# mimbres/neural-audio-fp

Measured on AMD Instinct MI355X. Metric: fingerprint generation throughput (1-s segments/s), higher is better.
Workload: dtype f32

## Files before the change

include/nafp.h:

```cpp
#ifndef NAFP_H
#define NAFP_H

#include <stdint.h>

#ifdef __cplusplus
extern "C" {
#endif

#define NAFP_ABI_VERSION 1

enum {
    NAFP_OK = 0,
    NAFP_ERR_INVALID_ARG = 1,
    NAFP_ERR_UNSUPPORTED = 2,
    NAFP_ERR_HIP = 3,
    NAFP_ERR_WORKSPACE = 4,
    NAFP_ERR_NO_WEIGHTS = 5
};

typedef struct nafp_melspec nafp_melspec;
typedef struct nafp_encoder nafp_encoder;

int nafp_abi_version(void);
const char* nafp_status_string(int status);
int nafp_last_hip_error(void);
uint32_t nafp_crc32c_host(const void* data_host, int64_t n, uint32_t crc);


int nafp_mel_filterbank_host(int fs, int n_fft, int n_mels, float f_min, float f_max,
                             float* out_host);

int nafp_melspec_create(nafp_melspec** plan, int fs, int seg_len, int n_fft, int hop,
                        int n_mels, float f_min, float f_max);
int nafp_melspec_destroy(nafp_melspec* plan);
int nafp_melspec_n_frames(const nafp_melspec* plan);
int nafp_melspec_n_mels(const nafp_melspec* plan);

#define NAFP_MELSPEC_DEFER 2
int nafp_melspec_forward_f32(nafp_melspec* plan, const float* audio, int64_t n_seg,
                             int group_size, int segment_norm, float* feat,
                             float* group_stat, void* stream);
int nafp_melspec_forward_i16(nafp_melspec* plan, const int16_t* audio, int64_t n_seg,
                             int group_size, int segment_norm, float* feat,
                             float* group_stat, void* stream);

int nafp_melspec_finish(nafp_melspec* plan, float* feat, const float* group_stat, int64_t n_seg, int group_size,
                        int segment_norm, void* stream);

int nafp_melspec_forward_windows_i16(nafp_melspec* plan, const int16_t* pcm, const int64_t* seg_offset,
                                     const int32_t* seg_valid, int64_t n_seg, int group_size,
                                     int segment_norm, float* feat, float* group_stat, void* stream);


int nafp_encoder_create(nafp_encoder** enc, int in_f, int in_t, int emb_sz);
int nafp_encoder_destroy(nafp_encoder* enc);

#define NAFP_NORM_LAYER2D 0
#define NAFP_NORM_LAYER1D 1
#define NAFP_NORM_BATCH 2
int nafp_encoder_create_ex(nafp_encoder** enc, int in_f, int in_t, int emb_sz, int norm);
int nafp_encoder_norm(const nafp_encoder* enc);
int nafp_encoder_n_trainable(const nafp_encoder* enc);

int nafp_encoder_n_tensors(const nafp_encoder* enc);
int64_t nafp_encoder_tensor_numel(const nafp_encoder* enc, int index);
int nafp_encoder_tensor_shape(const nafp_encoder* enc, int index, int64_t dims_out[4]);
int64_t nafp_encoder_flat_dim(const nafp_encoder* enc);

int nafp_encoder_set_weights(nafp_encoder* enc, const float* const* tensors_host_array,
                             void* stream);

int64_t nafp_encoder_workspace_bytes(const nafp_encoder* enc, int64_t n_seg);

int nafp_encoder_forward(nafp_encoder* enc, const float* feat, int64_t n_seg,
                         void* workspace, int64_t workspace_bytes,
                         float* out_flat, float* out_emb, int l2norm, void* stream);

int nafp_encoder_forward_raw(nafp_encoder* enc, const float* raw_feat, const float* group_stat, int group_size,
                             int segment_norm, int64_t n_seg, void* workspace, int64_t workspace_bytes,
                             float* out_flat, float* out_emb, int l2norm, void* stream);

#define NAFP_ENCODER_PROFILE_KERNELS 17
int nafp_encoder_profile_enable(nafp_encoder* enc, int max_forwards);
int nafp_encoder_profile_count(const nafp_encoder* enc);
int nafp_encoder_profile_coarse(nafp_encoder* enc, int coarse);
int nafp_encoder_profile_read(nafp_encoder* enc, int slot, float* ms_out_host);
int nafp_conv_timeline(void* dev_buf, int64_t capacity_u64, int cin, int cout, int positions);
int nafp_conv_timeline_grid(int* out5_host);

int64_t nafp_encoder_train_workspace_bytes(const nafp_encoder* enc, int64_t n_seg);
int nafp_encoder_forward_train(nafp_encoder* enc, const float* feat, int64_t n_seg, void* workspace,
                               int64_t workspace_bytes, float* out_emb, int l2norm, void* stream);
int nafp_encoder_backward(nafp_encoder* enc, const float* feat, const float* d_emb, int64_t n_seg,
                          void* workspace, int64_t workspace_bytes, float* const* grads_host_array,
                          int l2norm, void* stream);

#define NAFP_GRAD_GROUPS 4
int nafp_encoder_grad_group_range(const nafp_encoder* enc, int group, int* first_tensor, int* last_tensor);
int nafp_encoder_grad_group_wait(nafp_encoder* enc, int group, void* stream);

#define NAFP_OPT_FUSE_CONV0 1
#define NAFP_OPT_FUSED_LN_BWD 2
#define NAFP_OPT_BWD_OVERLAP 4
#define NAFP_OPT_SMALLNET 5
#define NAFP_OPT_BF16X3 3
int nafp_encoder_set_option(nafp_encoder* enc, int option, int value);

int nafp_encoder_div_enc(nafp_encoder* enc, const float* flat, int64_t n_seg,
                         float* out_emb, int l2norm, void* stream);

int nafp_l2_normalize_rows(const float* x, int64_t n_rows, int dim, float* out, void* stream);

int nafp_pack_embedding_grads(const float* d_a_all, const float* d_b_all, const float* loss_sum, float loss_scale,
                              int64_t world, int64_t n_anchors, int dim, float* send, void* stream);


int64_t nafp_ntxent_workspace_bytes(int64_t n_local, int64_t n_global);

int nafp_ntxent_forward(const float* emb_org_local, const float* emb_rep_local,
                        const float* emb_org_all, const float* emb_rep_all,
                        int64_t n_local, int64_t n_global, int64_t rank_offset, int d,
                        float tau, float* loss_sum, float* sim_mtx,
                        float* d_org_all, float* d_rep_all,
                        void* workspace, int64_t workspace_bytes, void* stream);


typedef struct { int f0, f1, t0, t1; } nafp_rect;

int nafp_specaug_apply(float* feat, int64_t n_seg, int F, int T, const nafp_rect* rects_host,
                       int n_rects, const unsigned char* active, float fill_value, void* stream);

int nafp_specaug_apply_fill_dev(float* feat, int64_t n_seg, int F, int T, const nafp_rect* rects_host,
                                int n_rects, const unsigned char* active, const float* fill_value_dev,
                                void* stream);
int64_t nafp_specaug_mean_workspace_bytes(void);
int nafp_specaug_mean(const float* feat, int64_t n, float* mean_out, void* workspace, int64_t workspace_bytes,
                      void* stream);

int nafp_specaug_apply_ex(float* feat, int64_t n_seg, int F, int T, const int32_t* rects_dev, int n_rects, int64_t n_sets,
                          const unsigned char* active_dev, const float* filler, int64_t n_fill_seg,
                          const float* scale_offset_dev, void* stream);
int nafp_specaug_range(const float* feat, int64_t n, float* scale_offset_out, void* workspace, int64_t workspace_bytes,
                       void* stream);


typedef struct {
    float* param; const float* grad; float* m; float* v;
    int64_t numel; int64_t var_len;
} nafp_opt_tensor;

float nafp_cosine_decay_lr_host(float lr0, int64_t step, int64_t decay_steps, float alpha);
float nafp_cosine_decay_restarts_lr_host(float lr0, int64_t step, int64_t first_decay_steps, float t_mul,
                                         float m_mul, float alpha);

int nafp_adam_step(const nafp_opt_tensor* tensors_host, int n, float lr, float beta1, float beta2,
                   float eps, int64_t step, void* stream);

int64_t nafp_lamb_workspace_bytes(const nafp_opt_tensor* tensors_host, int n);
int nafp_lamb_step(const nafp_opt_tensor* tensors_host, int n, float lr, float beta1, float beta2,
                   float eps, float weight_decay, int64_t step, void* workspace,
                   int64_t workspace_bytes, void* stream);

int64_t nafp_triplet_workspace_bytes(int64_t n_anchor, int64_t n_pos);
int nafp_triplet_forward(const float* emb_anchor, const float* emb_pos, int64_t n_anchor, int64_t n_pos, int dim,
                         int mode, float margin, float* loss_out, float* pairwise_dist, float* d_anchor,
                         float* d_pos, void* workspace, int64_t workspace_bytes, void* stream);

typedef struct nafp_aug_row {
    int64_t ev_off;
    int64_t nz_off;
    int64_t nz2_off;
    int64_t ir_off;
    int32_t ev_valid;
    int32_t nz_valid, nz2_valid;
    int32_t ir_len;
    float snr_db;
    float amp;
    int32_t mix;
    int32_t reserved;
} nafp_aug_row;

int nafp_augment_rows(const int16_t* pcm, const nafp_aug_row* rows, int64_t n_rows, int seg_len, float* out,
                      void* stream);


int64_t nafp_search_index_aux_floats(int64_t n_index);
int nafp_search_index_prepare(const float* index, int64_t n_index, int dim, float* aux, void* stream);

int64_t nafp_search_workspace_bytes(int64_t n_query, int64_t n_index, int k);
int nafp_search_topk_l2(const float* query, int64_t n_query, const float* index, const float* aux,
                        int64_t n_index, int dim, int k, float* out_dist, int32_t* out_ids,
                        void* workspace, int64_t workspace_bytes, void* stream);

int nafp_search_seq_scores(const float* query, const float* index, int64_t n_index, int dim,
                           const int32_t* task_q0, const int32_t* task_len, int64_t n_tasks,
                           const int32_t* cand, int n_slots, float* out_scores, void* stream);

int nafp_minisearch_scores(const float* query, const float* db, int64_t n_query, int64_t n_db, int dim, int mode,
                           float* out_scores, void* stream);
int nafp_minisearch_ranks(const float* scores, int64_t n_query, int64_t n_db, int scope, int mode, int gt_id_offset,
                          int32_t* out_rank, void* stream);

#ifdef __cplusplus
}
#endif
#endif
```

neural-audio-fp_amd/csrc/api.hip:

```cpp
#include "nafp_common.h"

#include <algorithm>
#include <cstdlib>
#include <cstring>
#include <vector>

namespace nafp {

thread_local int g_last_hip_error = 0;

static const int kHiddenCh[8] = {128, 128, 256, 256, 512, 512, 1024, 1024};
static const int kStrideT[8] = {2, 2, 2, 2, 1, 2, 1, 2};

std::vector<ConvGeom> encoder_geometry(int in_f, int in_t) {
    std::vector<ConvGeom> g;
    int F = in_f, T = in_t, C = 1;
    for (int i = 0; i < 8; ++i) {
        SamePad pt = same_pad(T, 3, kStrideT[i]);
        g.push_back(ConvGeom{0, F, T, C, F, pt.n_out, kHiddenCh[i], kStrideT[i], pt.before});
        T = pt.n_out; C = kHiddenCh[i];
        SamePad pf = same_pad(F, 3, 2);
        g.push_back(ConvGeom{1, F, T, C, pf.n_out, T, kHiddenCh[i], 2, pf.before});
        F = pf.n_out;
    }
    return g;
}

struct CopyTable { const float* src[96]; float* dst[96]; int64_t n[96]; int nz[96]; int count; int* nonfinite; };
__device__ __forceinline__ float nz_scale(float g) { return fabsf(g) < 1e-30f ? copysignf(1e-30f, g) : g; }
__device__ __forceinline__ bool nonfinite4(float4 v) {
    return !(fabsf(v.x) <= 3.4028234664e38f) || !(fabsf(v.y) <= 3.4028234664e38f) || !(fabsf(v.z) <= 3.4028234664e38f) || !(fabsf(v.w) <= 3.4028234664e38f);
}
__global__ __launch_bounds__(256) void multi_copy_kernel(const CopyTable t) {
    const int e = blockIdx.y;
    const float* __restrict__ s = t.src[e]; float* __restrict__ d = t.dst[e];
    const int64_t n = t.n[e];
    const bool nz = t.nz[e] != 0;
    bool bad = false;
    if ((((uintptr_t)s | (uintptr_t)d) & 15) == 0) {
        for (int64_t i = blockIdx.x * 256ll + threadIdx.x; i < n / 4; i += (int64_t)gridDim.x * 256) {
            float4 v = ((const float4*)s)[i];
            bad = bad || nonfinite4(v);
            if (nz) { v.x = nz_scale(v.x); v.y = nz_scale(v.y); v.z = nz_scale(v.z); v.w = nz_scale(v.w); }
            ((float4*)d)[i] = v;
        }
        for (int64_t i = n / 4 * 4 + blockIdx.x * 256ll + threadIdx.x; i < n; i += (int64_t)gridDim.x * 256) {
            bad = bad || !(fabsf(s[i]) <= 3.4028234664e38f);
            d[i] = nz ? nz_scale(s[i]) : s[i];
        }
    } else {
        for (int64_t i = blockIdx.x * 256ll + threadIdx.x; i < n; i += (int64_t)gridDim.x * 256) {
            bad = bad || !(fabsf(s[i]) <= 3.4028234664e38f);
            d[i] = nz ? nz_scale(s[i]) : s[i];
        }
    }
    if (bad && t.nonfinite) atomicOr(t.nonfinite, 1);
}
#define NAFP_OPT_DEBUG_SIDE_DELAY 6
#define NAFP_OPT_DEBUG_SW_DELAY 7
__global__ void debug_delay_kernel(long long us) {
    const unsigned long long t0 = __builtin_amdgcn_s_memrealtime();
    while ((long long)(__builtin_amdgcn_s_memrealtime() - t0) < us * 100) __builtin_amdgcn_s_sleep(32);
}
struct BiasTable { float* hb[16]; const float* bias[16]; int64_t n[16]; int cout[16]; int count; };
__global__ __launch_bounds__(256) void add_bias_kernel(const BiasTable t) {
    const int e = blockIdx.y;
    float* __restrict__ h = t.hb[e]; const float* __restrict__ b = t.bias[e];
    const int64_t n = t.n[e]; const int C = t.cout[e];
    for (int64_t i = blockIdx.x * 256ll + threadIdx.x; i < n; i += (int64_t)gridDim.x * 256) h[i] += b[i % C];
}

}

using namespace nafp;

constexpr int NAFP_PROF_EV = 34;
struct nafp_encoder {
    int in_f, in_t, emb_sz;
    int norm = NAFP_NORM_LAYER2D;
    int n_trainable = 68;
    std::vector<float*> d_gc, d_bc, d_mm, d_mv;
    bool ln1d_images_set = false;
    std::vector<ConvGeom> geom;
    int64_t flat_dim; int S;
    std::vector<std::vector<int64_t>> shapes;
    float* d_blob = nullptr;
    int64_t blob_floats = 0;
    std::vector<float*> d_w;
    std::vector<float*> d_bias, d_gamma, d_beta;
    std::vector<float*> d_G, d_Hb;
    float *d_w1p = nullptr, *d_b1p = nullptr, *d_w2p = nullptr, *d_b2 = nullptr;
    std::vector<float*> d_wd;
    float *d_w1k = nullptr, *d_b1k = nullptr, *d_w2k = nullptr;
    double* d_inv_n = nullptr;
    int* d_wflag = nullptr;
    float* d_sw_slab = nullptr; int64_t sw_slab_floats = 0;
    bool has_weights = false;
    hipEvent_t sw_copied = nullptr, sw_l1 = nullptr, sw_done = nullptr;
    hipStream_t sw_stream = nullptr;
    bool sw_recorded = false;
    bool opt_fuse_conv0 = []() { const char* v = getenv("NAFP_FUSE0"); return v && v[0] == '1'; }();
    int opt_fused_ln_bwd = []() { const char* v = getenv("NAFP_DGRAD_LN"); return v ? atoi(v) : 0; }();
    int64_t bufA_per_seg = 0, bufB_per_seg = 0;
    std::vector<hipEvent_t> prof_events;
    int prof_max = 0, prof_count = 0;
    int opt_bf16x3 = 0;
    float* d_x6_blob = nullptr; std::vector<float*> d_whm; std::vector<void*> d_wl; bool x6_dirty = true;
    std::vector<float*> d_wdhm; std::vector<void*> d_wdl;
    int prof_coarse = 0;
    hipEvent_t grad_events[NAFP_GRAD_GROUPS] = {nullptr, nullptr, nullptr, nullptr};
    bool grad_events_valid = false;
    int opt_bwd_overlap = []() { const char* v = getenv("NAFP_BWD_OVERLAP"); return v ? atoi(v) : 2; }();
    bool keep_t_env = []() { const char* v = getenv("NAFP_KEEP_T"); return v && v[0] == '1'; }();
    bool keep_t() const { return keep_t_env || (opt_fused_ln_bwd != 0 && norm == NAFP_NORM_LAYER2D) || norm == NAFP_NORM_LAYER1D; }
    struct TrainRec { const void* ws; int64_t B; bool keep_t; };
    std::vector<TrainRec> train_recs;
    void train_rec_put(const void* ws, int64_t B, bool kt) {
        for (auto& r : train_recs) if (r.ws == ws) { r.B = B; r.keep_t = kt; return; }
        if (train_recs.size() >= 16) train_recs.erase(train_recs.begin());
        train_recs.push_back({ws, B, kt});
    }
    bool train_rec_ok(const void* ws, int64_t B, bool kt) const {
        for (const auto& r : train_recs) if (r.ws == ws) return r.B == B && r.keep_t == kt;
        return false;
    }
    hipStream_t side_stream = nullptr;
    hipEvent_t ev_main[16] = {}, ev_side[16] = {};
    int debug_side_delay_us = 0;
    int debug_sw_delay_us = 0;
    static constexpr int NAFP_SW_STREAMS = 4;
    hipStream_t sw_streams[NAFP_SW_STREAMS] = {};
    hipEvent_t sw_fork = nullptr, sw_join[NAFP_SW_STREAMS] = {};
};

static const int kGroupFirst[NAFP_GRAD_GROUPS] = {48, 32, 16, 0};
static const int kGroupLast[NAFP_GRAD_GROUPS] = {67, 47, 31, 15};

static void profile_free(nafp_encoder* e) {
    for (auto ev : e->prof_events) (void)hipEventDestroy(ev);
    e->prof_events.clear();
    e->prof_max = 0; e->prof_count = 0;
}

static int64_t numel(const std::vector<int64_t>& s) {
    int64_t n = 1;
    for (auto d : s) n *= d;
    return n;
}

extern "C" int nafp_abi_version(void) { return NAFP_ABI_VERSION; }

extern "C" const char* nafp_status_string(int status) {
    switch (status) {
        case NAFP_OK: return "ok";
        case NAFP_ERR_INVALID_ARG: return "invalid argument";
        case NAFP_ERR_UNSUPPORTED: return "unsupported geometry or option";
        case NAFP_ERR_HIP: return "HIP runtime error";
        case NAFP_ERR_WORKSPACE: return "workspace too small";
        case NAFP_ERR_NO_WEIGHTS: return "encoder weights not set";
        default: return "unknown status";
    }
}

extern "C" int nafp_last_hip_error(void) { return g_last_hip_error; }

extern "C" uint32_t nafp_crc32c_host(const void* data, int64_t n, uint32_t crc) {
    static uint32_t T[8][256];
    static bool init = false;
    if (!init) {
        for (uint32_t i = 0; i < 256; ++i) {
            uint32_t c = i;
            for (int k = 0; k < 8; ++k) c = (c >> 1) ^ (0x82F63B78u & (0u - (c & 1u)));
            T[0][i] = c;
        }
        for (uint32_t i = 0; i < 256; ++i)
            for (int t = 1; t < 8; ++t) T[t][i] = (T[t - 1][i] >> 8) ^ T[0][T[t - 1][i] & 0xffu];
        init = true;
    }
    const unsigned char* p = (const unsigned char*)data;
    uint32_t c = ~crc;
    while (n > 0 && ((uintptr_t)p & 7)) { c = (c >> 8) ^ T[0][(c ^ *p++) & 0xffu]; --n; }
    while (n >= 8) {
        uint64_t w; memcpy(&w, p, 8);
        w ^= c;
        c = T[7][w & 0xff] ^ T[6][(w >> 8) & 0xff] ^ T[5][(w >> 16) & 0xff] ^ T[4][(w >> 24) & 0xff] ^
            T[3][(w >> 32) & 0xff] ^ T[2][(w >> 40) & 0xff] ^ T[1][(w >> 48) & 0xff] ^ T[0][(w >> 56) & 0xff];
        p += 8; n -= 8;
    }
    while (n-- > 0) c = (c >> 8) ^ T[0][(c ^ *p++) & 0xffu];
    return ~c;
}

extern "C" int nafp_encoder_create(nafp_encoder** out, int in_f, int in_t, int emb_sz) {
    return nafp_encoder_create_ex(out, in_f, in_t, emb_sz, NAFP_NORM_LAYER2D);
}
extern "C" int nafp_encoder_norm(const nafp_encoder* e) { return e ? e->norm : -1; }
extern "C" int nafp_encoder_n_trainable(const nafp_encoder* e) { return e ? e->n_trainable : -1; }

extern "C" int nafp_encoder_create_ex(nafp_encoder** out, int in_f, int in_t, int emb_sz, int norm) {
    if (!out || in_f <= 0 || in_t <= 0 || emb_sz <= 0) return NAFP_ERR_INVALID_ARG;
    if (norm != NAFP_NORM_LAYER2D && norm != NAFP_NORM_LAYER1D && norm != NAFP_NORM_BATCH) return NAFP_ERR_INVALID_ARG;
    nafp_encoder* e = new nafp_encoder();
    e->in_f = in_f; e->in_t = in_t; e->emb_sz = emb_sz; e->norm = norm;
    e->geom = encoder_geometry(in_f, in_t);
    const ConvGeom& last = e->geom.back();
    e->flat_dim = (int64_t)last.Fout * last.Tout * last.Cout;
    if (e->flat_dim % emb_sz != 0 || emb_sz % 64 != 0 || emb_sz > 256 || e->flat_dim / emb_sz > 16) {
        delete e; return NAFP_ERR_UNSUPPORTED;
    }
    e->S = (int)(e->flat_dim / emb_sz);
    for (int j = 0; j < 16; ++j) {
        const ConvGeom& g = e->geom[j];
        if (g.axis == 0) e->shapes.push_back({1, 3, g.Cin, g.Cout});
        else             e->shapes.push_back({3, 1, g.Cin, g.Cout});
        e->shapes.push_back({g.Cout});
        e->shapes.push_back({g.Fout, g.Tout, g.Cout});
        e->shapes.push_back({g.Fout, g.Tout, g.Cout});
    }
    e->shapes.push_back({emb_sz, e->S, 32});
    e->shapes.push_back({emb_sz, 32});
    e->shapes.push_back({emb_sz, 32, 1});
    e->shapes.push_back({emb_sz, 1});
    int64_t total = 0;
    for (auto& s : e->shapes) total += (numel(s) + 63) / 64 * 64;
    if (norm != NAFP_NORM_LAYER2D) for (int j = 0; j < 16; ++j) total += 4 * ((e->geom[j].Cout + 63) / 64 * 64);
    for (int j = 1; j < 16; ++j) total += 2 * ((numel(e->shapes[4 * j + 2]) + 63) / 64 * 64);
    for (int j = 1; j < 16; ++j) total += (numel(e->shapes[4 * j]) + 63) / 64 * 64;
    total += (numel(e->shapes[64]) + 63) / 64 * 64 + 2 * ((numel(e->shapes[65]) + 63) / 64 * 64) + 64 + 64;
    for (int j = 1; j < 16; ++j) e->sw_slab_floats = std::max(e->sw_slab_floats, conv_gemm_slab_floats(2, e->geom[j]));
    total += nafp_encoder::NAFP_SW_STREAMS * (e->sw_slab_floats + 64);
    e->blob_floats = total;
    hipError_t err = hipMalloc(&e->d_blob, sizeof(float) * total);
    if (err != hipSuccess) { g_last_hip_error = (int)err; delete e; return NAFP_ERR_HIP; }
    float* p = e->d_blob;
    auto take = [&](int idx) { float* r = p; p += (numel(e->shapes[idx]) + 63) / 64 * 64; return r; };
    for (int j = 0; j < 16; ++j) {
        e->d_w.push_back(take(4 * j));
        e->d_bias.push_back(take(4 * j + 1));
        e->d_gamma.push_back(take(4 * j + 2));
        e->d_beta.push_back(take(4 * j + 3));
    }
    e->d_w1p = take(64); e->d_b1p = take(65); e->d_w2p = take(66); e->d_b2 = take(67);
    e->d_G.push_back(nullptr); e->d_Hb.push_back(nullptr);
    for (int j = 1; j < 16; ++j) { e->d_G.push_back(take(4 * j + 2)); e->d_Hb.push_back(take(4 * j + 2)); }
    e->d_wd.push_back(nullptr);
    for (int j = 1; j < 16; ++j) e->d_wd.push_back(take(4 * j));
    e->d_w1k = take(64); e->d_b1k = take(65); e->d_w2k = take(65);
    e->d_inv_n = (double*)p; p += 64;
    e->d_wflag = (int*)p; p += 64;
    e->d_sw_slab = p; p += nafp_encoder::NAFP_SW_STREAMS * (e->sw_slab_floats + 64);
    if (norm != NAFP_NORM_LAYER2D)
        for (int j = 0; j < 16; ++j) {
            const int64_t c = (e->geom[j].Cout + 63) / 64 * 64;
            e->d_gc.push_back(p); e->d_bc.push_back(p + c); e->d_mm.push_back(p + 2 * c); e->d_mv.push_back(p + 3 * c); p += 4 * c;
        }
    for (int j = 0; j < 16; ++j) {
        const int64_t n = numel(e->shapes[4 * j + 2]);
        if (e->d_beta[j] != e->d_gamma[j] + n || (j >= 1 && e->d_Hb[j] != e->d_G[j] + n)) {
            (void)hipFree(e->d_blob); delete e; return NAFP_ERR_UNSUPPORTED;
        }
    }
    {
        double inv_n[16];
        for (int j = 0; j < 16; ++j) inv_n[j] = 1.0 / ((double)e->geom[j].Fout * e->geom[j].Tout * e->geom[j].Cout);
        err = hipMemcpy(e->d_inv_n, inv_n, sizeof(inv_n), hipMemcpyHostToDevice);
        if (err != hipSuccess) { g_last_hip_error = (int)err; (void)hipFree(e->d_blob); delete e; return NAFP_ERR_HIP; }
    }
    for (int j = 0; j < 16; ++j) {
        const ConvGeom& g = e->geom[j];
        const int64_t n = (int64_t)g.Fout * g.Tout * g.Cout;
        if (j % 2 == 0) e->bufA_per_seg = std::max(e->bufA_per_seg, n);
        else            e->bufB_per_seg = std::max(e->bufB_per_seg, n);
    }
    if (norm != NAFP_NORM_LAYER2D) {
        for (int j = 0; j < 16; ++j) { e->shapes[4 * j + 2] = {e->geom[j].Cout}; e->shapes[4 * j + 3] = {e->geom[j].Cout}; }
        if (norm == NAFP_NORM_BATCH)
            for (int j = 0; j < 16; ++j) { e->shapes.push_back({e->geom[j].Cout}); e->shapes.push_back({e->geom[j].Cout}); }
    }
    *out = e;
    return NAFP_OK;
}

extern "C" int nafp_encoder_destroy(nafp_encoder* e) {
    if (!e) return NAFP_OK;
    if (e->d_blob) (void)hipFree(e->d_blob);
    if (e->d_x6_blob) (void)hipFree(e->d_x6_blob);
    profile_free(e);
    for (auto& ev : e->grad_events) if (ev) (void)hipEventDestroy(ev);
    for (auto& ev : e->ev_main) if (ev) (void)hipEventDestroy(ev);
    for (auto& ev : e->ev_side) if (ev) (void)hipEventDestroy(ev);
    if (e->side_stream) (void)hipStreamDestroy(e->side_stream);
    for (auto& q : e->sw_streams) if (q) (void)hipStreamDestroy(q);
    for (auto& ev : e->sw_join) if (ev) (void)hipEventDestroy(ev);
    if (e->sw_fork) (void)hipEventDestroy(e->sw_fork);
    if (e->sw_copied) (void)hipEventDestroy(e->sw_copied);
    if (e->sw_l1) (void)hipEventDestroy(e->sw_l1);
    if (e->sw_done) (void)hipEventDestroy(e->sw_done);
    delete e;
    return NAFP_OK;
}

static int split_weights(nafp_encoder* e, hipStream_t st, int j_lo, int j_hi) {
    SplitTable t; t.count = 0;
    for (int j = j_lo; j <= j_hi; ++j) {
        const int64_t n = (int64_t)e->geom[j].Cout * 3 * e->geom[j].Cin;
        t.wp[t.count] = e->d_w[j]; t.hm[t.count] = e->d_whm[j]; t.wl[t.count] = e->d_wl[j]; t.n8[t.count] = n / 8; t.K[t.count] = 3 * e->geom[j].Cin; ++t.count;
        if (e->geom[j].Cout % 16 == 0 && e->d_wd[j]) {
            t.wp[t.count] = e->d_wd[j]; t.hm[t.count] = e->d_wdhm[j]; t.wl[t.count] = e->d_wdl[j]; t.n8[t.count] = n / 8; t.K[t.count] = 3 * e->geom[j].Cout; ++t.count;
        }
    }
    return launch_split_weights_multi(t, st);
}
static int split_all_weights(nafp_encoder* e, hipStream_t st) {
    { int rcs = split_weights(e, st, 1, 15); if (rcs != NAFP_OK) return rcs; }
    e->x6_dirty = false;
    return NAFP_OK;
}

extern "C" int nafp_encoder_set_option(nafp_encoder* e, int option, int value) {
    if (!e) return NAFP_ERR_INVALID_ARG;
    switch (option) {
        case NAFP_OPT_FUSE_CONV0: e->opt_fuse_conv0 = value != 0; return NAFP_OK;
        case NAFP_OPT_BF16X3:
            if (value < 0 || value > 2) return NAFP_ERR_INVALID_ARG;
            if (value == 2 && !e->d_x6_blob) {
                int64_t tot = 0;
                for (int j = 1; j < 16; ++j) tot += 2 * (((int64_t)e->geom[j].Cout * 3 * e->geom[j].Cin * 3 / 2 + 63) / 64 * 64);
                hipError_t er = hipMalloc(&e->d_x6_blob, sizeof(float) * tot);
                if (er != hipSuccess) { g_last_hip_error = (int)er; e->d_x6_blob = nullptr; return NAFP_ERR_HIP; }
                float* q = e->d_x6_blob;
                e->d_whm.assign(16, nullptr); e->d_wl.assign(16, nullptr); e->d_wdhm.assign(16, nullptr); e->d_wdl.assign(16, nullptr);
                for (int j = 1; j < 16; ++j) {
                    const int64_t n = (int64_t)e->geom[j].Cout * 3 * e->geom[j].Cin;
                    e->d_whm[j] = q; e->d_wl[j] = q + n; q += (n * 3 / 2 + 63) / 64 * 64;
                    e->d_wdhm[j] = q; e->d_wdl[j] = q + n; q += (n * 3 / 2 + 63) / 64 * 64;
                }
                e->x6_dirty = true;
            }
            e->opt_bf16x3 = value; return NAFP_OK;
        case NAFP_OPT_FUSED_LN_BWD:
            if (value < 0 || value > 2) return NAFP_ERR_INVALID_ARG;
            e->opt_fused_ln_bwd = value; return NAFP_OK;
        case NAFP_OPT_BWD_OVERLAP: e->opt_bwd_overlap = value < 0 ? 0 : (value > 2 ? 1 : value); return NAFP_OK;
        case NAFP_OPT_SMALLNET: return NAFP_OK;
        case NAFP_OPT_DEBUG_SIDE_DELAY:
        case NAFP_OPT_DEBUG_SW_DELAY: {
            static const bool hooks = []() { const char* v = getenv("NAFP_TEST_HOOKS"); return v && v[0] == '1'; }();
            if (!hooks) return NAFP_ERR_UNSUPPORTED;
            (option == NAFP_OPT_DEBUG_SIDE_DELAY ? e->debug_side_delay_us : e->debug_sw_delay_us) = value < 0 ? 0 : value; return NAFP_OK;
        }
        default: return NAFP_ERR_INVALID_ARG;
    }
}

extern "C" int nafp_encoder_n_tensors(const nafp_encoder* e) { return e ? (int)e->shapes.size() : -1; }

extern "C" int64_t nafp_encoder_tensor_numel(const nafp_encoder* e, int index) {
    if (!e || index < 0 || index >= (int)e->shapes.size()) return -1;
    return numel(e->shapes[index]);
}

extern "C" int nafp_encoder_tensor_shape(const nafp_encoder* e, int index, int64_t dims_out[4]) {
    if (!e || !dims_out || index < 0 || index >= (int)e->shapes.size()) return -1;
    const auto& s = e->shapes[index];
    for (size_t i = 0; i < s.size(); ++i) dims_out[i] = s[i];
    return (int)s.size();
}

extern "C" int64_t nafp_encoder_flat_dim(const nafp_encoder* e) { return e ? e->flat_dim : -1; }

extern "C" int nafp_encoder_set_weights(nafp_encoder* e, const float* const* t, void* stream) {
    if (!e || !t) return NAFP_ERR_INVALID_ARG;
    for (size_t i = 0; i < e->shapes.size(); ++i)
        if (!t[i]) return NAFP_ERR_INVALID_ARG;
    hipStream_t st = (hipStream_t)stream;
    CopyTable ct; ct.count = 0;
    auto add_copy = [&](const float* src, float* dst, int64_t n, int nz = 0) { ct.src[ct.count] = src; ct.dst[ct.count] = dst; ct.n[ct.count] = n; ct.nz[ct.count] = nz; ++ct.count; };
    add_copy(t[0], e->d_w[0], 3 * e->geom[0].Cout);
    for (int j = 0; j < 16; ++j) {
        const ConvGeom& g = e->geom[j];
        const int64_t nln = (int64_t)g.Fout * g.Tout * g.Cout;
        add_copy(t[4 * j + 1], e->d_bias[j], g.Cout);
        if (e->norm == NAFP_NORM_LAYER2D) {
            add_copy(t[4 * j + 2], e->d_gamma[j], nln, 1);
            add_copy(t[4 * j + 3], e->d_beta[j], nln);
        } else {
            add_copy(t[4 * j + 2], e->d_gc[j], g.Cout);
            add_copy(t[4 * j + 3], e->d_bc[j], g.Cout);
            if (e->norm == NAFP_NORM_BATCH) { add_copy(t[68 + 2 * j], e->d_mm[j], g.Cout); add_copy(t[69 + 2 * j], e->d_mv[j], g.Cout); }
        }
    }
    add_copy(t[64], e->d_w1k, numel(e->shapes[64]));
    add_copy(t[65], e->d_b1k, numel(e->shapes[65]));
    add_copy(t[66], e->d_w2k, numel(e->shapes[66]));
    add_copy(t[67], e->d_b2, e->emb_sz);
    if (!e->sw_copied) {
        NAFP_HIP_CHECK(hipEventCreateWithFlags(&e->sw_copied, hipEventDisableTiming));
        NAFP_HIP_CHECK(hipEventCreateWithFlags(&e->sw_done, hipEventDisableTiming));
        NAFP_HIP_CHECK(hipEventCreateWithFlags(&e->sw_l1, hipEventDisableTiming));
    }
    e->sw_recorded = false;
    NAFP_HIP_CHECK(hipMemsetAsync(e->d_wflag, 0, sizeof(int), st));
    ct.nonfinite = e->d_wflag;
    multi_copy_kernel<<<dim3(32, ct.count), 256, 0, st>>>(ct);
    NAFP_LAUNCH_CHECK();
    if (e->norm == NAFP_NORM_LAYER1D && !e->ln1d_images_set) {
        e->ln1d_images_set = true;
        for (int j = 0; j < 16; ++j) {
            const int64_t nln = (int64_t)e->geom[j].Fout * e->geom[j].Tout * e->geom[j].Cout;
            NAFP_HIP_CHECK(hipMemsetD32Async((hipDeviceptr_t)e->d_gamma[j], 0x3f800000, nln, st));
            NAFP_HIP_CHECK(hipMemsetAsync(e->d_beta[j], 0, sizeof(float) * nln, st));
        }
    } else if (e->norm == NAFP_NORM_BATCH) {
        BnExpandTable bx; bx.count = 16;
        for (int j = 0; j < 16; ++j) {
            bx.gamma_c[j] = e->d_gc[j]; bx.beta_c[j] = e->d_bc[j]; bx.mmean[j] = e->d_mm[j]; bx.mvar[j] = e->d_mv[j];
            bx.gamma_pos[j] = e->d_gamma[j]; bx.n[j] = (int64_t)e->geom[j].Fout * e->geom[j].Tout * e->geom[j].Cout; bx.C[j] = e->geom[j].Cout;
        }
        int rcx = launch_bn_expand(bx, st);
        if (rcx != NAFP_OK) return rcx;
    }
    NAFP_HIP_CHECK(hipEventRecord(e->sw_copied, st));
    auto sw_delay = [&]() -> int {
        if (e->debug_sw_delay_us <= 0) return NAFP_OK;
        debug_delay_kernel<<<1, 64, 0, st>>>((long long)e->debug_sw_delay_us);
        NAFP_LAUNCH_CHECK();
        return NAFP_OK;
    };
    { int rcd = sw_delay(); if (rcd != NAFP_OK) return rcd; }
    auto split_l1 = [&]() -> int { return e->opt_bf16x3 == 2 ? split_weights(e, st, 1, 1) : NAFP_OK; };
    {
        PackTable pt; pt.count = 0; pt.nonfinite = e->d_wflag;
        for (int j = 1; j < 16; ++j) {
            pt.k3[pt.count] = t[4 * j]; pt.wp[pt.count] = e->d_w[j]; pt.wd[pt.count] = e->d_wd[j];
            pt.cin[pt.count] = e->geom[j].Cin; pt.cout[pt.count] = e->geom[j].Cout; ++pt.count;
        }
        int rc = launch_multi_pack(pt, st);
        if (rc != NAFP_OK) return rc;
    }
    BiasTable bt; bt.count = 0;
    static const int ns_env = []() { const char* v = getenv("NAFP_SW_NSTREAMS"); return v ? atoi(v) : nafp_encoder::NAFP_SW_STREAMS; }();
    static const bool gemv_own = []() { const char* v = getenv("NAFP_SW_GEMV_OWN"); return v && v[0] == '1'; }();
    const int NS = std::max(1, std::min<int>(nafp_encoder::NAFP_SW_STREAMS, ns_env));
    if (!e->sw_fork) {
        NAFP_HIP_CHECK(hipEventCreateWithFlags(&e->sw_fork, hipEventDisableTiming));
        for (int k = 0; k < NS; ++k) {
            NAFP_HIP_CHECK(hipStreamCreateWithFlags(&e->sw_streams[k], hipStreamNonBlocking));
            NAFP_HIP_CHECK(hipEventCreateWithFlags(&e->sw_join[k], hipEventDisableTiming));
        }
    }
    bool l1_done = false;
    if (!gh_gemv_eligible(e->geom[1])) {
        ConvGemmArgs a{};
        a.wp = e->d_w[1]; a.plain = true; a.x = e->d_gamma[0]; a.bias = nullptr; a.y = e->d_G[1];
        a.slab = e->sw_slab_floats ? e->d_sw_slab : nullptr; a.slab_floats = e->sw_slab_floats;
        int rc1 = launch_conv_gemm(a, 2, e->geom[1], st);
        if (rc1 != NAFP_OK) return rc1;
        BiasTable b1; b1.count = 1;
        b1.hb[0] = e->d_Hb[1]; b1.bias[0] = e->d_bias[1]; b1.n[0] = (int64_t)e->geom[1].Fout * e->geom[1].Tout * e->geom[1].Cout; b1.cout[0] = e->geom[1].Cout;
        add_bias_kernel<<<dim3(32, 1), 256, 0, st>>>(b1);
        NAFP_LAUNCH_CHECK();
        l1_done = true;
        { int rcs = split_l1(); if (rcs != NAFP_OK) return rcs; }
        NAFP_HIP_CHECK(hipEventRecord(e->sw_l1, st));
        { int rcd = sw_delay(); if (rcd != NAFP_OK) return rcd; }
    }
    NAFP_HIP_CHECK(hipEventRecord(e->sw_fork, st));
    int fork_rc = NAFP_OK;
    int forked = 0;
    for (int k = 0; k < NS && fork_rc == NAFP_OK; ++k) {
        if (hipStreamWaitEvent(e->sw_streams[k], e->sw_fork, 0) != hipSuccess) fork_rc = NAFP_ERR_HIP; else ++forked;
    }
    GhTable gh; gh.count = 0;
    bool by_gemv[16] = {};
    for (int j = 1; j < 16; ++j)
        if (gh.count < GH_MAX_LAYERS && gh_gemv_eligible(e->geom[j])) {
            gh_table_add(gh, e->geom[j], e->d_w[j], e->d_gamma[j - 1], e->d_G[j]);
            by_gemv[j] = true;
            bt.hb[bt.count] = e->d_Hb[j]; bt.bias[bt.count] = e->d_bias[j];
            bt.n[bt.count] = (int64_t)e->geom[j].Fout * e->geom[j].Tout * e->geom[j].Cout; bt.cout[bt.count] = e->geom[j].Cout; ++bt.count;
        }
    if (fork_rc == NAFP_OK && forked == NS) fork_rc = launch_gh_gemv(gh, gemv_own ? st : e->sw_streams[NS - 1]);
    else for (int j = 1; j < 16; ++j) by_gemv[j] = false;
    if (forked != NS) bt.count = 0;
    int n_tiled = 0;
    for (int j = 1; j < 16 && fork_rc == NAFP_OK; ++j) {
        if (by_gemv[j] || (j == 1 && l1_done)) continue;
        const int k = (n_tiled++) % NS;
        ConvGemmArgs a{};
        a.wp = e->d_w[j]; a.plain = true;
        a.x = e->d_gamma[j - 1]; a.bias = nullptr; a.y = e->d_G[j];
        a.slab = e->sw_slab_floats ? e->d_sw_slab + (int64_t)k * (e->sw_slab_floats + 64) : nullptr; a.slab_floats = e->sw_slab_floats;
        fork_rc = launch_conv_gemm(a, 2, e->geom[j], e->sw_streams[k]);
        bt.hb[bt.count] = e->d_Hb[j]; bt.bias[bt.count] = e->d_bias[j];
        bt.n[bt.count] = (int64_t)e->geom[j].Fout * e->geom[j].Tout * e->geom[j].Cout; bt.cout[bt.count] = e->geom[j].Cout; ++bt.count;
    }
    for (int k = 0; k < forked; ++k) {
        if (hipEventRecord(e->sw_join[k], e->sw_streams[k]) != hipSuccess || hipStreamWaitEvent(st, e->sw_join[k], 0) != hipSuccess) {
            (void)hipStreamSynchronize(e->sw_streams[k]);
            if (fork_rc == NAFP_OK) fork_rc = NAFP_ERR_HIP;
        }
    }
    if (fork_rc != NAFP_OK) return fork_rc;
    add_bias_kernel<<<dim3(32, bt.count), 256, 0, st>>>(bt);
    NAFP_LAUNCH_CHECK();
    int rc = launch_pack_div(t[64], t[65], t[66], e->d_w1p, e->d_b1p, e->d_w2p, e->emb_sz, e->S, st);
    if (rc != NAFP_OK) return rc;
    if (!l1_done) {
        { int rcs = split_l1(); if (rcs != NAFP_OK) return rcs; }
        NAFP_HIP_CHECK(hipEventRecord(e->sw_l1, st));
        { int rcd = sw_delay(); if (rcd != NAFP_OK) return rcd; }
    }
    e->x6_dirty = true;
    if (e->opt_bf16x3 == 2) {
        int rcs = split_weights(e, st, 2, 15);
        if (rcs != NAFP_OK) return rcs;
        e->x6_dirty = false;
    }
    NAFP_HIP_CHECK(hipEventRecord(e->sw_done, st));
    e->sw_stream = st; e->sw_recorded = true;
    e->has_weights = true;
    return NAFP_OK;
}

static int wait_weights(nafp_encoder* e, hipStream_t st, int stage = 2) {
    if (!e->sw_recorded || st == e->sw_stream) return NAFP_OK;
    NAFP_HIP_CHECK(hipStreamWaitEvent(st, stage == 0 ? e->sw_copied : (stage == 1 ? e->sw_l1 : e->sw_done), 0));
    return NAFP_OK;
}

static int64_t align_up(int64_t v, int64_t a) { return (v + a - 1) / a * a; }

static int64_t forward_slab_floats(const nafp_encoder* e, int64_t n_seg) {
    int64_t slab = 0;
    for (int j = 1; j < 16; ++j) slab = std::max(slab, conv_gemm_slab_floats(n_seg, e->geom[j], false, fwd_plan_b()));
    return slab;
}

extern "C" int64_t nafp_encoder_workspace_bytes(const nafp_encoder* e, int64_t n_seg) {
    if (!e || n_seg < 0) return -1;
    const int64_t stats = align_up((int64_t)sizeof(double) * 2 * 16 * n_seg, 256) + NAFP_TICKET_SLOTS * (int64_t)sizeof(unsigned);
    const int64_t a = align_up((int64_t)sizeof(float) * e->bufA_per_seg * n_seg, 256);
    const int64_t b = align_up((int64_t)sizeof(float) * e->bufB_per_seg * n_seg, 256);
    return stats + a + b + align_up(forward_slab_floats(e, n_seg) * (int64_t)sizeof(float), 256) + 256;
}

static int encoder_forward_impl(nafp_encoder* e, const float* feat, const float* gstat, int group_size, int segment_norm,
                                int64_t n_seg, void* workspace, int64_t workspace_bytes, float* out_flat,
                                float* out_emb, int l2norm, void* stream);

extern "C" int nafp_encoder_forward(nafp_encoder* e, const float* feat, int64_t n_seg,
                                    void* workspace, int64_t workspace_bytes,
                                    float* out_flat, float* out_emb, int l2norm, void* stream) {
    return encoder_forward_impl(e, feat, nullptr, 0, 0, n_seg, workspace, workspace_bytes, out_flat, out_emb, l2norm, stream);
}

extern "C" int nafp_encoder_forward_raw(nafp_encoder* e, const float* raw_feat, const float* group_stat, int group_size,
                                        int segment_norm, int64_t n_seg, void* workspace, int64_t workspace_bytes,
                                        float* out_flat, float* out_emb, int l2norm, void* stream) {
    if (!group_stat) return NAFP_ERR_INVALID_ARG;
    if (group_size <= 0 || group_size > n_seg) group_size = (int)std::min<int64_t>(n_seg, INT32_MAX);
    return encoder_forward_impl(e, raw_feat, group_stat, group_size, segment_norm & 1, n_seg, workspace, workspace_bytes,
                                out_flat, out_emb, l2norm, stream);
}

static int encoder_forward_impl(nafp_encoder* e, const float* feat, const float* gstat, int group_size, int segment_norm,
                                int64_t n_seg, void* workspace, int64_t workspace_bytes, float* out_flat,
                                float* out_emb, int l2norm, void* stream) {
    if (!e || !feat || !workspace || n_seg < 0) return NAFP_ERR_INVALID_ARG;
    if (!e->has_weights) return NAFP_ERR_NO_WEIGHTS;
    if (n_seg == 0) return NAFP_OK;
    if (workspace_bytes < nafp_encoder_workspace_bytes(e, n_seg)) return NAFP_ERR_WORKSPACE;
    if (n_seg * e->bufA_per_seg >= ((int64_t)1 << 40)) return NAFP_ERR_UNSUPPORTED;
    hipStream_t st = (hipStream_t)stream;
    char* ws = (char*)align_up((int64_t)(uintptr_t)workspace, 256);
    const int64_t stats_only = align_up((int64_t)sizeof(double) * 2 * 16 * n_seg, 256);
    const int64_t stats_bytes = stats_only + NAFP_TICKET_SLOTS * (int64_t)sizeof(unsigned);
    stat_t* stats = (stat_t*)ws;
    unsigned* tickets = (unsigned*)(ws + stats_only);
    float* bufA = (float*)(ws + stats_bytes);
    float* bufB = (float*)(ws + stats_bytes + align_up((int64_t)sizeof(float) * e->bufA_per_seg * n_seg, 256));
    float* slab = (float*)((char*)bufB + align_up((int64_t)sizeof(float) * e->bufB_per_seg * n_seg, 256));
    const int64_t slab_floats = forward_slab_floats(e, n_seg);
    { int wrc = wait_weights(e, st); if (wrc != NAFP_OK) return wrc; }
    if (e->opt_bf16x3 == 2 && e->x6_dirty) {
        { int rcs = split_all_weights(e, st); if (rcs != NAFP_OK) return rcs; }
        if (!e->sw_done) NAFP_HIP_CHECK(hipEventCreateWithFlags(&e->sw_done, hipEventDisableTiming));
        NAFP_HIP_CHECK(hipEventRecord(e->sw_done, st));
        e->sw_stream = st; e->sw_recorded = true;
    }
    NAFP_HIP_CHECK(hipMemsetAsync(stats, 0, stats_bytes, st));
    hipEvent_t* ev = nullptr;
    if (e->prof_max > 0 && e->prof_count < e->prof_max) ev = e->prof_events.data() + (size_t)NAFP_PROF_EV * e->prof_count++;
    if (ev && e->prof_coarse < 2) NAFP_HIP_CHECK(hipEventRecord(ev[0], st));

    const bool alt = e->norm != NAFP_NORM_LAYER2D;
    auto stats_of = [&](int j) { return stats + 2 * n_seg * j; };
    auto row_pass = [&](float* z, int j) -> int {
        if (e->norm != NAFP_NORM_LAYER1D) return NAFP_OK;
        return launch_ln1d_fwd(z, n_seg * e->geom[j].Fout * e->geom[j].Tout, e->geom[j].Cout, e->d_gc[j], e->d_bc[j], st);
    };
    static const bool x6_fuse0 = []() { const char* v = getenv("NAFP_X6_FUSE0"); return !v || v[0] != '0'; }();
    const bool fuse0 = !alt && (e->opt_fuse_conv0 || (e->opt_bf16x3 == 2 && x6_fuse0)) && e->geom[1].axis == 1 && e->geom[1].Cin % 16 == 0 &&
                       e->geom[0].Tin <= 64 && (e->opt_bf16x3 != 2 || e->geom[1].Cin == 128);
    int rc = fuse0 ? launch_conv0_stats(feat, e->d_w[0], e->d_bias[0], stats, n_seg, e->geom[0], st, gstat, group_size, segment_norm)
                   : launch_conv0(feat, e->d_w[0], e->d_bias[0], e->d_gamma[0], bufA, nullptr, stats, n_seg, e->geom[0], st,
                                  gstat, group_size, segment_norm, alt);
    if (rc != NAFP_OK) return rc;
    if (!fuse0) { rc = row_pass(bufA, 0); if (rc != NAFP_OK) return rc; }
    if (ev && e->prof_coarse < 2) NAFP_HIP_CHECK(hipEventRecord(ev[1], st));
    float* cur = bufA;
    for (int j = 1; j < 16; ++j) {
        float* nxt = (j % 2 == 0) ? bufA : bufB;
        ConvGemmArgs a{};
        a.x = cur; a.stats_in = stats_of(j - 1); a.ident_stats = alt;
        a.wp = e->d_w[j]; a.G = e->d_G[j]; a.Hb = e->d_Hb[j]; a.gamma_out = e->d_gamma[j];
        a.y = nxt; a.stats_out = stats + 2 * n_seg * j; a.plain = false;
        a.slab = slab_floats ? slab : nullptr; a.slab_floats = slab_floats; a.tickets = tickets; a.bf16x3 = e->opt_bf16x3;
        static const int x6_layers = []() { const char* v = getenv("NAFP_X6_LAYERS"); return v ? (int)strtol(v, nullptr, 0) : 0xffff; }();
        if (!((x6_layers >> j) & 1)) a.bf16x3 = 0;
        if (a.bf16x3 == 2) { a.wp_hm = e->d_whm[j]; a.wp_l = e->d_wl[j]; }
        a.plan_b = fwd_plan_b();
        if (j == 1 && fuse0) {
            a.x = nullptr; a.f0_feat = feat; a.f0_w = e->d_w[0]; a.f0_bias = e->d_bias[0];
            a.f0_gamma = e->d_gamma[0]; a.f0_geom = &e->geom[0];
            a.f0_gstat = gstat; a.f0_group = group_size; a.f0_segnorm = segment_norm;
        }
        if (ev && e->prof_coarse == 0) { a.ev_start = ev[2 * j]; a.ev_stop = ev[2 * j + 1]; }
        if (ev && e->prof_coarse == 2) {
            if (j == 1) a.ev_start = ev[2];
            if (j == 15) a.ev_stop = ev[31];
        }
        rc = launch_conv_gemm(a, n_seg, e->geom[j], st);
        if (rc != NAFP_OK) return rc;
        rc = row_pass(nxt, j);
        if (rc != NAFP_OK) return rc;
        cur = nxt;
    }
    TailArgs t;
    t.x = cur; t.stats = stats_of(15); t.ident_stats = alt; t.gamma = e->d_gamma[15]; t.beta = e->d_beta[15];
    t.w1p = e->d_w1p; t.b1p = e->d_b1p; t.w2p = e->d_w2p; t.b2 = e->d_b2;
    t.out_flat = out_flat; t.out_emb = out_emb;
    t.D = (int)e->flat_dim; t.Q = e->emb_sz; t.S = e->S; t.l2norm = l2norm; t.nonfinite_weights = e->d_wflag; t.launch_error = nullptr;
    if (ev && e->prof_coarse < 2) NAFP_HIP_CHECK(hipEventRecord(ev[32], st));
    rc = launch_tail(t, n_seg, st);
    if (rc != NAFP_OK) return rc;
    if (ev && e->prof_coarse < 2) NAFP_HIP_CHECK(hipEventRecord(ev[33], st));
    return NAFP_OK;
}

extern "C" int nafp_encoder_profile_enable(nafp_encoder* e, int max_forwards) {
    if (!e || max_forwards < 0 || max_forwards > 4096) return NAFP_ERR_INVALID_ARG;
    profile_free(e);
    for (int i = 0; i < max_forwards * NAFP_PROF_EV; ++i) {
        hipEvent_t ev;
        static const int ev_mode = []() { const char* v = getenv("NAFP_PROF_EVENT_FENCE"); return v ? atoi(v) : 0; }();
        hipError_t err = ev_mode == 1 ? hipEventCreate(&ev)
                         : hipEventCreateWithFlags(&ev, ev_mode == 2 ? hipEventReleaseToDevice : hipEventDisableSystemFence);
        if (err != hipSuccess) { g_last_hip_error = (int)err; profile_free(e); return NAFP_ERR_HIP; }
        e->prof_events.push_back(ev);
    }
    e->prof_max = max_forwards;
    return NAFP_OK;
}

extern "C" int nafp_encoder_profile_coarse(nafp_encoder* e, int coarse) {
    if (!e) return NAFP_ERR_INVALID_ARG;
    e->prof_coarse = coarse < 0 ? 0 : (coarse > 2 ? 2 : coarse);
    return NAFP_OK;
}

extern "C" int nafp_encoder_profile_count(const nafp_encoder* e) { return e ? e->prof_count : -1; }

extern "C" int nafp_encoder_profile_read(nafp_encoder* e, int slot, float* ms_out_host) {
    if (!e || !ms_out_host || slot < 0 || slot >= e->prof_count) return NAFP_ERR_INVALID_ARG;
    hipEvent_t* ev = e->prof_events.data() + (size_t)NAFP_PROF_EV * slot;
    NAFP_HIP_CHECK(hipEventSynchronize(e->prof_coarse == 2 ? ev[31] : ev[33]));
    for (int k = 0; k < 17; ++k) ms_out_host[k] = 0.f;
    if (e->prof_coarse == 2) {
        NAFP_HIP_CHECK(hipEventElapsedTime(ms_out_host + 1, ev[2], ev[31]));
        return NAFP_OK;
    }
    NAFP_HIP_CHECK(hipEventElapsedTime(ms_out_host + 0, ev[0], ev[1]));
    NAFP_HIP_CHECK(hipEventElapsedTime(ms_out_host + 16, ev[32], ev[33]));
    if (e->prof_coarse) {
        NAFP_HIP_CHECK(hipEventElapsedTime(ms_out_host + 1, ev[1], ev[32]));
        return NAFP_OK;
    }
    for (int j = 1; j < 16; ++j) NAFP_HIP_CHECK(hipEventElapsedTime(ms_out_host + j, ev[2 * j], ev[2 * j + 1]));
    return NAFP_OK;
}

extern "C" int nafp_conv_timeline(void* dev_buf, int64_t capacity_u64, int cin, int cout, int positions) {
    if (dev_buf && capacity_u64 <= 0) return NAFP_ERR_INVALID_ARG;
    return conv_timeline_set((unsigned long long*)dev_buf, capacity_u64, cin, cout, positions);
}
extern "C" int nafp_conv_timeline_grid(int* out5_host) {
    if (!out5_host) return NAFP_ERR_INVALID_ARG;
    return conv_timeline_grid(out5_host);
}

extern "C" int nafp_encoder_div_enc(nafp_encoder* e, const float* flat, int64_t n_seg,
                                    float* out_emb, int l2norm, void* stream) {
    if (!e || !flat || !out_emb || n_seg < 0) return NAFP_ERR_INVALID_ARG;
    if (!e->has_weights) return NAFP_ERR_NO_WEIGHTS;
    TailArgs t;
    t.x = flat; t.stats = nullptr; t.ident_stats = false; t.gamma = nullptr; t.beta = nullptr;
    t.w1p = e->d_w1p; t.b1p = e->d_b1p; t.w2p = e->d_w2p; t.b2 = e->d_b2;
    t.out_flat = nullptr; t.out_emb = out_emb;
    t.D = (int)e->flat_dim; t.Q = e->emb_sz; t.S = e->S; t.l2norm = l2norm; t.nonfinite_weights = e->d_wflag; t.launch_error = nullptr;
    { int wrc = wait_weights(e, (hipStream_t)stream); if (wrc != NAFP_OK) return wrc; }
    return launch_tail(t, n_seg, (hipStream_t)stream);
}


namespace {
struct TrainLayout {
    int64_t B;
    stat_t* stats; unsigned* tickets; float* mr; float* sc;
    char* zero_begin; int64_t zero_bytes;
    double* lnsum[16]; float* S1[16]; float* S2[16];
    float* z[16]; float* v[16];
    float* slab; int64_t slab_floats;
    float* slab2; int64_t slab2_floats; unsigned* tickets2;
    float* dA; float* dB; float* dy;
    float* dts[16];
    float* dgp; float* dbp;
    int64_t bytes;
};

TrainLayout train_layout(const nafp_encoder* e, int64_t B, void* ws) {
    TrainLayout L; L.B = B;
    char* p = (char*)(((uintptr_t)ws + 255) & ~(uintptr_t)255);
    char* p0 = p;
    auto take = [&](int64_t bytes) { char* r = p; p += (bytes + 255) / 256 * 256; return r; };
    L.stats = (stat_t*)take((int64_t)sizeof(stat_t) * 2 * 16 * B);
    L.tickets = (unsigned*)take(2 * NAFP_TICKET_SLOTS * (int64_t)sizeof(unsigned));
    L.tickets2 = L.tickets + NAFP_TICKET_SLOTS;
    L.mr = (float*)take((int64_t)sizeof(float) * 2 * 16 * B);
    L.sc = (float*)take((int64_t)sizeof(float) * 8 * B);
    L.zero_begin = p;
    for (int j = 0; j < 16; ++j) L.lnsum[j] = (double*)take((int64_t)sizeof(double) * 2 * B);
    for (int j = 0; j < 16; ++j) {
        const int64_t n = (int64_t)e->geom[j].Fout * e->geom[j].Tout * e->geom[j].Cout;
        L.S1[j] = (float*)take((int64_t)sizeof(float) * n);
        L.S2[j] = (float*)take((int64_t)sizeof(float) * n);
    }
    L.zero_bytes = p - L.zero_begin;
    int64_t max_n = 0;
    for (int j = 0; j < 16; ++j) {
        const int64_t n = (int64_t)e->geom[j].Fout * e->geom[j].Tout * e->geom[j].Cout;
        max_n = std::max(max_n, n);
        L.z[j] = (float*)take((int64_t)sizeof(float) * n * B);
        L.v[j] = ((j == 0 && e->norm != NAFP_NORM_LAYER1D) || !e->keep_t()) ? nullptr : (float*)take((int64_t)sizeof(float) * n * B);
    }
    L.slab_floats = 0;
    for (int j = 1; j < 16; ++j)
        L.slab_floats = std::max(L.slab_floats, std::max(conv_gemm_slab_floats(B, e->geom[j], true), wgrad_slab_floats(B, e->geom[j])));
    L.slab = (float*)take((int64_t)sizeof(float) * L.slab_floats);
    L.slab2_floats = 0;
    for (int j = 1; j < 16; ++j)
        if (e->geom[j].Fout * e->geom[j].Tout < 16) L.slab2_floats = std::max(L.slab2_floats, wgrad_slab_floats(B, e->geom[j]));
    L.slab2 = (float*)take((int64_t)sizeof(float) * L.slab2_floats);
    L.dA = (float*)take((int64_t)sizeof(float) * max_n * B);
    L.dB = (float*)take((int64_t)sizeof(float) * max_n * B);
    L.dy = (float*)take((int64_t)sizeof(float) * e->emb_sz * B);
    for (int j = 0; j < 16; ++j) {
        const int64_t n = (int64_t)e->geom[j].Fout * e->geom[j].Tout * e->geom[j].Cout;
        L.dts[j] = (j >= 1 && e->geom[j].Fout * e->geom[j].Tout < 16) ? (float*)take((int64_t)sizeof(float) * n * B) : nullptr;
    }
    L.dgp = nullptr; L.dbp = nullptr;
    if (e->norm != NAFP_NORM_LAYER2D) {
        L.dgp = (float*)take((int64_t)sizeof(float) * 2 * max_n);
        L.dbp = L.dgp + max_n;
// ... 262 lines not shown
```

neural-audio-fp_amd/csrc/conv.hip:

```cpp
#include "nafp_common.h"
#include <hip/hip_ext.h>

#include <cstdlib>

namespace nafp {

using f32x16 = __attribute__((ext_vector_type(16))) float;
using f32x2 = __attribute__((ext_vector_type(2))) float;
#ifndef NAFP_Z_AUX
#define NAFP_Z_AUX 0
#endif
#ifndef NAFP_T_AUX
#define NAFP_T_AUX 2
#endif
__device__ __forceinline__ int f2i(float x) { return __builtin_bit_cast(int, x); }

__device__ __forceinline__ f32x2 elu2(f32x2 t) {
    const f32x2 m = t * 1.44269504088896341f;
    f32x2 e;
    e.x = fminf(fmaxf(__builtin_amdgcn_exp2f(m.x), 0.f), 1.f);
    e.y = fminf(fmaxf(__builtin_amdgcn_exp2f(m.y), 0.f), 1.f);
    e = e - 1.0f;
    f32x2 r;
    r.x = fmaxf(t.x, e.x); r.y = fmaxf(t.y, e.y);
// ... 185 lines not shown
                                                                      gstat, group_size, segment_norm);
        NAFP_LAUNCH_CHECK();
        return NAFP_OK;
    }
    constexpr int R = 32;
    const int64_t blocks = B * ((g.Fin + R - 1) / R);
    conv0_kernel<false, R><<<dim3((unsigned)blocks), 256, 0, st>>>(feat, w3, bias, nullptr, nullptr, nullptr, stats,
                                                                   g.Fin, g.Tin, g.Tout, g.Cout, g.stride, g.pad, gstat, group_size, segment_norm, 0);
    NAFP_LAUNCH_CHECK();
    return NAFP_OK;
}

constexpr int BN = 128;

#ifdef NAFP_ABLATION
#define NAFP_ABL(p_, bits_) ((p_).abl & (bits_))
#elif defined(NAFP_ABL_CONST)
#define NAFP_ABL(p_, bits_) ((NAFP_ABL_CONST) & (bits_))
#else
#define NAFP_ABL(p_, bits_) (0)
#endif

struct ConvKernelParams {
    const float* x;
    const float* wp;
    const float* wp_hm;
    const unsigned short* wp_l;
    const float* G;
    const float* Hb;
    const float* gamma_out;
    const float* bias;
    const stat_t* stats_in;
    stat_t* stats_out;
    float* y;
    float* v_out;
    int Fin, Tin, Cin, Tout, Cout;
    int axis, stride, pad;
    int B, P;
    int PT, ST, log2ST;
    int n_sg;
    int n_pb, log2_ncol;
    int xcd_group, xcd_full;
    int64_t sample_in;
    int tap_stride;
    double inv_n_in;
    int mode;
    int dgrad;
    int perm_on, perm_n0, perm_c0;
    unsigned wp_bytes;
    int n_split;
    int abl;
    unsigned* tickets;
    float* y_final;
    unsigned long long* tl;
    int opt;
    const float* f0_feat;
    const float* f0_w;
    const float* f0_bias;
    const float* f0_gamma;
    int f0_T, f0_stride, f0_pad;
    const float* f0_gstat;
    int f0_group, f0_segnorm;
    ScalarsJob sj;
};

typedef __attribute__((address_space(3))) void* lds_ptr_t;
typedef unsigned u32x4 __attribute__((ext_vector_type(4)));

__device__ __forceinline__ u32x4 make_rsrc(const void* base, unsigned bytes) {
    const unsigned long long a = (unsigned long long)base;
    u32x4 r;
    r.x = __builtin_amdgcn_readfirstlane((unsigned)a);
    r.y = __builtin_amdgcn_readfirstlane((unsigned)(a >> 32) & 0xffffu);
    r.z = __builtin_amdgcn_readfirstlane(bytes);
    r.w = 0x00020000u;
    return r;
}

__device__ __forceinline__ void lds_dma16(unsigned lds_addr, unsigned voff, u32x4 rsrc, unsigned soff) {
    unsigned keep;
    lds_addr = __builtin_amdgcn_readfirstlane(lds_addr);
    soff = __builtin_amdgcn_readfirstlane(soff);
    asm volatile("s_mov_b32 %0, m0\n\ts_mov_b32 m0, %1\n\ts_nop 4\n\t"
                 "buffer_load_dwordx4 %2, %3, %4 offen lds\n\ts_mov_b32 m0, %0"
                 : "=&s"(keep) : "s"(lds_addr), "v"(voff), "s"(rsrc), "s"(soff) : "memory");
}

struct RowGeom { int inner; unsigned mask; };
__device__ __forceinline__ RowGeom row_geom(const ConvKernelParams& p, int pos) {
    const int fo = pos / p.Tout, to = pos - fo * p.Tout;
    RowGeom g; g.mask = 0;
    if (!p.dgrad) {
        int pos0, lim;
        if (p.axis == 0) { pos0 = to * p.stride - p.pad; lim = p.Tin; g.inner = (fo * p.Tin + pos0) * p.Cin; }
        else             { pos0 = fo * p.stride - p.pad; lim = p.Fin; g.inner = (pos0 * p.Tin + to) * p.Cin; }
#pragma unroll
        for (int t = 0; t < 3; ++t)
            if (pos0 + t >= 0 && pos0 + t < lim) g.mask |= 1u << t;
    } else {
        const int u = (p.axis == 0 ? to : fo) + p.pad;
        const int n_out = p.axis == 0 ? p.Tin : p.Fin;
        const int S = p.axis == 0 ? p.Cin : p.Tin * p.Cin;
        const int A0 = p.axis == 0 ? (fo * p.Tin) * p.Cin : to * p.Cin;
        const int sh = p.stride == 2 ? 1 : 0;
        g.inner = A0 + ((u * S) >> sh);
#pragma unroll
        for (int k = 0; k < 3; ++k) {
            const int d = u - k;
            if (d >= 0 && (d & sh) == 0 && (d >> sh) < n_out) g.mask |= 1u << k;
        }
    }
    return g;
}

__device__ __forceinline__ int tile_pos(const ConvKernelParams& p, int idx) {
    if (!p.perm_on || idx >= p.P) return idx;
    if (p.perm_on == 2) {
        const int L = p.Tout, lines = p.P / L, n0 = L - 1;
        if (idx < lines * n0) { const int line = idx / n0; return line * L + (idx - line * n0); }
        return (idx - lines * n0) * L + n0;
    }
    const int n0 = p.perm_n0;
    if (p.axis == 0) {
        const int L = p.Tout, lines = p.P / L, n1 = L - n0;
        if (idx < lines * n0) { const int line = idx / n0; return line * L + 2 * (idx - line * n0) + p.perm_c0; }
        const int j = idx - lines * n0, line = j / n1;
        return line * L + 2 * (j - line * n1) + 1 - p.perm_c0;
    }
    if (idx < n0 * p.Tout) { const int e = idx / p.Tout; return (2 * e + p.perm_c0) * p.Tout + (idx - e * p.Tout); }
    const int j = idx - n0 * p.Tout, e = j / p.Tout;
    return (2 * e + 1 - p.perm_c0) * p.Tout + (j - e * p.Tout);
}

__device__ __forceinline__ float half_wave_sum_dpp(float x) {
    int v = __builtin_bit_cast(int, x);
#define NAFP_DPP_ADD(ctrl_, rmask_)                                                                       \
    v = __builtin_bit_cast(int, __builtin_bit_cast(float, v) +                                            \
                                    __builtin_bit_cast(float, __builtin_amdgcn_update_dpp(0, v, ctrl_, rmask_, 0xf, true)));
    NAFP_DPP_ADD(0x111, 0xf)
    NAFP_DPP_ADD(0x112, 0xf)
    NAFP_DPP_ADD(0x114, 0xf)
    NAFP_DPP_ADD(0x118, 0xf)
    NAFP_DPP_ADD(0x142, 0xa)
#undef NAFP_DPP_ADD
    return __builtin_bit_cast(float, v);
}

#ifndef NAFP_EXP_X6_NOSPLIT
#define NAFP_EXP_X6_NOSPLIT 0
#endif
#ifndef NAFP_EXP_SKIP_TAP2
#define NAFP_EXP_SKIP_TAP2 0
#endif
template <int BM, int BNT, int BK, int NSTAGE, bool FUSE0, int EPI, int PREC = 0>
__device__ __forceinline__ bool conv_gemm_body(const ConvKernelParams& p) {
    static_assert(!FUSE0 || (BK == 16 && BM == 128), "the in-kernel conv0 generator is written for BK = 16, BM = 128");
    static_assert(BM == 128 || BM == 256, "tile rows");
    static_assert(BNT == 128 || (BNT == 64 && BM == 128 && !FUSE0), "tile columns");
    constexpr int NIW = BNT / 64;
    constexpr int NT = 2 * BM;
    constexpr int NW = BM / 32;
    constexpr int CH = BK / 4;
    constexpr int RPI = 64 / CH;
    constexpr int NI = 32 / RPI;
    constexpr int BROWS = BNT / NW;
    constexpr int NIB = BROWS / RPI;
    static_assert(NIB >= 1, "B rows per wave");
    constexpr int TILE = (FUSE0 && PREC == 2) ? BM * 24 : BM * BK;
    constexpr int TILEB = BNT * BK;
    constexpr int LROWS = BNT / NW;
    constexpr int TILEL = PREC == 2 ? BNT * 8 : 0;
    constexpr int STAGE = TILE + TILEB + TILEL;
    constexpr int NDMA = NI + NIB + (PREC == 2 ? 1 : 0);
    extern __shared__ __attribute__((aligned(16))) float smem[];
    float* sRB = smem + NSTAGE * STAGE;
    float* sCB = sRB + BM;
    int* sPos = (int*)(sCB + BM);
    int* sInner = sPos + 32;
    unsigned* sMask = (unsigned*)(sPos + 64);
    float* sW0 = sCB + BM + 96;
    const int tid = threadIdx.x, lane = tid & 63;
    const int wave = __builtin_amdgcn_readfirstlane(tid >> 6);
    const int wm = wave >> 1, wn = wave & 1;
    int sg = blockIdx.x, pb = blockIdx.y, colz = blockIdx.z, zsp = 0;
    if (p.opt & 8) {
        const unsigned lin = blockIdx.x, G = (unsigned)p.xcd_group;
        unsigned v = lin;
        if (lin < (unsigned)p.xcd_full) {
            const unsigned xcd = lin & 7u, j = lin >> 3;
            const unsigned blk = j / G, i = j - blk * G;
            v = (blk * 8u + xcd) * G + i;
        }
        unsigned rt;
        if (p.opt & 16) {
            const unsigned n_rt = (unsigned)(p.n_sg * p.n_pb);
            unsigned t = v / n_rt; rt = v - t * n_rt;
            if (p.n_split > 1) { const unsigned c = t / (unsigned)p.n_split; zsp = (int)(t - c * (unsigned)p.n_split); t = c; }
            colz = (int)t;
        } else {
            colz = (int)(v & ((1u << p.log2_ncol) - 1u)); v >>= p.log2_ncol;
            if (p.n_split > 1) { const unsigned r = v / (unsigned)p.n_split; zsp = (int)(v - r * (unsigned)p.n_split); v = r; }
            rt = v;
        }
        pb = (int)(rt / (unsigned)p.n_sg); sg = (int)(rt - (unsigned)pb * (unsigned)p.n_sg);
    } else
    if (!(p.opt & 4)) { pb = blockIdx.x / p.n_sg; sg = blockIdx.x - pb * p.n_sg; colz = blockIdx.y; zsp = blockIdx.z; }
    if ((EPI == 3 || EPI == 5) && p.sj.sc) {
        const long long wg = blockIdx.x + (long long)gridDim.x * (blockIdx.y + (long long)gridDim.y * blockIdx.z);
        const long long n_wg = (long long)gridDim.x * gridDim.y * gridDim.z;
        for (long long b = wg * NT + tid; b < p.sj.B; b += n_wg * NT) {
            const float mean = p.sj.mr[2 * b], rstd = p.sj.mr[2 * b + 1];
            float* o = p.sj.sc + 8 * b;
            o[0] = mean; o[1] = rstd;
            o[2] = (float)(p.sj.lnsum[2 * b] * p.sj.inv_n); o[3] = (float)(p.sj.lnsum[2 * b + 1] * p.sj.inv_n);
            o[4] = 1.f / rstd;
            o[5] = p.sj.mr_prev ? p.sj.mr_prev[2 * b + 1] : 1.f;
            o[6] = p.sj.mr_prev ? -p.sj.mr_prev[2 * b] : 0.f;
            o[7] = 0.f;
        }
    }
    const int tile_n0 = colz * BNT;
    const int K = 3 * p.Cin;
#define NAFP_TL(k_)                                                                            \
    if (p.tl && lane == 0)                                                                                 \
        p.tl[(((size_t)blockIdx.x + (size_t)gridDim.x * (blockIdx.y + (size_t)gridDim.y * blockIdx.z)) * 8 + wave) * 8 + (k_)] = \
            __builtin_readcyclecounter();
    if (p.tl && lane == 0)
        p.tl[(((size_t)blockIdx.x + (size_t)gridDim.x * (blockIdx.y + (size_t)gridDim.y * blockIdx.z)) * 8 + wave) * 8] =
            (unsigned long long)__builtin_amdgcn_s_getreg(0xF804) |
            ((unsigned long long)__builtin_amdgcn_s_getreg(0xF814) << 32);
    NAFP_TL(1)
    if (p.opt & 1) __builtin_amdgcn_s_setprio(3);
    const int ST1 = p.ST - 1;
    const int b0 = sg * p.ST;
    const int nb = min(p.ST, p.B - b0);

    const bool stat_thread = tid >= 64 && tid < 64 + p.ST;
    double st_sum = 0.0, st_sq = 0.0;
    if (stat_thread && p.mode != 1 && b0 + tid - 64 < p.B) {
        st_sum = stat_get(p.stats_in + 2 * (int64_t)(b0 + tid - 64));
        st_sq = stat_get(p.stats_in + 2 * (int64_t)(b0 + tid - 64) + 1);
        if (st_sq != st_sq && p.stats_out) stat_poison(p.stats_out + 2 * (int64_t)(b0 + tid - 64));
    }
    if (tid < 32) {
        int pos = p.P, inner = 0; unsigned mask = 0;
        if (tid < p.PT) {
            pos = tile_pos(p, pb * p.PT + tid);
            if (pos < p.P) { const RowGeom rg = row_geom(p, pos); inner = rg.inner; mask = rg.mask; }
        }
        sPos[tid] = pos; sInner[tid] = inner; sMask[tid] = mask;
    }
    __syncthreads();

    constexpr unsigned OOB = 0x80000000u;
    unsigned voffA[NI];
    unsigned vmaskA[NI];
    unsigned voffB[NIB];
#pragma unroll
    for (int q = 0; q < NIB; ++q) {
        const int lr = wave * BROWS + q * RPI + lane / CH;
        const int pc = lane % CH;
        const int swz = BK == 32 ? ((lr >> 1) & 7) : ((lr >> 2) & 3);
        voffB[q] = (unsigned)((tile_n0 + lr) * K + (pc ^ swz) * 4) * 4u;
    }
#pragma unroll
    for (int q = 0; q < NI; ++q) {
        const int lr = wave * 32 + q * RPI + lane / CH;
        const int pc = lane % CH;
        const int swz = BK == 32 ? ((lr >> 1) & 7) : ((lr >> 2) & 3);
        const int lc = pc ^ swz;
        const int slot_q = lr >> p.log2ST;
        const int sl = lr & ST1;
        voffA[q] = 0; vmaskA[q] = 0;
        if (sPos[slot_q] < p.P && sl < nb) {
            voffA[q] = (unsigned)(sl * (int)p.sample_in + sInner[slot_q] + lc * 4) * 4u;
            vmaskA[q] = sMask[slot_q];
        }
    }
    float x0[3][3];
    unsigned g_valid = 0;
    int g_off = 0;
    const int g_row = tid >> 1, g_ch = (tid & 1) * 8;
    const int g_swz = (g_row >> 2) & 3;
    if (FUSE0) {
        for (int i = tid; i < 4 * p.Cin; i += NT) sW0[i] = i < 3 * p.Cin ? p.f0_w[i] : p.f0_bias[i - 3 * p.Cin];
#pragma unroll
        for (int t = 0; t < 3; ++t) { x0[t][0] = 0.f; x0[t][1] = 0.f; x0[t][2] = 0.f; }
        const int pos = pb * p.PT + (g_row >> p.log2ST);
        const int sl = g_row & ST1;
        if (pos < p.P && sl < nb) {
            float f0_gmax = 0.f, f0_nh = 0.f, f0_nd = 1.f;
            if (p.f0_gstat) {
                const int64_t gi = p.f0_group > 0 ? (int64_t)(b0 + sl) / p.f0_group : 0;
                f0_gmax = p.f0_gstat[2 * gi];
                if (p.f0_segnorm) { const float mn = fmaxf(p.f0_gstat[2 * gi + 1] - f0_gmax, -80.f); f0_nh = mn / 2.f; f0_nd = fabsf(f0_nh + 1e-10f); }
            }
            const int fo = pos / p.Tout, to = pos - fo * p.Tout;
            const int f00 = fo * p.stride - p.pad;
            g_off = (f00 * p.Tin + to) * p.Cin;
            const int t00 = to * p.f0_stride - p.f0_pad;
            const float* fb = p.f0_feat + ((int64_t)(b0 + sl) * p.Fin) * p.f0_T;
#pragma unroll
            for (int t = 0; t < 3; ++t) {
                const int f = f00 + t;
                if (f >= 0 && f < p.Fin) {
                    g_valid |= 1u << t;
#pragma unroll
                    for (int k = 0; k < 3; ++k) {
                        const int tt = t00 + k;
                        float xv = 0.f;
                        if (tt >= 0 && tt < p.f0_T) {
                            xv = fb[(int64_t)f * p.f0_T + tt];
                            if (p.f0_gstat) {
                                xv = max_keep_nan(xv - f0_gmax, -80.f);
                                if (p.f0_segnorm) xv = (xv - f0_nh) / f0_nd;
                            }
                        }
                        x0[t][k] = xv;
                    }
                }
            }
        }
        __syncthreads();
    }
    unsigned live = 0;
    {
        const unsigned m = sMask[lane & 31];
#pragma unroll
        for (int t = 0; t < 3; ++t)
            if (__ballot((m >> t) & 1u) != 0ull) live |= 1u << t;
    }
    unsigned tap_pack = 0; int n_live = 0;
#pragma unroll
    for (int t = 0; t < 3; ++t)
        if (live & (1u << t)) { tap_pack |= (unsigned)t << (2 * n_live); ++n_live; }
    const int cpt = p.Cin / BK;
    const int n_steps_all = n_live * cpt;
    int s_begin = 0, n_steps = n_steps_all;
    if (p.n_split > 1) {
        s_begin = (int)((unsigned)(n_steps_all * zsp) / (unsigned)p.n_split);
        n_steps = (int)((unsigned)(n_steps_all * (zsp + 1)) / (unsigned)p.n_split);
    }
#define NAFP_STEP_AT(step_, tsel_, c0_)                                                        \
    const int tsel_ = s_begin == 0 ? ((step_) >= cpt ? 1 : 0) : (step_) / cpt;                 \
    const int c0_ = ((step_) - tsel_ * cpt) * BK;

    const u32x4 rsA = make_rsrc(p.x + (int64_t)b0 * p.sample_in,
                                NAFP_ABL(p, 512) ? 0u : (unsigned)nb * (unsigned)p.sample_in * 4u);
    const u32x4 rsB = make_rsrc(PREC == 2 ? p.wp_hm : p.wp, NAFP_ABL(p, 4096) ? 0u : p.wp_bytes);
    const unsigned lds0 = (unsigned)(unsigned long long)(lds_ptr_t)smem + (unsigned)(wave * 32 * BK * 4);
    const unsigned ldsB0 = (unsigned)(unsigned long long)(lds_ptr_t)smem + (unsigned)((TILE + wave * BROWS * BK) * 4);
    const u32x4 rsL = make_rsrc((const float*)p.wp_l, NAFP_ABL(p, 4096) ? 0u : p.wp_bytes / 2);
    const unsigned ldsL0 = (unsigned)(unsigned long long)(lds_ptr_t)smem + (unsigned)((TILE + TILEB) * 4 + wave * LROWS * 32);
    const unsigned voffL = (unsigned)((tile_n0 + wave * LROWS + (lane >> 1)) * K) * 2u + (unsigned)(lane & 1) * 16u;
#define NAFP_DMA_L(slot_, k0_)                                                                 \
    if (PREC == 2 && lane < 2 * LROWS) lds_dma16(ldsL0 + (unsigned)((slot_) * STAGE * 4), voffL, rsL, (unsigned)((k0_) * 2));

#define NAFP_DMA_STEP(s_, slot_)                                                              \
    {                                                                                          \
        NAFP_STEP_AT(s_, tsel_l, c0_l)                                                         \
        const int tap_l = (int)((tap_pack >> (2 * tsel_l)) & 3u);                              \
        const unsigned la_l = lds0 + (unsigned)((slot_) * STAGE * 4);                          \
        const unsigned lb_l = ldsB0 + (unsigned)((slot_) * STAGE * 4);                         \
        const unsigned tapb_l = (unsigned)(tap_l * p.tap_stride) * 4u;                         \
        _Pragma("unroll") for (int q = 0; q < NI; ++q) {                                       \
            const unsigned va = ((vmaskA[q] >> tap_l) & 1u) ? voffA[q] + tapb_l : OOB;         \
            if (!FUSE0) lds_dma16(la_l + q * RPI * BK * 4, va, rsA, (unsigned)(c0_l * 4));     \
            if (q < NIB) lds_dma16(lb_l + q * RPI * BK * 4, voffB[q], rsB,                      \
                                   (unsigned)((tap_l * p.Cin + c0_l) * 4));                    \
        }                                                                                      \
        NAFP_DMA_L(slot_, tap_l * p.Cin + c0_l)                                                \
    }
    float4 gg0 = make_float4(0.f, 0.f, 0.f, 0.f), gg1 = gg0;
#define NAFP_GEN_LOAD(s_)                                                                     \
    {                                                                                          \
        const int tsel_l = (s_) / cpt;                                                         \
        const int tap_l = (int)((tap_pack >> (2 * tsel_l)) & 3u);                              \
        const int c0_l = ((s_) - tsel_l * cpt) * BK;                                           \
        const int go_l = ((g_valid >> tap_l) & 1u) ? g_off + tap_l * p.tap_stride + c0_l + g_ch : 0; \
        gg0 = *(const float4*)(p.f0_gamma + go_l);                                             \
        gg1 = *(const float4*)(p.f0_gamma + go_l + 4);                                         \
    }
#define NAFP_GEN_ONE(j_, G_) \
    __fmul_rn((ok_l ? elu1(fmaf(xc_l, wt_l[2 * p.Cin + (j_)], fmaf(xb_l, wt_l[p.Cin + (j_)], fmaf(xa_l, wt_l[(j_)], wt_l[3 * p.Cin + (j_)])))) : 0.f), (G_))
#define NAFP_GEN_STORE(s_, slot_)                                                             \
    {                                                                                          \
        const int tsel_l = (s_) / cpt;                                                         \
        const int tap_l = (int)((tap_pack >> (2 * tsel_l)) & 3u);                              \
        const int c0_l = ((s_) - tsel_l * cpt) * BK;                                           \
        const bool ok_l = (g_valid >> tap_l) & 1u;                                             \
        const float xa_l = tap_l == 0 ? x0[0][0] : (tap_l == 1 ? x0[1][0] : x0[2][0]);         \
        const float xb_l = tap_l == 0 ? x0[0][1] : (tap_l == 1 ? x0[1][1] : x0[2][1]);         \
        const float xc_l = tap_l == 0 ? x0[0][2] : (tap_l == 1 ? x0[1][2] : x0[2][2]);         \
        const float* wt_l = sW0 + c0_l + g_ch;                                                 \
        float* dst_l = smem + (slot_) * STAGE + g_row * BK;                                    \
        *(float4*)(dst_l + (((2 * (tid & 1)) ^ g_swz) * 4)) = make_float4(                      \
            NAFP_GEN_ONE(0, gg0.x), NAFP_GEN_ONE(1, gg0.y), NAFP_GEN_ONE(2, gg0.z), NAFP_GEN_ONE(3, gg0.w)); \
        *(float4*)(dst_l + (((2 * (tid & 1) + 1) ^ g_swz) * 4)) = make_float4(                  \
            NAFP_GEN_ONE(4, gg1.x), NAFP_GEN_ONE(5, gg1.y), NAFP_GEN_ONE(6, gg1.z), NAFP_GEN_ONE(7, gg1.w)); \
    }

    f32x16 acc[2][NIW];
#pragma unroll
    for (int mi = 0; mi < 2; ++mi)
#pragma unroll
        for (int ni = 0; ni < NIW; ++ni)
#pragma unroll
            for (int r = 0; r < 16; ++r) acc[mi][ni][r] = 0.f;

    NAFP_TL(2)
    if (p.opt & 1) __builtin_amdgcn_s_setprio(0);
#pragma unroll
    for (int s = 0; s < NSTAGE - 1; ++s)
        if (s_begin + s < n_steps) {
            NAFP_DMA_STEP(s_begin + s, s)
            if (FUSE0 && PREC != 2) {
                NAFP_GEN_LOAD(s_begin + s)
                NAFP_GEN_STORE(s_begin + s, s)
            }
        }

    if (stat_thread) {
        float r = 0.f, c = 0.f;
        if (p.mode != 1 && b0 + tid - 64 < p.B) {
            if (p.inv_n_in < 0.0) {
                const double z = st_sq * 0.0;
                r = (float)(1.0 + z); c = (float)z;
            } else {
                const double mean = st_sum * p.inv_n_in;
                double var = st_sq * p.inv_n_in - mean * mean;
                var = var < 0.0 ? 0.0 : var;
                const double rstd = 1.0 / sqrt(var + (double)LN_EPS);
                r = (float)rstd; c = (float)(-mean * rstd);
            }
        }
        sRB[tid - 64] = r; sCB[tid - 64] = c;
    }

    const int rl = lane & 31, hh = lane >> 5;
    const int rswz = BK == 32 ? ((rl >> 1) & 7) : ((rl >> 2) & 3);
    const int aoff = (wm * 64 + rl) * BK, boff = TILE + (wn * (BNT / 2) + rl) * BK;
    const int ncol = lane & 31;
    const int n_base = tile_n0 + wn * (BNT / 2) + ncol;
    const int g4 = p.ST >> 2;
    constexpr int MIL = 1;
    float Gv[MIL][4][NIW], Hv[MIL][4][NIW], gv[MIL][4][NIW];
    const int pc_bytes = p.P * p.Cout * 4;
    const __amdgpu_buffer_rsrc_t rsG = __builtin_amdgcn_make_buffer_rsrc(const_cast<float*>(p.G), 0, pc_bytes, 0x00020000);
    const __amdgpu_buffer_rsrc_t rsH = __builtin_amdgcn_make_buffer_rsrc(const_cast<float*>(p.Hb), 0, pc_bytes, 0x00020000);
    const __amdgpu_buffer_rsrc_t rsg = __builtin_amdgcn_make_buffer_rsrc(const_cast<float*>(p.gamma_out), 0, pc_bytes, 0x00020000);
#define NAFP_EPI_LOAD(mi_, slot_)                                                              \
    _Pragma("unroll") for (int rg = 0; rg < 4; ++rg) {                                         \
        const int grp_l = wm * 16 + (mi_) * 8 + 2 * rg + (lane >> 5);                          \
        const int pos_l = sPos[grp_l >> (p.log2ST - 2)];                \
        const int pofs_l = pos_l < p.P ? (pos_l * p.Cout + n_base) * 4 : (int)0x80000000;      \
        _Pragma("unroll") for (int ni = 0; ni < NIW; ++ni) {                                   \
            if NAFP_ABL(p, 32) { Gv[slot_][rg][ni] = 0.5f; Hv[slot_][rg][ni] = 0.25f; gv[slot_][rg][ni] = 1.5f; continue; } \
            Gv[slot_][rg][ni] = __builtin_bit_cast(float, __builtin_amdgcn_raw_buffer_load_b32(rsG, pofs_l, ni * 128, 0)); \
            Hv[slot_][rg][ni] = __builtin_bit_cast(float, __builtin_amdgcn_raw_buffer_load_b32(rsH, pofs_l, ni * 128, 0)); \
            gv[slot_][rg][ni] = __builtin_bit_cast(float, __builtin_amdgcn_raw_buffer_load_b32(rsg, pofs_l, ni * 128, 0)); \
        }                                                                                      \
    }
    int slot = 0;
    if NAFP_ABL(p, 8) {
        asm volatile("s_waitcnt vmcnt(0)" ::: "memory");
        if (acc[0][0][0] == 12345.678f) p.y[tid] = smem[tid];
        return false;
    }
#define NAFP_LD_FRAG(St_, kk_, a_, b_)                                                         \
    {                                                                                          \
        const int pc4_l = ((2 * (kk_) + hh) ^ rswz) * 4;                                       \
        _Pragma("unroll") for (int mi = 0; mi < 2; ++mi) a_[mi] = *(const float4*)((St_) + aoff + mi * 32 * BK + pc4_l);   \
        _Pragma("unroll") for (int ni = 0; ni < NIW; ++ni) b_[ni] = *(const float4*)((St_) + boff + ni * 32 * BK + pc4_l); \
    }
#define NAFP_MM_FRAG(a_, b_)                                                                   \
    _Pragma("unroll") for (int mi = 0; mi < 2; ++mi)                                           \
        _Pragma("unroll") for (int ni = 0; ni < NIW; ++ni) {                                   \
            acc[mi][ni] = __builtin_amdgcn_mfma_f32_32x32x2f32(a_[mi].x, b_[ni].x, acc[mi][ni], 0, 0, 0); \
            acc[mi][ni] = __builtin_amdgcn_mfma_f32_32x32x2f32(a_[mi].y, b_[ni].y, acc[mi][ni], 0, 0, 0); \
            acc[mi][ni] = __builtin_amdgcn_mfma_f32_32x32x2f32(a_[mi].z, b_[ni].z, acc[mi][ni], 0, 0, 0); \
            acc[mi][ni] = __builtin_amdgcn_mfma_f32_32x32x2f32(a_[mi].w, b_[ni].w, acc[mi][ni], 0, 0, 0); \
        }
#define NAFP_WAIT_STEP(s_)                                                                     \
    if (NSTAGE == 2 || (s_) + NSTAGE - 2 >= n_steps) asm volatile("s_waitcnt vmcnt(0)" ::: "memory"); \
    else asm volatile("s_waitcnt vmcnt(%0)" :: "i"((NSTAGE - 2) * NDMA) : "memory");
    if (!FUSE0 && BK == 16 && !NAFP_ABL(p, 4 | 2048) && s_begin < n_steps) {
        float4 a0[2], b0[NIW], a1[2], b1[NIW];
        NAFP_STEP_AT(s_begin + NSTAGE - 1, d_tsel0, d_c00)
        int d_tsel = d_tsel0, d_c0 = d_c00;
        int d_tap = 0; unsigned d_tapb = 0;
        unsigned cur_va[NI];
#define NAFP_DMA_TAP()                                                                         \
        {                                                                                      \
            d_tap = (int)((tap_pack >> (2 * d_tsel)) & 3u); d_tapb = (unsigned)(d_tap * p.tap_stride) * 4u; \
            _Pragma("unroll") for (int q = 0; q < NI; ++q) cur_va[q] = (((vmaskA[q] >> d_tap) & 1u) && !(NAFP_EXP_SKIP_TAP2 && d_tap == 2)) ? voffA[q] + d_tapb : OOB; \
        }
        NAFP_DMA_TAP()
#define NAFP_DMA_PIECE(q_, slot_)                                                              \
        {                                                                                      \
            lds_dma16(lds0 + (unsigned)((slot_) * STAGE * 4) + (q_) * RPI * BK * 4, cur_va[q_], rsA, (unsigned)(d_c0 * 4)); \
            if ((q_) < NIB) lds_dma16(ldsB0 + (unsigned)((slot_) * STAGE * 4) + (q_) * RPI * BK * 4, voffB[(q_) < NIB ? (q_) : 0], rsB, \
                                      (unsigned)((d_tap * p.Cin + d_c0) * 4));                 \
            if ((q_) == NI - 1) { d_c0 += BK; if (d_c0 == p.Cin) { d_c0 = 0; ++d_tsel; NAFP_DMA_TAP() } } \
        }
#define NAFP_MM_HALF(a_, b_, mi_)                                                              \
        _Pragma("unroll") for (int ni = 0; ni < NIW; ++ni) {                                   \
            acc[mi_][ni] = __builtin_amdgcn_mfma_f32_32x32x2f32(a_[mi_].x, b_[ni].x, acc[mi_][ni], 0, 0, 0); \
            acc[mi_][ni] = __builtin_amdgcn_mfma_f32_32x32x2f32(a_[mi_].y, b_[ni].y, acc[mi_][ni], 0, 0, 0); \
            acc[mi_][ni] = __builtin_amdgcn_mfma_f32_32x32x2f32(a_[mi_].z, b_[ni].z, acc[mi_][ni], 0, 0, 0); \
            acc[mi_][ni] = __builtin_amdgcn_mfma_f32_32x32x2f32(a_[mi_].w, b_[ni].w, acc[mi_][ni], 0, 0, 0); \
        }
        static_assert(NI == 2, "the DMA of a step is issued as two pieces");
        if (PREC >= 1) {
            typedef __bf16 bf16x8 __attribute__((ext_vector_type(8)));
            for (int s = s_begin; s < n_steps; ++s) {
                NAFP_WAIT_STEP(s)
                __builtin_amdgcn_s_barrier();
                if (s == s_begin) { NAFP_TL(3) }
                const bool has_next = s + NSTAGE - 1 < n_steps && !NAFP_ABL(p, 1);
                int nslot = slot + NSTAGE - 1; if (nslot >= NSTAGE) nslot -= NSTAGE;
                const float* St = smem + slot * STAGE;
                float4 af[2][2], bf[PREC == 2 ? 1 : NIW][2];
                bf16x8 ah[2], al[2], bh[NIW], bl[NIW];
                bf16x8 am[PREC == 2 ? 2 : 1], bm[PREC == 2 ? NIW : 1];
#pragma unroll
                for (int c = 0; c < 2; ++c) {
                    const int pc4 = ((2 * hh + c) ^ rswz) * 4;
#pragma unroll
                    for (int mi = 0; mi < 2; ++mi) af[mi][c] = *(const float4*)(St + aoff + mi * 32 * BK + pc4);
                    if (PREC != 2) {
#pragma unroll
                        for (int ni = 0; ni < NIW; ++ni) bf[ni][c] = *(const float4*)(St + boff + ni * 32 * BK + pc4);
                    }
                }
                if (PREC == 2) {
#pragma unroll
                    for (int ni = 0; ni < NIW; ++ni) {
                        bh[ni] = *(const bf16x8*)(St + boff + ni * 32 * BK + ((hh ^ rswz) * 4));
                        bm[ni] = *(const bf16x8*)(St + boff + ni * 32 * BK + (((2 + hh) ^ rswz) * 4));
                        bl[ni] = *(const bf16x8*)(St + TILE + TILEB + (wn * (BNT / 2) + ni * 32 + rl) * 8 + hh * 4);
                    }
                }
                if (has_next) { NAFP_DMA_PIECE(0, nslot) NAFP_DMA_L(nslot, d_tap * p.Cin + d_c0) NAFP_DMA_PIECE(1, nslot) }
#define NAFP_SPLIT8(f_, hi_, mid_, lo_)                                                        \
                {                                                                                  \
                    const float x_l[8] = {f_[0].x, f_[0].y, f_[0].z, f_[0].w, f_[1].x, f_[1].y, f_[1].z, f_[1].w}; \
                    _Pragma("unroll") for (int e = 0; e < 8; ++e) {                                \
                        const __bf16 h_l = (__bf16)x_l[e];                                         \
                        const float r1_l = x_l[e] - (float)h_l;                                    \
                        hi_[e] = h_l;                                                              \
                        if (PREC == 2 && NAFP_EXP_X6_NOSPLIT) {                                    \
                            mid_[e] = h_l; lo_[e] = h_l;       \
                        } else if (PREC == 2) {                                                    \
                            const __bf16 m_l = (__bf16)r1_l;                                       \
                            mid_[e] = m_l; lo_[e] = (__bf16)(r1_l - (float)m_l);                   \
                        } else {                                                                   \
                            lo_[e] = (__bf16)r1_l;                                                 \
                        }                                                                          \
                    }                                                                              \
                }
#define NAFP_SPLIT8_PAIRS(f_, hi_, mid_, lo_)                                                  \
                {                                                                                  \
                    typedef __bf16 bf16x2_l __attribute__((ext_vector_type(2)));                   \
                    typedef float f32x2_l __attribute__((ext_vector_type(2)));                     \
                    typedef unsigned u32x4_l __attribute__((ext_vector_type(4)));                  \
                    const float x_l[8] = {f_[0].x, f_[0].y, f_[0].z, f_[0].w, f_[1].x, f_[1].y, f_[1].z, f_[1].w}; \
                    u32x4_l uh_l, um_l, ul_l;                                                      \
                    _Pragma("unroll") for (int e = 0; e < 4; ++e) {                                \
                        f32x2_l x2; x2.x = x_l[2 * e]; x2.y = x_l[2 * e + 1];                      \
                        const unsigned h2 = __builtin_bit_cast(unsigned, __builtin_convertvector(x2, bf16x2_l)); \
                        f32x2_l r2; r2.x = x2.x - __uint_as_float(h2 << 16); r2.y = x2.y - __uint_as_float(h2 & 0xffff0000u); \
                        const unsigned m2 = __builtin_bit_cast(unsigned, __builtin_convertvector(r2, bf16x2_l)); \
                        f32x2_l t2; t2.x = r2.x - __uint_as_float(m2 << 16); t2.y = r2.y - __uint_as_float(m2 & 0xffff0000u); \
                        uh_l[e] = h2; um_l[e] = m2; ul_l[e] = __builtin_bit_cast(unsigned, __builtin_convertvector(t2, bf16x2_l)); \
                    }                                                                              \
                    hi_ = __builtin_bit_cast(bf16x8, uh_l); mid_ = __builtin_bit_cast(bf16x8, um_l); lo_ = __builtin_bit_cast(bf16x8, ul_l); \
                }
                if (PREC == 2 && !NAFP_EXP_X6_NOSPLIT) {
#pragma unroll
                    for (int mi = 0; mi < 2; ++mi) NAFP_SPLIT8_PAIRS(af[mi], ah[mi], am[PREC == 2 ? mi : 0], al[mi])
                } else {
#pragma unroll
                for (int mi = 0; mi < 2; ++mi) NAFP_SPLIT8(af[mi], ah[mi], am[PREC == 2 ? mi : 0], al[mi])
                }
#undef NAFP_SPLIT8_PAIRS
                if (PREC != 2) {
#pragma unroll
                    for (int ni = 0; ni < NIW; ++ni) NAFP_SPLIT8(bf[PREC == 2 ? 0 : ni], bh[ni], bm[0], bl[ni])
                }
#undef NAFP_SPLIT8
#pragma unroll
                for (int mi = 0; mi < 2; ++mi)
#pragma unroll
                    for (int ni = 0; ni < NIW; ++ni) {
                        if (PREC == 2) {
                            acc[mi][ni] = __builtin_amdgcn_mfma_f32_32x32x16_bf16(al[mi], bh[ni], acc[mi][ni], 0, 0, 0);
                            acc[mi][ni] = __builtin_amdgcn_mfma_f32_32x32x16_bf16(am[PREC == 2 ? mi : 0], bm[PREC == 2 ? ni : 0], acc[mi][ni], 0, 0, 0);
                            acc[mi][ni] = __builtin_amdgcn_mfma_f32_32x32x16_bf16(ah[mi], bl[ni], acc[mi][ni], 0, 0, 0);
                            acc[mi][ni] = __builtin_amdgcn_mfma_f32_32x32x16_bf16(am[PREC == 2 ? mi : 0], bh[ni], acc[mi][ni], 0, 0, 0);
                            acc[mi][ni] = __builtin_amdgcn_mfma_f32_32x32x16_bf16(ah[mi], bm[PREC == 2 ? ni : 0], acc[mi][ni], 0, 0, 0);
                            acc[mi][ni] = __builtin_amdgcn_mfma_f32_32x32x16_bf16(ah[mi], bh[ni], acc[mi][ni], 0, 0, 0);
                        } else {
                            acc[mi][ni] = __builtin_amdgcn_mfma_f32_32x32x16_bf16(al[mi], bh[ni], acc[mi][ni], 0, 0, 0);
                            acc[mi][ni] = __builtin_amdgcn_mfma_f32_32x32x16_bf16(ah[mi], bl[ni], acc[mi][ni], 0, 0, 0);
                            acc[mi][ni] = __builtin_amdgcn_mfma_f32_32x32x16_bf16(ah[mi], bh[ni], acc[mi][ni], 0, 0, 0);
                        }
                    }
                if (++slot == NSTAGE) slot = 0;
            }
        } else {
        {
            NAFP_WAIT_STEP(s_begin)
            __builtin_amdgcn_s_barrier();
            NAFP_TL(3)
            const float* St = smem + slot * STAGE;
            NAFP_LD_FRAG(St, 0, a0, b0)
            NAFP_LD_FRAG(St, 1, a1, b1)
            __builtin_amdgcn_sched_barrier(0);
            if (s_begin + NSTAGE - 1 < n_steps && !NAFP_ABL(p, 1)) { NAFP_DMA_PIECE(0, NSTAGE - 1) NAFP_DMA_PIECE(1, NSTAGE - 1) }
            __builtin_amdgcn_sched_barrier(0);
            NAFP_MM_FRAG(a0, b0)
            __builtin_amdgcn_sched_barrier(0);
            slot = 1;
        }
#define NAFP_K_STEP(SLOT_, NSLOT_)                                                             \
        {                                                                                      \
             \
            asm volatile("s_waitcnt lgkmcnt(0)" ::: "memory");                                 \
            NAFP_WAIT_STEP(s)                                                                  \
            __builtin_amdgcn_s_barrier();                                                      \
            const bool has_next = s + NSTAGE - 1 < n_steps && !NAFP_ABL(p, 1);                 \
            const int nslot = (NSLOT_);                                                        \
            const float* St = smem + (SLOT_) * STAGE;                                          \
            NAFP_LD_FRAG(St, 0, a0, b0)                                                        \
            __builtin_amdgcn_sched_barrier(0);                                                 \
            NAFP_MM_HALF(a1, b1, 0)                                                            \
            __builtin_amdgcn_sched_barrier(0);                                                 \
            if (has_next) { NAFP_DMA_PIECE(0, nslot) }                                         \
            __builtin_amdgcn_sched_barrier(0);                                                 \
            NAFP_MM_HALF(a1, b1, 1)                                                            \
            __builtin_amdgcn_sched_barrier(0);                                                 \
            if (has_next) { NAFP_DMA_PIECE(1, nslot) }                                         \
            NAFP_LD_FRAG(St, 1, a1, b1)                                                        \
            __builtin_amdgcn_sched_barrier(0);                                                 \
            if (s == n_steps - 1) break;           \
            NAFP_MM_FRAG(a0, b0)                                                               \
            __builtin_amdgcn_sched_barrier(0);                                                 \
            ++s;                                                                               \
        }
        static_assert(PREC != 0 || NSTAGE == 3 || BNT == 64, "the K-loop body is written out once per ring slot (128-column tiles)");
        if (s_begin + 1 < n_steps) {
            if (BNT == 128) {
                for (int s = s_begin + 1;;) {
                    NAFP_K_STEP(1, 0)
                    NAFP_K_STEP(2, 1)
                    NAFP_K_STEP(0, 2)
                }
            } else {
                int rs = 1;
                int s = s_begin + 1;
                for (; s < n_steps - 1;) {
                    NAFP_K_STEP(rs, (rs == 0 ? NSTAGE - 1 : rs - 1))
                    if (++rs == NSTAGE) rs = 0;
                }
                do { NAFP_K_STEP(rs, (rs == 0 ? NSTAGE - 1 : rs - 1)) } while (false);
            }
        }
#undef NAFP_K_STEP
        if ((EPI == 0 || EPI == 1) && BM == 128) { NAFP_EPI_LOAD(0, 0) }
        __builtin_amdgcn_sched_barrier(0);
        if (s_begin + 1 < n_steps) { NAFP_MM_FRAG(a0, b0) }
        NAFP_MM_FRAG(a1, b1)
        }
#undef NAFP_DMA_PIECE
#undef NAFP_DMA_TAP
#undef NAFP_MM_HALF
    } else if (FUSE0 && PREC == 2) {
        typedef __bf16 bf16x8 __attribute__((ext_vector_type(8)));
        static_assert(!(FUSE0 && PREC == 2) || NSTAGE == 2, "two ring slots");
        constexpr int C0 = 128;
        const int a_rd = (wm * 64 + rl) * 8 + ((hh ^ ((rl >> 3) & 1)) * 4);
        const int a_wr = g_row * 8 + (((tid & 1) ^ ((g_row >> 3) & 1)) * 4);
        const __amdgpu_buffer_rsrc_t rsG0 = __builtin_amdgcn_make_buffer_rsrc(const_cast<float*>(p.f0_gamma), 0, (int)((unsigned)p.sample_in * 4u), 0x00020000);
        int gvoff0, gvoff1, gvoff2;
        gvoff0 = (g_valid & 1u) ? (g_off + g_ch) * 4 : (int)0x80000000;
        gvoff1 = (g_valid & 2u) ? (g_off + p.tap_stride + g_ch) * 4 : (int)0x80000000;
        gvoff2 = (g_valid & 4u) ? (g_off + 2 * p.tap_stride + g_ch) * 4 : (int)0x80000000;
        const float* wrow = sW0 + g_ch;
        int g_tsel = 0, g_c0 = 0;
        float4 wq[8], gq[2];
        float gxa = 0.f, gxb = 0.f, gxc = 0.f;
#define NAFP_X6_GEN_REQ()                                                                      \
        {                                                                                      \
            const int tap_l = (int)((tap_pack >> (2 * g_tsel)) & 3u);                          \
            gxa = tap_l == 0 ? x0[0][0] : (tap_l == 1 ? x0[1][0] : x0[2][0]);                  \
            gxb = tap_l == 0 ? x0[0][1] : (tap_l == 1 ? x0[1][1] : x0[2][1]);                  \
            gxc = tap_l == 0 ? x0[0][2] : (tap_l == 1 ? x0[1][2] : x0[2][2]);                  \
            const int gv_l = tap_l == 0 ? gvoff0 : (tap_l == 1 ? gvoff1 : gvoff2);             \
            gq[0] = __builtin_bit_cast(float4, __builtin_amdgcn_raw_buffer_load_b128(rsG0, gv_l, g_c0 * 4, 0));      \
            gq[1] = __builtin_bit_cast(float4, __builtin_amdgcn_raw_buffer_load_b128(rsG0, gv_l + 16, g_c0 * 4, 0)); \
            const float* w_l = wrow + g_c0;                                                    \
            _Pragma("unroll") for (int r_ = 0; r_ < 4; ++r_) {                                 \
                wq[2 * r_] = *(const float4*)(w_l + r_ * C0); wq[2 * r_ + 1] = *(const float4*)(w_l + r_ * C0 + 4); \
            }                                                                                  \
            g_c0 += BK; if (g_c0 == C0) { g_c0 = 0; ++g_tsel; }                                \
        }
#define NAFP_X6_GEN_ONE(e_) \
        __fmul_rn(elu1(fmaf(gxc, ((const float*)&wq[4])[e_], fmaf(gxb, ((const float*)&wq[2])[e_], fmaf(gxa, ((const float*)&wq[0])[e_], ((const float*)&wq[6])[e_])))), ((const float*)&gq[0])[e_])
#define NAFP_X6_GEN(slot_)                                                                     \
        {                                                                                      \
            bf16x8 h_l, m_l, l_l;                                                              \
            _Pragma("unroll") for (int e = 0; e < 8; ++e) {                                    \
                const float v_l = NAFP_X6_GEN_ONE(e);                                          \
                const __bf16 hh_l = (__bf16)v_l;                                               \
                const float r1_l = v_l - (float)hh_l;                                          \
                const __bf16 mm_l = (__bf16)r1_l;                                              \
                h_l[e] = hh_l; m_l[e] = mm_l; l_l[e] = (__bf16)(r1_l - (float)mm_l);           \
            }                                                                                  \
            float* dst_l = smem + (slot_) * STAGE + a_wr;                                      \
            *(bf16x8*)dst_l = h_l; *(bf16x8*)(dst_l + BM * 8) = m_l; *(bf16x8*)(dst_l + 2 * BM * 8) = l_l; \
        }
        NAFP_X6_GEN_REQ()
        NAFP_X6_GEN(0)
#define NAFP_X6_MFMAS()                                                                        \
        _Pragma("unroll") for (int mi = 0; mi < 2; ++mi)                                       \
            _Pragma("unroll") for (int ni = 0; ni < NIW; ++ni) {                               \
                acc[mi][ni] = __builtin_amdgcn_mfma_f32_32x32x16_bf16(al[mi], bh[ni], acc[mi][ni], 0, 0, 0); \
                acc[mi][ni] = __builtin_amdgcn_mfma_f32_32x32x16_bf16(am[mi], bm[ni], acc[mi][ni], 0, 0, 0); \
                acc[mi][ni] = __builtin_amdgcn_mfma_f32_32x32x16_bf16(ah[mi], bl[ni], acc[mi][ni], 0, 0, 0); \
                acc[mi][ni] = __builtin_amdgcn_mfma_f32_32x32x16_bf16(am[mi], bh[ni], acc[mi][ni], 0, 0, 0); \
                acc[mi][ni] = __builtin_amdgcn_mfma_f32_32x32x16_bf16(ah[mi], bm[ni], acc[mi][ni], 0, 0, 0); \
                acc[mi][ni] = __builtin_amdgcn_mfma_f32_32x32x16_bf16(ah[mi], bh[ni], acc[mi][ni], 0, 0, 0); \
            }
#define NAFP_X6_READ_FRAGS(St_)                                                                \
        _Pragma("unroll") for (int mi = 0; mi < 2; ++mi) {                                     \
            ah[mi] = *(const bf16x8*)((St_) + a_rd + mi * 32 * 8);                             \
            am[mi] = *(const bf16x8*)((St_) + BM * 8 + a_rd + mi * 32 * 8);                    \
            al[mi] = *(const bf16x8*)((St_) + 2 * BM * 8 + a_rd + mi * 32 * 8);                \
        }                                                                                      \
        _Pragma("unroll") for (int ni = 0; ni < NIW; ++ni) {                                   \
            bh[ni] = *(const bf16x8*)((St_) + boff + ni * 32 * BK + ((hh ^ rswz) * 4));        \
            bm[ni] = *(const bf16x8*)((St_) + boff + ni * 32 * BK + (((2 + hh) ^ rswz) * 4));  \
            bl[ni] = *(const bf16x8*)((St_) + TILE + TILEB + (wn * (BNT / 2) + ni * 32 + rl) * 8 + hh * 4); \
        }
        int s = 0;
        for (; s + 1 < n_steps; ++s) {
            asm volatile("s_waitcnt vmcnt(0) lgkmcnt(0)" ::: "memory");
            __builtin_amdgcn_s_barrier();
            if (s == 0) { NAFP_TL(3) }
            const int nslot = slot ^ 1;
            const float* St = smem + slot * STAGE;
            bf16x8 ah[2], am[2], al[2], bh[NIW], bm[NIW], bl[NIW];
            NAFP_X6_READ_FRAGS(St)
            NAFP_DMA_STEP(s + 1, nslot)
            NAFP_X6_GEN_REQ()
            NAFP_X6_MFMAS()
            NAFP_X6_GEN(nslot)
            slot = nslot;
        }
        {
            asm volatile("s_waitcnt vmcnt(0) lgkmcnt(0)" ::: "memory");
            __builtin_amdgcn_s_barrier();
            const float* St = smem + slot * STAGE;
            bf16x8 ah[2], am[2], al[2], bh[NIW], bm[NIW], bl[NIW];
            NAFP_X6_READ_FRAGS(St)
            NAFP_X6_MFMAS()
        }
#undef NAFP_X6_GEN_REQ
#undef NAFP_X6_GEN_ONE
#undef NAFP_X6_GEN
#undef NAFP_X6_MFMAS
#undef NAFP_X6_READ_FRAGS
    } else
    for (int s = s_begin; s < n_steps; ++s) {
        if (FUSE0) asm volatile("s_waitcnt vmcnt(0) lgkmcnt(0)" ::: "memory");
        else if (NSTAGE == 2 || s + NSTAGE - 2 >= n_steps) asm volatile("s_waitcnt vmcnt(0)" ::: "memory");
        else asm volatile("s_waitcnt vmcnt(%0)" :: "i"((NSTAGE - 2) * (NI + NIB)) : "memory");
        __builtin_amdgcn_s_barrier();
        const bool has_next = s + NSTAGE - 1 < n_steps && !NAFP_ABL(p, 1);
        int nslot = slot + NSTAGE - 1; if (nslot >= NSTAGE) nslot -= NSTAGE;
        const float* St = smem + slot * STAGE;
        if NAFP_ABL(p, 4) {
            if (has_next) { NAFP_DMA_STEP(s + NSTAGE - 1, nslot) }
            if (++slot == NSTAGE) slot = 0;
            continue;
        }
        float4 a0[2], b0[NIW];
        {
            const int pc4 = ((0 + hh) ^ rswz) * 4;
#pragma unroll
            for (int mi = 0; mi < 2; ++mi) a0[mi] = *(const float4*)(St + aoff + mi * 32 * BK + pc4);
#pragma unroll
            for (int ni = 0; ni < NIW; ++ni) b0[ni] = *(const float4*)(St + boff + ni * 32 * BK + pc4);
        }
        if (has_next) {
            NAFP_DMA_STEP(s + NSTAGE - 1, nslot)
            if (FUSE0) NAFP_GEN_LOAD(s + NSTAGE - 1)
        }
#pragma unroll
        for (int kk = 0; kk < BK / 8; ++kk) {
            const int pc4 = ((2 * kk + hh) ^ rswz) * 4;
            float4 a[2], b[NIW];
#pragma unroll
            for (int mi = 0; mi < 2; ++mi) a[mi] = kk == 0 ? a0[mi] : *(const float4*)(St + aoff + mi * 32 * BK + pc4);
#pragma unroll
            for (int ni = 0; ni < NIW; ++ni) b[ni] = kk == 0 ? b0[ni] : *(const float4*)(St + boff + ni * 32 * BK + pc4);
#pragma unroll
            for (int mi = 0; mi < 2; ++mi)
#pragma unroll
                for (int ni = 0; ni < NIW; ++ni) {
                    acc[mi][ni] = __builtin_amdgcn_mfma_f32_32x32x2f32(a[mi].x, b[ni].x, acc[mi][ni], 0, 0, 0);
                    acc[mi][ni] = __builtin_amdgcn_mfma_f32_32x32x2f32(a[mi].y, b[ni].y, acc[mi][ni], 0, 0, 0);
                    acc[mi][ni] = __builtin_amdgcn_mfma_f32_32x32x2f32(a[mi].z, b[ni].z, acc[mi][ni], 0, 0, 0);
                    acc[mi][ni] = __builtin_amdgcn_mfma_f32_32x32x2f32(a[mi].w, b[ni].w, acc[mi][ni], 0, 0, 0);
                }
        }
        if (FUSE0 && has_next) NAFP_GEN_STORE(s + NSTAGE - 1, nslot)
        if (++slot == NSTAGE) slot = 0;
    }
    NAFP_TL(4)
    if (p.opt & 2) __builtin_amdgcn_s_setprio(3);
    asm volatile("s_waitcnt lgkmcnt(0)" ::: "memory");
    __builtin_amdgcn_s_barrier();
    NAFP_TL(5)

    if NAFP_ABL(p, 2) {
        float t = 0.f;
#pragma unroll
        for (int mi = 0; mi < 2; ++mi)
#pragma unroll
            for (int ni = 0; ni < NIW; ++ni)
#pragma unroll
                for (int r = 0; r < 16; ++r) t += acc[mi][ni][r];
        if (t == 12345.678f) p.y[tid] = t;
        return false;
    }
    const int ystep_b = p.P * p.Cout * 4;
    if (EPI == 3) {
        float bv[NIW];
#pragma unroll
        for (int ni = 0; ni < NIW; ++ni) bv[ni] = p.bias ? p.bias[n_base + ni * 32] : 0.f;
#pragma unroll
        for (int ni = 0; ni < NIW; ++ni) asm volatile("" : "+v"(bv[ni]));
        const __amdgpu_buffer_rsrc_t rsP = __builtin_amdgcn_make_buffer_rsrc(
            p.y + ((int64_t)zsp * p.B + b0) * p.P * p.Cout, 0, (int)((unsigned)nb * (unsigned)ystep_b), 0x00020000);
#pragma unroll
        for (int mi = 0; mi < 2; ++mi)
#pragma unroll
            for (int rg = 0; rg < 4; ++rg) {
                const int grp = wm * 16 + mi * 8 + 2 * rg + (lane >> 5);
                const int pos = sPos[grp >> (p.log2ST - 2)];
                const int sl0 = (grp & (g4 - 1)) << 2;
                const int voff = pos < p.P ? ((sl0 * p.P + pos) * p.Cout + n_base) * 4 : (int)0x80000000;
#pragma unroll
                for (int q = 0; q < 4; ++q)
#pragma unroll
                    for (int ni = 0; ni < NIW; ++ni)
                        __builtin_amdgcn_raw_buffer_store_b32(f2i(acc[mi][ni][rg * 4 + q] + bv[ni]), rsP, voff, q * ystep_b + ni * 128, 0);
            }
        NAFP_TL(6)
        NAFP_TL(7)
        return false;
    }

    if (EPI == 4 || EPI == 5) {
        const __amdgpu_buffer_rsrc_t rsP = __builtin_amdgcn_make_buffer_rsrc(
            p.y + ((int64_t)zsp * p.B + b0) * p.P * p.Cout, 0, (int)((unsigned)nb * (unsigned)ystep_b), 0x00020000);
        int voffs[2][4];
#pragma unroll
        for (int mi = 0; mi < 2; ++mi)
#pragma unroll
            for (int rg = 0; rg < 4; ++rg) {
                const int grp = wm * 16 + mi * 8 + 2 * rg + (lane >> 5);
                const int pos = sPos[grp >> (p.log2ST - 2)];
                const int sl0 = (grp & (g4 - 1)) << 2;
                voffs[mi][rg] = pos < p.P ? ((sl0 * p.P + pos) * p.Cout + n_base) * 4 : (int)0x80000000;
#pragma unroll
                for (int q = 0; q < 4; ++q)
#pragma unroll
                    for (int ni = 0; ni < NIW; ++ni)
                        __builtin_amdgcn_raw_buffer_store_b32(f2i(acc[mi][ni][rg * 4 + q]), rsP, voffs[mi][rg], q * ystep_b + ni * 128, 17);
            }
        asm volatile("s_waitcnt vmcnt(0)" ::: "memory");
        __builtin_amdgcn_s_barrier();
        unsigned* sTicket = (unsigned*)smem;
        const unsigned tile_id = (unsigned)((pb * p.n_sg + sg) * (p.Cout / BNT) + colz);
        if (tid == 0) sTicket[0] = __hip_atomic_fetch_add(p.tickets + tile_id, 1u, __ATOMIC_RELAXED, __HIP_MEMORY_SCOPE_AGENT);
        __syncthreads();
        const unsigned ticket = sTicket[0];
        if (ticket != (unsigned)(p.n_split - 1)) return false;
        __syncthreads();
        if (tid == 0)
            __hip_atomic_store(p.tickets + tile_id, 0u, __ATOMIC_RELAXED, __HIP_MEMORY_SCOPE_AGENT);
#pragma unroll
        for (int mi = 0; mi < 2; ++mi)
#pragma unroll
            for (int ni = 0; ni < NIW; ++ni)
#pragma unroll
                for (int r = 0; r < 16; ++r) acc[mi][ni][r] = 0.f;
        for (int z = 0; z < p.n_split; ++z) {
            const __amdgpu_buffer_rsrc_t rsZ = __builtin_amdgcn_make_buffer_rsrc(
                p.y + ((int64_t)z * p.B + b0) * p.P * p.Cout, 0, (int)((unsigned)nb * (unsigned)ystep_b), 0x00020000);
#pragma unroll
            for (int mi = 0; mi < 2; ++mi)
#pragma unroll
                for (int rg = 0; rg < 4; ++rg)
#pragma unroll
                    for (int q = 0; q < 4; ++q)
#pragma unroll
                        for (int ni = 0; ni < NIW; ++ni)
                            acc[mi][ni][rg * 4 + q] += __builtin_bit_cast(
                                float, __builtin_amdgcn_raw_buffer_load_b32(rsZ, voffs[mi][rg], q * ystep_b + ni * 128, 17));
        }
        if (EPI == 5) {
            float bv[NIW];
#pragma unroll
            for (int ni = 0; ni < NIW; ++ni) bv[ni] = p.bias ? p.bias[n_base + ni * 32] : 0.f;
#pragma unroll
            for (int ni = 0; ni < NIW; ++ni) asm volatile("" : "+v"(bv[ni]));
            const __amdgpu_buffer_rsrc_t rsF = __builtin_amdgcn_make_buffer_rsrc(
                p.y_final + (int64_t)b0 * p.P * p.Cout, 0, (int)((unsigned)nb * (unsigned)ystep_b), 0x00020000);
#pragma unroll
            for (int mi = 0; mi < 2; ++mi)
#pragma unroll
                for (int rg = 0; rg < 4; ++rg)
#pragma unroll
                    for (int q = 0; q < 4; ++q)
#pragma unroll
                        for (int ni = 0; ni < NIW; ++ni)
                            __builtin_amdgcn_raw_buffer_store_b32(f2i(acc[mi][ni][rg * 4 + q] + bv[ni]), rsF, voffs[mi][rg], q * ystep_b + ni * 128, 0);
            return false;
        }
    }

    f32x2 s2[2] = {{0.f, 0.f}, {0.f, 0.f}}, q2[2] = {{0.f, 0.f}, {0.f, 0.f}};
    float* rowS = smem;
    float* rowQ = smem + BM;
    const bool fast_stats = (EPI != 2 && EPI != 4) || p.ST == 4 || p.ST == 8;
    if (!fast_stats) {
        if (tid < BM) { rowS[tid] = 0.f; rowQ[tid] = 0.f; }
        __syncthreads();
    }
    constexpr bool PREF = (EPI == 0 || EPI == 1) && !FUSE0 && BK == 16 && BM == 128 && PREC == 0;
    if (MIL == 2) { if (!PREF) { NAFP_EPI_LOAD(0, 0) } NAFP_EPI_LOAD(1, MIL - 1) }
    const __amdgpu_buffer_rsrc_t rsY = __builtin_amdgcn_make_buffer_rsrc(
        (EPI == 4 ? p.y_final : p.y) + (int64_t)b0 * p.P * p.Cout, 0, (int)((unsigned)nb * (unsigned)ystep_b), 0x00020000);
    const __amdgpu_buffer_rsrc_t rsV = __builtin_amdgcn_make_buffer_rsrc(
        (p.v_out ? p.v_out : (EPI == 4 ? p.y_final : p.y)) + (int64_t)b0 * p.P * p.Cout, 0, (int)((unsigned)nb * (unsigned)ystep_b), 0x00020000);
#define NAFP_EPI_MAIN(KEEP_, FAST_)                                                            \
    _Pragma("unroll") for (int mi = 0; mi < 2; ++mi) {                                         \
        const int ms = MIL == 2 ? mi : 0;                                                      \
        if (MIL == 1 && !(PREF && mi == 0)) { NAFP_EPI_LOAD(mi, 0) }                           \
        _Pragma("unroll") for (int rg = 0; rg < 4; ++rg) {                                     \
            const int grp = wm * 16 + mi * 8 + 2 * rg + (lane >> 5);       \
            const int pos = sPos[grp >> (p.log2ST - 2)];                                       \
            const int sl0 = (grp & (g4 - 1)) << 2;                          \
            const int voff = pos < p.P ? ((sl0 * p.P + pos) * p.Cout + n_base) * 4 : (int)0x80000000; \
            _Pragma("unroll") for (int qp = 0; qp < 2; ++qp) {              \
                const int r0 = rg * 4 + 2 * qp;                                                \
                const f32x2 rb2 = *(const f32x2*)(sRB + sl0 + 2 * qp), cb2 = *(const f32x2*)(sCB + sl0 + 2 * qp); \
                f32x2 rs2 = {0.f, 0.f}, rq2 = {0.f, 0.f};                                      \
                _Pragma("unroll") for (int ni = 0; ni < NIW; ++ni) {                           \
                    const f32x2 a2 = {acc[mi][ni][r0], acc[mi][ni][r0 + 1]};                   \
                    const f32x2 t2 = __builtin_elementwise_fma(rb2, a2, __builtin_elementwise_fma(cb2, (f32x2)(Gv[ms][rg][ni]), (f32x2)(Hv[ms][rg][ni]))); \
                    const f32x2 v2 = NAFP_ABL(p, 128) ? t2 : elu2(t2);     \
                    const f32x2 z2 = v2 * gv[ms][rg][ni];                                      \
                    if (!NAFP_ABL(p, 64)) {                                 \
                        __builtin_amdgcn_raw_buffer_store_b32(f2i(z2.x), rsY, voff, (2 * qp) * ystep_b + ni * 128, NAFP_Z_AUX); \
                        __builtin_amdgcn_raw_buffer_store_b32(f2i(z2.y), rsY, voff, (2 * qp + 1) * ystep_b + ni * 128, NAFP_Z_AUX); \
                    }                                                                          \
                    if (KEEP_) {                                            \
                        __builtin_amdgcn_raw_buffer_store_b32(f2i(t2.x), rsV, voff, (2 * qp) * ystep_b + ni * 128, NAFP_T_AUX); \
                        __builtin_amdgcn_raw_buffer_store_b32(f2i(t2.y), rsV, voff, (2 * qp + 1) * ystep_b + ni * 128, NAFP_T_AUX); \
                    }                                                                          \
                    rs2 += v2; rq2 = __builtin_elementwise_fma(v2, v2, rq2);                   \
                }                                                                              \
                if (FAST_) { s2[qp] += rs2; q2[qp] += rq2; }                                   \
                else {                                                                         \
                    _Pragma("unroll") for (int h2 = 0; h2 < 2; ++h2) {                         \
                        float rs = rs2[h2], rq = rq2[h2];                                      \
                        _Pragma("unroll") for (int o = 16; o > 0; o >>= 1) { rs += __shfl_xor(rs, o, 64); rq += __shfl_xor(rq, o, 64); } \
                        if (ncol == 0) { atomicAdd(rowS + (grp << 2) + 2 * qp + h2, rs); atomicAdd(rowQ + (grp << 2) + 2 * qp + h2, rq); } \
                    }                                                                          \
                }                                                                              \
            }                                                                                  \
        }                                                                                      \
    }
    if (EPI == 0) { NAFP_EPI_MAIN(false, true) }
    else if (EPI == 1) { NAFP_EPI_MAIN(true, true) }
    else if (fast_stats) {
        if (p.v_out) { NAFP_EPI_MAIN(true, true) } else { NAFP_EPI_MAIN(false, true) }
    } else {
        if (p.v_out) { NAFP_EPI_MAIN(true, false) } else { NAFP_EPI_MAIN(false, false) }
    }
#undef NAFP_EPI_MAIN
    NAFP_TL(6)
    if NAFP_ABL(p, 16) {
        if (s2[0].x + s2[0].y + s2[1].x + s2[1].y + q2[0].x + q2[0].y + q2[1].x + q2[1].y == 12345.678f) p.y[tid] = 1.f;
        return false;
    }
    if (fast_stats) {
        double* red = (double*)smem;
        float hs[4], hq[4];
#pragma unroll
        for (int q = 0; q < 4; ++q) { hs[q] = half_wave_sum_dpp(s2[q >> 1][q & 1]); hq[q] = half_wave_sum_dpp(q2[q >> 1][q & 1]); }
        if ((lane & 31) == 31) {
#pragma unroll
            for (int q = 0; q < 4; ++q) {
                red[wave * 16 + (lane >> 5) * 8 + q] = (double)hs[q];
                red[wave * 16 + (lane >> 5) * 8 + 4 + q] = (double)hq[q];
            }
        }
        __syncthreads();
        if (tid < 2 * p.ST) {
            const int which = tid / p.ST, sl = tid - which * p.ST;
            const int b = sg * p.ST + sl;
            if (b < p.B) {
                double t = 0.0;
                if (p.ST == 8) {
#pragma unroll
                    for (int w = 0; w < NW; ++w) t += red[w * 16 + (sl >> 2) * 8 + which * 4 + (sl & 3)];
                } else {
#pragma unroll
                    for (int w = 0; w < NW; ++w) t += red[w * 16 + which * 4 + sl] + red[w * 16 + 8 + which * 4 + sl];
                }
                stat_add(p.stats_out + 2 * (int64_t)b + which, t, p.inv_n_in < 0.0);
            }
        }
    } else {
        __syncthreads();
        if (tid < p.ST) {
            const int b = sg * p.ST + tid;
            if (b < p.B) {
                double ds = 0.0, dq = 0.0;
                for (int pl = 0; pl < p.PT; ++pl) { ds += (double)rowS[pl * p.ST + tid]; dq += (double)rowQ[pl * p.ST + tid]; }
                stat_add(p.stats_out + 2 * (int64_t)b, ds, p.inv_n_in < 0.0);
                stat_add(p.stats_out + 2 * (int64_t)b + 1, dq, p.inv_n_in < 0.0);
            }
        }
    }
    NAFP_TL(7)
#undef NAFP_TL
    return true;
}

#define NAFP_GEMM_KERNEL(name_, BM_, BN_, BK_, NSTAGE_, MINW_, FUSE0_, EPI_)                 \
    __global__ __launch_bounds__(2 * BM_, MINW_) void name_(const ConvKernelParams p) {       \
        conv_gemm_body<BM_, BN_, BK_, NSTAGE_, FUSE0_, EPI_>(p);                              \
    }
#define NAFP_GEMM_KERNEL_BF16X3(name_, BM_, BN_, NSTAGE_, MINW_)                                \
    __global__ __launch_bounds__(2 * BM_, MINW_) void name_(const ConvKernelParams p) {       \
        conv_gemm_body<BM_, BN_, 16, NSTAGE_, false, 0, 1>(p);                                \
    }
#define NAFP_GEMM_KERNEL_BF16X6(name_, BM_, BN_, NSTAGE_, MINW_, EPI_)                          \
    __global__ __launch_bounds__(2 * BM_, MINW_) void name_(const ConvKernelParams p) {       \
        conv_gemm_body<BM_, BN_, 16, NSTAGE_, false, EPI_, 2>(p);                             \
    }
#define NAFP_GEMM_KERNELS(name_, BM_, BN_, MINW_)                                             \
    NAFP_GEMM_KERNEL(name_##_infer, BM_, BN_, 16, 3, MINW_, false, 0)                         \
    NAFP_GEMM_KERNEL(name_##_train, BM_, BN_, 16, 3, MINW_, false, 1)                         \
    NAFP_GEMM_KERNEL(name_##_any, BM_, BN_, 16, 3, MINW_, false, 2)                           \
    NAFP_GEMM_KERNEL(name_##_plain, BM_, BN_, 16, 3, MINW_, false, 3)                         \
    static void (*const name_##_tab[4])(const ConvKernelParams) = {name_##_infer, name_##_train, name_##_any, name_##_plain};
NAFP_GEMM_KERNELS(conv_gemm_k16s3, 128, 128, 3)
NAFP_GEMM_KERNEL(conv_gemm_k16s3_fuse0, 128, 128, 16, 3, 3, true, 0)
NAFP_GEMM_KERNEL(conv_gemm_n64k16s3_infer, 128, 64, 16, 3, 4, false, 0)
NAFP_GEMM_KERNEL(conv_gemm_n64k16s3_train, 128, 64, 16, 3, 4, false, 1)
NAFP_GEMM_KERNEL(conv_gemm_n64k16s3_any, 128, 64, 16, 3, 4, false, 2)
NAFP_GEMM_KERNEL(conv_gemm_n64k16s3_plain, 128, 64, 16, 3, 4, false, 3)
NAFP_GEMM_KERNEL(conv_gemm_n64k16s3_splitfin, 128, 64, 16, 3, 4, false, 4)
NAFP_GEMM_KERNEL(conv_gemm_n64k16s3_plainfin, 128, 64, 16, 3, 4, false, 5)
NAFP_GEMM_KERNEL(conv_gemm_k16s3_plainfin, 128, 128, 16, 3, 3, false, 5)
NAFP_GEMM_KERNEL(conv_gemm_n64k16s2_infer, 128, 64, 16, 2, 5, false, 0)
NAFP_GEMM_KERNEL(conv_gemm_n64k16s2_train, 128, 64, 16, 2, 5, false, 1)
NAFP_GEMM_KERNEL(conv_gemm_n64k16s2_splitfin, 128, 64, 16, 2, 5, false, 4)
static void (*const conv_gemm_n64k16s2_tab[5])(const ConvKernelParams) = {conv_gemm_n64k16s2_infer, conv_gemm_n64k16s2_train, nullptr, nullptr,
                                                                           conv_gemm_n64k16s2_splitfin};
static void (*const conv_gemm_n64k16s3_tab[5])(const ConvKernelParams) = {conv_gemm_n64k16s3_infer, conv_gemm_n64k16s3_train, conv_gemm_n64k16s3_any,
                                                                           conv_gemm_n64k16s3_plain, conv_gemm_n64k16s3_splitfin};
NAFP_GEMM_KERNEL(conv_gemm_m256k16s3_infer, 256, 128, 16, 3, 4, false, 0)
NAFP_GEMM_KERNEL(conv_gemm_m256k16s3_train, 256, 128, 16, 3, 4, false, 1)
NAFP_GEMM_KERNEL(conv_gemm_m256k16s3_plain, 256, 128, 16, 3, 4, false, 3)
static void (*const conv_gemm_m256k16s3_tab[4])(const ConvKernelParams) = {conv_gemm_m256k16s3_infer, conv_gemm_m256k16s3_train, nullptr,
                                                                            conv_gemm_m256k16s3_plain};

NAFP_GEMM_KERNEL_BF16X3(conv_gemm_k16s3_infer_bf16x3, 128, 128, 3, 3)
NAFP_GEMM_KERNEL_BF16X3(conv_gemm_m256k16s3_infer_bf16x3, 256, 128, 3, 4)
NAFP_GEMM_KERNEL_BF16X3(conv_gemm_n64k16s2_infer_bf16x3, 128, 64, 2, 5)
#ifndef NAFP_X6_K16_NSTAGE
#define NAFP_X6_K16_NSTAGE 2
#endif
#ifndef NAFP_X6_K16_MINW
#define NAFP_X6_K16_MINW 3
#endif
#ifndef NAFP_X6_M256_NSTAGE
#define NAFP_X6_M256_NSTAGE 3
#endif
#ifndef NAFP_X6_M256_MINW
#define NAFP_X6_M256_MINW 2
#endif
NAFP_GEMM_KERNEL_BF16X6(conv_gemm_k16s3_infer_bf16x6, 128, 128, NAFP_X6_K16_NSTAGE, NAFP_X6_K16_MINW, 0)
NAFP_GEMM_KERNEL_BF16X6(conv_gemm_m256k16s3_infer_bf16x6, 256, 128, NAFP_X6_M256_NSTAGE, NAFP_X6_M256_MINW, 0)
NAFP_GEMM_KERNEL_BF16X6(conv_gemm_n64k16s2_infer_bf16x6, 128, 64, 2, 4, 0)
NAFP_GEMM_KERNEL_BF16X6(conv_gemm_k16s3_plain_bf16x6, 128, 128, NAFP_X6_K16_NSTAGE, NAFP_X6_K16_MINW, 3)
NAFP_GEMM_KERNEL_BF16X6(conv_gemm_k16s3_train_bf16x6, 128, 128, NAFP_X6_K16_NSTAGE, NAFP_X6_K16_MINW, 1)
NAFP_GEMM_KERNEL_BF16X6(conv_gemm_n64k16s2_train_bf16x6, 128, 64, 2, 4, 1)
NAFP_GEMM_KERNEL_BF16X6(conv_gemm_k16s3_any_bf16x6, 128, 128, NAFP_X6_K16_NSTAGE, NAFP_X6_K16_MINW, 2)
NAFP_GEMM_KERNEL_BF16X6(conv_gemm_n64k16s2_any_bf16x6, 128, 64, 2, 4, 2)
NAFP_GEMM_KERNEL_BF16X6(conv_gemm_n64k16s2_plain_bf16x6, 128, 64, 2, 4, 3)
__global__ __launch_bounds__(256, 3) void conv_gemm_k16s2_fuse0_bf16x6(const ConvKernelParams p) {
    conv_gemm_body<128, 128, 16, 2, true, 0, 2>(p);
}

static thread_local hipEvent_t g_ev_start = nullptr, g_ev_stop = nullptr;

__global__ __launch_bounds__(256) void split_weights_multi_kernel(const SplitTable t) {
    const float* __restrict__ wp = t.wp[blockIdx.y];
    unsigned short* __restrict__ hm = (unsigned short*)t.hm[blockIdx.y];
    unsigned short* __restrict__ wl = (unsigned short*)t.wl[blockIdx.y];
    const int64_t n8 = t.n8[blockIdx.y];
    const int K = t.K[blockIdx.y];
    typedef unsigned short u16x8 __attribute__((ext_vector_type(8)));
    for (int64_t i8 = blockIdx.x * 256ll + threadIdx.x; i8 < n8; i8 += (int64_t)gridDim.x * 256) {
        const int64_t i = i8 * 8;
        const float4 a = *(const float4*)(wp + i), b = *(const float4*)(wp + i + 4);
        const float x[8] = {a.x, a.y, a.z, a.w, b.x, b.y, b.z, b.w};
        u16x8 vh, vm, vl;
#pragma unroll
        for (int e = 0; e < 8; ++e) {
            const __bf16 h = (__bf16)x[e];
            const float r1 = x[e] - (float)h;
            const __bf16 m = (__bf16)r1;
            vh[e] = __builtin_bit_cast(unsigned short, h);
            vm[e] = __builtin_bit_cast(unsigned short, m);
            vl[e] = __builtin_bit_cast(unsigned short, (__bf16)(r1 - (float)m));
        }
        const int64_t row = i / K;
        const int k = (int)(i - row * K);
        const int64_t base = row * 2 * K + (int64_t)(k >> 4) * 32 + (k & 8);
        *(u16x8*)(hm + base) = vh;
        *(u16x8*)(hm + base + 16) = vm;
        *(u16x8*)(wl + i) = vl;
    }
}

int launch_split_weights_multi(const SplitTable& t, hipStream_t st) {
    if (t.count <= 0) return NAFP_OK;
    int64_t n8_max = 0;
    for (int j = 0; j < t.count; ++j) {
        if (t.K[j] % 16 != 0) return NAFP_ERR_UNSUPPORTED;
        n8_max = std::max(n8_max, t.n8[j]);
    }
    split_weights_multi_kernel<<<dim3((unsigned)std::min<int64_t>((n8_max + 255) / 256, 1024), (unsigned)t.count), 256, 0, st>>>(t);
    NAFP_LAUNCH_CHECK();
    return NAFP_OK;
}

template <typename KernelT>
static int launch_variant(KernelT kernel, int BM, int BNt, int BK, int NSTAGE, const ConvKernelParams& p, dim3 grid, hipStream_t st,
                          int extra_stage_floats = 0) {
    static const int lds_pad = []() { const char* e = getenv("NAFP_LDS_PAD"); return e ? atoi(e) : 0; }();
    const int lds = (NSTAGE * ((BM + BNt) * BK + extra_stage_floats) + 2 * BM + 96 + (p.f0_feat ? 4 * p.Cin : 0)) * (int)sizeof(float) + lds_pad;
    NAFP_HIP_CHECK(hipFuncSetAttribute((const void*)kernel, hipFuncAttributeMaxDynamicSharedMemorySize, lds));
    if (g_ev_start || g_ev_stop) {
        ConvKernelParams pc = p;
        void* args[] = {(void*)&pc};
        NAFP_HIP_CHECK(hipExtLaunchKernel((const void*)kernel, grid, dim3(2 * BM), args, (size_t)lds, st, g_ev_start, g_ev_stop, 0));
        g_ev_start = nullptr; g_ev_stop = nullptr;
    } else {
        kernel<<<grid, 2 * BM, lds, st>>>(p);
    }
    NAFP_LAUNCH_CHECK();
    return NAFP_OK;
}

constexpr int FIN_MAXS = 64;
template <int FIN_F4>
__global__ __launch_bounds__(256) void splitk_finish_kernel(
        const float* __restrict__ slab, int S, const float* __restrict__ G, const float* __restrict__ Hb,
        const float* __restrict__ gamma_out, const stat_t* __restrict__ stats_in,
        stat_t* __restrict__ stats_out, float* __restrict__ y, float* __restrict__ v_out, int B, int P, int Cout,
        double inv_n_in) {
    __shared__ float sR[FIN_MAXS], sC[FIN_MAXS];
    __shared__ float sPart[4][FIN_F4 / 256][2][2];
    __shared__ int sPartB[4][FIN_F4 / 256][2];
    const int tid = threadIdx.x, lane = tid & 63;
    const int c4 = Cout / 4;
    const int64_t total = (int64_t)B * P * c4;
    const int64_t i0 = (int64_t)blockIdx.x * FIN_F4;
    const int64_t i_last = std::min<int64_t>(total, i0 + FIN_F4) - 1;
    const int b_first = (int)((i0 / c4) / P), b_last = (int)((i_last / c4) / P);
    if (tid <= b_last - b_first) {
        const int b = b_first + tid;
        stat_ln_scalars(stats_in + 2 * (int64_t)b, inv_n_in, &sR[tid], &sC[tid]);
        stat_forward_poison(stats_in + 2 * (int64_t)b, stats_out + 2 * (int64_t)b);
    }
    __syncthreads();
    const int64_t slab_stride4 = total;
#pragma unroll 1
    for (int e = 0; e < FIN_F4 / 256; ++e) {
        const int64_t idx = i0 + e * 256 + tid;
        const bool live = idx < total;
        const int64_t ii = live ? idx : i0;
        const int64_t row = ii / c4;
        const int n = (int)(ii - row * c4) * 4;
        const int b = (int)(row / P), pos = (int)(row - (int64_t)b * P);
        const float4* src = (const float4*)slab + ii;
        float4 acc = src[0];
        for (int sp = 1; sp < S; ++sp) {
            const float4 t = src[sp * slab_stride4];
            acc.x += t.x; acc.y += t.y; acc.z += t.z; acc.w += t.w;
        }
        const float4 g4 = *(const float4*)(G + (int64_t)pos * Cout + n);
        const float4 h4 = *(const float4*)(Hb + (int64_t)pos * Cout + n);
        const float4 go = *(const float4*)(gamma_out + (int64_t)pos * Cout + n);
        const float rb = sR[b - b_first], cb = sC[b - b_first];
        float4 tq, v;
        tq.x = fmaf(rb, acc.x, fmaf(cb, g4.x, h4.x));
        tq.y = fmaf(rb, acc.y, fmaf(cb, g4.y, h4.y));
        tq.z = fmaf(rb, acc.z, fmaf(cb, g4.z, h4.z));
        tq.w = fmaf(rb, acc.w, fmaf(cb, g4.w, h4.w));
        v.x = elu1(tq.x); v.y = elu1(tq.y); v.z = elu1(tq.z); v.w = elu1(tq.w);
        float s = live ? (v.x + v.y) + (v.z + v.w) : 0.f;
        float q = live ? (v.x * v.x + v.y * v.y) + (v.z * v.z + v.w * v.w) : 0.f;
        if (live) {
            ((float4*)y)[idx] = make_float4(v.x * go.x, v.y * go.y, v.z * go.z, v.w * go.w);
            if (v_out) ((float4*)v_out)[idx] = tq;
        }
        const int b_lo = __shfl(b, 0, 64), b_hi = __shfl(b, 63, 64);
        const float s_lo = wave_sum(b == b_lo ? s : 0.f), q_lo = wave_sum(b == b_lo ? q : 0.f);
        const float s_hi = wave_sum(b != b_lo ? s : 0.f), q_hi = wave_sum(b != b_lo ? q : 0.f);
        if (lane == 0) {
            const int w = tid >> 6;
            sPart[w][e][0][0] = s_lo; sPart[w][e][0][1] = q_lo; sPartB[w][e][0] = b_lo;
            sPart[w][e][1][0] = s_hi; sPart[w][e][1][1] = q_hi; sPartB[w][e][1] = b_hi != b_lo ? b_hi : -1;
        }
    }
    __syncthreads();
    if (tid <= b_last - b_first) {
        const int b = b_first + tid;
        double ds = 0.0, dq = 0.0;
        for (int w = 0; w < 4; ++w)
            for (int e = 0; e < FIN_F4 / 256; ++e)
                for (int h = 0; h < 2; ++h)
                    if (sPartB[w][e][h] == b) { ds += (double)sPart[w][e][h][0]; dq += (double)sPart[w][e][h][1]; }
        stat_add(stats_out + 2 * (int64_t)b, ds, inv_n_in < 0.0);
        stat_add(stats_out + 2 * (int64_t)b + 1, dq, inv_n_in < 0.0);
    }
}

static int live_k_steps(const ConvGeom& g) {
    const int n_in = g.axis == 0 ? g.Tin : g.Fin, n_out = g.axis == 0 ? g.Tout : g.Fout;
    int n_live = 0;
    for (int t = 0; t < 3; ++t) {
        bool live = false;
        for (int o = 0; o < n_out && !live; ++o) { const int i = o * g.stride - g.pad + t; live = i >= 0 && i < n_in; }
        n_live += live;
    }
    return n_live * g.Cin / 16;
}

static bool n64_two_stage() {
    static const bool on = []() { const char* e = getenv("NAFP_N64S2"); return !e || e[0] != '0'; }();
    return on;
}

static int choose_split(int64_t n_tiles, int k_steps, int64_t out_floats, double slots = 768.0) {
    static const int force = []() { const char* e = getenv("NAFP_SPLITK"); return e ? atoi(e) : -1; }();
    if (force == 0) return 1;
    if (force > 0) return force;
    if (n_tiles >= 3072) return 1;
    if (slots == 1280.0)
        return (n_tiles >= 1000 || k_steps / 2 < 24 || 2 * out_floats * 4 > ((int64_t)64 << 20)) ? 1 : 2;
    if (slots == 768.0 && n_tiles <= 200) {
        int S = n_tiles <= 40 ? 6 : 3;
        while (S > 1 && (k_steps / S < 8 || (int64_t)S * out_floats * 4 > ((int64_t)64 << 20))) --S;
        return S;
    }
    const double overhead_steps = 6.0;
    int best = 1; double best_score = 0.0;
    for (int S = 1; S <= 16; ++S) {
        const double k = (double)k_steps / S;
        if (S > 1 && (k < 8.0 || (int64_t)S * out_floats * 4 > ((int64_t)64 << 20))) break;
        const double w = (double)n_tiles * S;
        const double rounds = (double)((int64_t)((w + slots - 1) / slots));
        double score = (w / (rounds * slots)) * (k / (k + overhead_steps));
        if (S > 1) score *= 0.93;
        if (score > best_score + 1e-9) { best_score = score; best = S; }
    }
    return best;
}

__global__ __launch_bounds__(256) void plain_finish_kernel(const float* __restrict__ slab, int S, const float* __restrict__ bias,
                                                          float* __restrict__ y, int64_t n4, int Cout) {
    for (int64_t i = blockIdx.x * 256ll + threadIdx.x; i < n4; i += (int64_t)gridDim.x * 256) {
        float4 acc = ((const float4*)slab)[i];
        for (int sp = 1; sp < S; ++sp) {
            const float4 t = ((const float4*)slab)[i + sp * n4];
            acc.x += t.x; acc.y += t.y; acc.z += t.z; acc.w += t.w;
        }
        if (bias) {
            const float4 bv = *(const float4*)(bias + (4 * i) % Cout);
            acc.x += bv.x; acc.y += bv.y; acc.z += bv.z; acc.w += bv.w;
        }
        ((float4*)y)[i] = acc;
    }
}

static int dgrad_k_steps(const ConvGeom& g) { return (g.stride == 2 ? 3 : 6) * g.Cout / 32; }

static int tile_pt(int P) {
    int pt = 1;
    while (pt * 2 <= P && pt * 2 <= 32) pt *= 2;
    return pt;
}

struct FwdTile { int pt, perm; double saved; };
static FwdTile fwd_tile(const ConvGeom& g, int BM) {
    const int P = g.Fout * g.Tout;
    FwdTile r{tile_pt(P), 0, 0.0};
    static const int mode = []() { const char* e = getenv("NAFP_TAPCLASS"); return e ? atoi(e) : 1; }();
    const int L = g.axis == 0 ? g.Tout : g.Fout, n_in = g.axis == 0 ? g.Tin : g.Fin;
    if (!mode || L < 2) return r;
// ... 155 lines not shown
        while ((1 << p.log2ST) < p.ST) ++p.log2ST;
        p.n_sg = (int)((B + p.ST - 1) / p.ST);
        p.sample_in = (int64_t)g.Fout * g.Tout * g.Cout;
        const int S = g.axis == 0 ? g.Cout : g.Tout * g.Cout;
        p.tap_stride = -(S / g.stride);
        p.inv_n_in = 1.0;
        const int L = g.axis == 0 ? g.Tin : g.Fin;
        if (g.stride == 2 && L >= 2) {
            p.perm_on = 1; p.perm_c0 = g.pad & 1;
            p.perm_n0 = (L - p.perm_c0 + 1) / 2;
        } else if (g.stride == 1 && g.axis == 0 && L == 2 && g.pad == 1) {
            p.perm_on = 2;
        }
        k_steps = dgrad_k_steps(g);
    }
    if ((int64_t)p.ST * p.sample_in * 4 >= ((int64_t)1 << 31)) return NAFP_ERR_UNSUPPORTED;
    const int64_t wbytes = (int64_t)g.Cout * 3 * g.Cin * 4;
    if (wbytes >= ((int64_t)1 << 31)) return NAFP_ERR_UNSUPPORTED;
    p.wp_bytes = (unsigned)wbytes;
    static const int abl = []() { const char* e = getenv("NAFP_ABL"); return e ? atoi(e) : 0; }();
    p.abl = a.plain ? 0 : abl;
    p.tl = nullptr;
    static const int gemm_prio = []() { const char* e = getenv("NAFP_GEMM_PRIO"); return e ? atoi(e) : 0; }();
    p.opt = gemm_prio;
    const int n_pb = (p.P + p.PT - 1) / p.PT;
    const int64_t n_tiles128 = (int64_t)p.n_sg * n_pb * (p.Cout / BN);
    const int64_t n_tiles128_plan = ((Bp + p.ST - 1) / p.ST) * n_pb * (p.Cout / BN);
    int bn = (BM == 256 || a.f0_feat) ? 128 : pick_bn(n_tiles128_plan, p.Cout, (a.plain || a.dgrad) ? 0 : k_steps);
    const bool plan_forced = BM == 128 && !a.plain && !a.dgrad && !a.f0_feat && plan_override().bn > 0;
    if (plan_forced && (plan_override().bn == 128 || p.Cout % 64 == 0)) bn = plan_override().bn;
    const bool dplan_forced = BM == 128 && a.dgrad && dgrad_plan_override().bn > 0;
    if (dplan_forced && (dgrad_plan_override().bn == 128 || p.Cout % 64 == 0)) bn = dgrad_plan_override().bn;
    const int64_t n_tiles = n_tiles128 * (BN / bn);
    int S = 1;
    const int64_t out_floats = B * p.P * p.Cout;
    if (a.slab && !a.f0_feat && BM == 128) {
        S = choose_split(n_tiles128_plan * (BN / bn), k_steps, Bp * p.P * p.Cout, bn == 64 ? ((n64_two_stage() && !a.plain) ? 1280.0 : 1024.0) : 768.0);
        if (plan_forced && plan_override().S > 0) { S = plan_override().S; while (S > 1 && k_steps / S < 4) --S; }
        if (dplan_forced && dgrad_plan_override().S > 0) { S = dgrad_plan_override().S; while (S > 1 && k_steps / S < 4) --S; }
        if ((int64_t)S * out_floats > a.slab_floats) S = 1;
        if (x6 && bn == 64 && S == 2 && (p.ST == 4 || p.ST == 8)) S = 1;
    }
    if (S > 1) { p.mode = a.plain ? 1 : 2; p.n_split = S; p.y = a.slab; p.bias = nullptr; }
    static const int fin_min = []() { const char* e = getenv("NAFP_SPLIT_INKERNEL"); return e ? atoi(e) : 320; }();
    const bool in_kernel_finish = fin_min > 0 && S > 1 && !a.plain && bn == 64 && a.tickets && n_tiles128_plan * (BN / bn) >= fin_min &&
                                  (int64_t)n_pb * (p.Cout / bn) <= NAFP_TICKET_SLOTS;
    static const int plain_fin = []() { const char* e = getenv("NAFP_PLAIN_INKERNEL"); return e ? atoi(e) : 1; }();
    const bool plain_in_kernel = plain_fin > 0 && S > 1 && a.plain && a.tickets && n_tiles <= NAFP_TICKET_SLOTS && !x6d;
    p.tickets = (in_kernel_finish || plain_in_kernel) ? a.tickets : nullptr; p.y_final = a.y;
    if (plain_in_kernel) p.bias = a.bias;
    static const int grid3d = []() { const char* e = getenv("NAFP_GRID3D"); return e ? atoi(e) : 1; }();
    static const int xcdmap = []() { const char* e = getenv("NAFP_XCDMAP"); return e ? atoi(e) : 1; }();
    const int n_col = p.Cout / bn;
    p.n_pb = n_pb; p.log2_ncol = 0; p.xcd_group = 1; p.xcd_full = 0;
    while ((1 << p.log2_ncol) < n_col) ++p.log2_ncol;
    const int64_t total_wg = (int64_t)p.n_sg * n_pb * n_col * S;
    bool xm = xcdmap != 0 && !a.f0_feat && !in_kernel_finish && !plain_in_kernel && (1 << p.log2_ncol) == n_col && total_wg < ((int64_t)1 << 31);
    if (xm) {
        const double a_bytes = (double)B * (double)p.sample_in * 4.0, w_bytes = (double)k_steps * 16.0 * p.Cout * 4.0;
        const bool row_fast = xcdmap == 3 || (xcdmap == 1 && w_bytes > a_bytes);
        p.xcd_group = row_fast ? p.n_sg * n_pb : n_col * S;
        p.xcd_full = (int)(total_wg / (8 * (int64_t)p.xcd_group) * (8 * (int64_t)p.xcd_group));
        if (p.xcd_group <= 1 || p.xcd_full == 0) xm = false;
        else p.opt |= row_fast ? (8 | 16) : 8;
    }
    const bool g3 = !xm && S == 1 && grid3d != 0 && (grid3d == 1 || BM == 256 || bn == 128);
    if (g3) p.opt |= 4;
    const dim3 grid = xm ? dim3((unsigned)total_wg)
                    : g3 ? dim3((unsigned)p.n_sg, (unsigned)n_pb, (unsigned)(p.Cout / bn))
                         : dim3((unsigned)((int64_t)p.n_sg * n_pb), (unsigned)(p.Cout / bn), (unsigned)S);
    if (!xm && (n_pb > 65535 || p.Cout / bn > 65535)) return NAFP_ERR_UNSUPPORTED;
    if (g_timeline.buf && ((!a.plain && !a.dgrad && g.Cin == g_timeline.cin) || (a.dgrad && g.Cin == -g_timeline.cin)) &&
        g.Cout == g_timeline.cout && g.Fout * g.Tout == g_timeline.positions &&
        (int64_t)grid.x * grid.y * grid.z * 64 <= g_timeline.capacity) {
        p.tl = g_timeline.buf;
        g_timeline.last_grid[0] = (int)grid.x; g_timeline.last_grid[1] = (int)grid.y; g_timeline.last_grid[2] = (int)grid.z;
        g_timeline.last_grid[3] = BM; g_timeline.last_grid[4] = bn;
    }
    int rc;
    const bool finish_follows = S > 1 && !in_kernel_finish && !plain_in_kernel;
    g_ev_start = a.ev_start; g_ev_stop = finish_follows ? nullptr : a.ev_stop;
    p.f0_feat = nullptr; p.f0_w = nullptr; p.f0_bias = nullptr; p.f0_gamma = nullptr;
    p.f0_T = 0; p.f0_stride = 1; p.f0_pad = 0; p.f0_gstat = nullptr; p.f0_group = 0; p.f0_segnorm = 0;
    p.sj = (a.sj && a.plain) ? *a.sj : ScalarsJob{nullptr, nullptr, nullptr, nullptr, 0, 0.0};
    if (a.f0_feat) {
        if (a.plain || S != 1 || !a.f0_geom || g.axis != 1 || a.f0_geom->Cout != g.Cin || a.f0_geom->Tout != g.Tin ||
            a.f0_geom->Fin != g.Fin || g.Cin % 16 != 0)
            return NAFP_ERR_UNSUPPORTED;
        p.f0_feat = a.f0_feat; p.f0_w = a.f0_w; p.f0_bias = a.f0_bias; p.f0_gamma = a.f0_gamma;
        p.f0_T = a.f0_geom->Tin; p.f0_stride = a.f0_geom->stride; p.f0_pad = a.f0_geom->pad;
        if (a.v_out || (p.ST != 4 && p.ST != 8)) return NAFP_ERR_UNSUPPORTED;
        p.f0_gstat = a.f0_gstat; p.f0_group = a.f0_group; p.f0_segnorm = a.f0_segnorm;
        if (a.bf16x3 == 2 && a.wp_hm && a.wp_l) {
            if (g.Cin != 128) return NAFP_ERR_UNSUPPORTED;
            p.wp_hm = a.wp_hm; p.wp_l = (const unsigned short*)a.wp_l;
            return launch_variant(conv_gemm_k16s2_fuse0_bf16x6, 128, 128, 16, 2, p, grid, st, 128 * 8 + 128 * 8);
        }
        return launch_variant(conv_gemm_k16s3_fuse0, 128, 128, 16, 3, p, grid, st);
    }
    const bool fast_st = p.ST == 4 || p.ST == 8;
    if (plain_in_kernel)
        return bn == 64 ? launch_variant(conv_gemm_n64k16s3_plainfin, 128, 64, 16, 3, p, grid, st)
                        : launch_variant(conv_gemm_k16s3_plainfin, 128, 128, 16, 3, p, grid, st);
    const int epi = in_kernel_finish ? 4 : p.mode != 0 ? 3 : (!fast_st ? 2 : (p.v_out ? 1 : 0));
    const bool two_stage = n64_two_stage() && bn == 64 && (epi == 0 || epi == 1 || epi == 4);
    if (a.bf16x3 == 2 && epi == 0 && (bn == 128 || two_stage) && a.wp_hm && a.wp_l) {
        p.wp_hm = a.wp_hm; p.wp_l = (const unsigned short*)a.wp_l;
        return BM == 256 ? launch_variant(conv_gemm_m256k16s3_infer_bf16x6, 256, 128, 16, NAFP_X6_M256_NSTAGE, p, grid, st, 128 * 8)
             : bn == 64 ? launch_variant(conv_gemm_n64k16s2_infer_bf16x6, 128, 64, 16, 2, p, grid, st, 64 * 8)
                        : launch_variant(conv_gemm_k16s3_infer_bf16x6, 128, 128, 16, NAFP_X6_K16_NSTAGE, p, grid, st, 128 * 8);
    }
    static const bool x6_any = []() { const char* e = getenv("NAFP_X6_ANY"); return !e || e[0] != '0'; }();
    if (x6 && epi == 2 && BM == 128 && x6_any) {
        p.wp_hm = a.wp_hm; p.wp_l = (const unsigned short*)a.wp_l;
        return bn == 64 ? launch_variant(conv_gemm_n64k16s2_any_bf16x6, 128, 64, 16, 2, p, grid, st, 64 * 8)
                        : launch_variant(conv_gemm_k16s3_any_bf16x6, 128, 128, 16, NAFP_X6_K16_NSTAGE, p, grid, st, 128 * 8);
    }
    if (x6 && epi == 1 && BM == 128 && (bn == 128 || two_stage)) {
        p.wp_hm = a.wp_hm; p.wp_l = (const unsigned short*)a.wp_l;
        return bn == 64 ? launch_variant(conv_gemm_n64k16s2_train_bf16x6, 128, 64, 16, 2, p, grid, st, 64 * 8)
                        : launch_variant(conv_gemm_k16s3_train_bf16x6, 128, 128, 16, NAFP_X6_K16_NSTAGE, p, grid, st, 128 * 8);
    }
    if (a.bf16x3 && epi == 0 && (bn == 128 || two_stage))
        return BM == 256 ? launch_variant(conv_gemm_m256k16s3_infer_bf16x3, 256, 128, 16, 3, p, grid, st)
             : bn == 64 ? launch_variant(conv_gemm_n64k16s2_infer_bf16x3, 128, 64, 16, 2, p, grid, st)
                        : launch_variant(conv_gemm_k16s3_infer_bf16x3, 128, 128, 16, 3, p, grid, st);
    if (x6 && epi == 3 && bn == 128 && BM == 128 && p.mode == 2) {
        p.wp_hm = a.wp_hm; p.wp_l = (const unsigned short*)a.wp_l;
        rc = launch_variant(conv_gemm_k16s3_plain_bf16x6, 128, 128, 16, NAFP_X6_K16_NSTAGE, p, grid, st, 128 * 8);
    } else if (x6d && epi == 3 && BM == 128) {
        p.wp_hm = a.wp_hm; p.wp_l = (const unsigned short*)a.wp_l;
        rc = bn == 64 ? launch_variant(conv_gemm_n64k16s2_plain_bf16x6, 128, 64, 16, 2, p, grid, st, 64 * 8)
                      : launch_variant(conv_gemm_k16s3_plain_bf16x6, 128, 128, 16, NAFP_X6_K16_NSTAGE, p, grid, st, 128 * 8);
    } else if (in_kernel_finish && n_tiles > NAFP_TICKET_SLOTS) {
        const int64_t tiles_per_sg = (int64_t)n_pb * (p.Cout / bn);
        const int64_t sg_per_launch = NAFP_TICKET_SLOTS / tiles_per_sg;
        const int64_t b_step = sg_per_launch * p.ST;
        const int64_t out_per_sample = (int64_t)p.P * p.Cout;
        hipEvent_t ev0 = g_ev_start, ev1 = g_ev_stop;
        rc = NAFP_OK;
        for (int64_t b0 = 0; b0 < B && rc == NAFP_OK; b0 += b_step) {
            ConvKernelParams q = p;
            const int64_t bc = std::min<int64_t>(b_step, B - b0);
            q.B = (int)bc; q.n_sg = (int)((bc + p.ST - 1) / p.ST);
            q.x = p.x + b0 * p.sample_in; q.y_final = p.y_final + b0 * out_per_sample;
            if (p.v_out) q.v_out = p.v_out + b0 * out_per_sample;
            q.stats_in = p.stats_in + 2 * b0; q.stats_out = p.stats_out + 2 * b0;
            g_ev_start = b0 == 0 ? ev0 : nullptr; g_ev_stop = b0 + b_step >= B ? ev1 : nullptr;
            const dim3 gq((unsigned)((int64_t)q.n_sg * n_pb), (unsigned)(p.Cout / bn), (unsigned)S);
            rc = two_stage ? launch_variant(conv_gemm_n64k16s2_tab[epi], 128, 64, 16, 2, q, gq, st)
                           : launch_variant(conv_gemm_n64k16s3_tab[epi], 128, 64, 16, 3, q, gq, st);
        }
        return rc;
    } else
    rc = BM == 256 ? launch_variant(conv_gemm_m256k16s3_tab[epi], 256, 128, 16, 3, p, grid, st)
         : (bn == 64 && two_stage) ? launch_variant(conv_gemm_n64k16s2_tab[epi], 128, 64, 16, 2, p, grid, st)
         : bn == 64 ? launch_variant(conv_gemm_n64k16s3_tab[epi], 128, 64, 16, 3, p, grid, st)
                    : launch_variant(conv_gemm_k16s3_tab[epi], 128, 128, 16, 3, p, grid, st);
    if (rc != NAFP_OK || S == 1 || in_kernel_finish) return rc;
    if (a.plain) {
        const int64_t n4 = out_floats / 4;
        const dim3 fgrid((unsigned)std::min<int64_t>((n4 + 255) / 256, 8192));
        if (a.ev_stop) hipExtLaunchKernelGGL(plain_finish_kernel, fgrid, dim3(256), 0, st, nullptr, a.ev_stop, 0, (const float*)a.slab, S, a.bias, a.y, n4, p.Cout);
        else plain_finish_kernel<<<fgrid, 256, 0, st>>>(a.slab, S, a.bias, a.y, n4, p.Cout);
        NAFP_LAUNCH_CHECK();
        return NAFP_OK;
    }
    if (4096 / g.Cout + 1 > FIN_MAXS || g.Cout < 128) return NAFP_ERR_UNSUPPORTED;
    const int64_t f4 = out_floats / 4;
    const int64_t f4_plan = Bp * p.P * p.Cout / 4;
#define NAFP_FIN(E_)                                                                                             \
    if (a.ev_stop) hipExtLaunchKernelGGL(splitk_finish_kernel<E_>, dim3((unsigned)((f4 + (E_) - 1) / (E_))), dim3(256), 0, st, nullptr,   \
                                         a.ev_stop, 0, (const float*)a.slab, S, a.G, a.Hb, a.gamma_out, a.stats_in, a.stats_out, a.y,   \
                                         a.v_out, p.B, p.P, g.Cout, p.inv_n_in);                                   \
    else splitk_finish_kernel<E_><<<dim3((unsigned)((f4 + (E_) - 1) / (E_))), 256, 0, st>>>(                       \
        a.slab, S, a.G, a.Hb, a.gamma_out, a.stats_in, a.stats_out, a.y, a.v_out, p.B, p.P, g.Cout, p.inv_n_in)
    if (f4_plan >= 1024 * 1024) { NAFP_FIN(1024); }
    else if (f4_plan >= 1024 * 512) { NAFP_FIN(512); }
    else { NAFP_FIN(256); }
#undef NAFP_FIN
    NAFP_LAUNCH_CHECK();
    return NAFP_OK;
}

struct DgradLnParams {
    ConvKernelParams c;
    const float* t;
    const float* gamma;
    const float* G; const float* Hb;
    const float* sc;
    float* dts;
    float* dgamma; float* dbeta; float* dbias;
    float* S1; float* S2;
    double* lnsum_below;
    int n_groups, groups_per_wg, n_chunks;
};

__global__ __launch_bounds__(256, 3) void dgrad_ln_kernel(const DgradLnParams q) {
    constexpr int BM = 128, BK = 16, NSTAGE = 3, CH = 4, RPI = 16, NI = 2;
    constexpr int TILE = BM * BK, STAGE = 2 * TILE;
    constexpr unsigned OOB = 0x80000000u;
    const ConvKernelParams& p = q.c;
    extern __shared__ __attribute__((aligned(16))) float smem[];
    float* sSc = smem + NSTAGE * STAGE;
    float* sRow = sSc + BM * 8;
    float* sCol = sRow + BM * 2;
    float* sDummy = sCol + 5 * BN;
    const int tid = threadIdx.x, lane = tid & 63;
    const int wave = __builtin_amdgcn_readfirstlane(tid >> 6);
    const int wm = wave >> 1, wn = wave & 1;
    const int chunk = blockIdx.x % q.n_chunks;
    const int pos = tile_pos(p, blockIdx.x / q.n_chunks);
    const int tile_n0 = blockIdx.y * BN;
    const int K = 3 * p.Cin;
    const int C = p.Cout;
    const RowGeom rg = row_geom(p, pos);
    unsigned tap_pack = 0; int n_live = 0;
#pragma unroll
    for (int t = 0; t < 3; ++t)
        if (rg.mask & (1u << t)) { tap_pack |= (unsigned)t << (2 * n_live); ++n_live; }
    const int cpt = p.Cin / BK, n_steps = n_live * cpt;

    unsigned voffA[NI], voffB[NI];
#pragma unroll
    for (int i = 0; i < NI; ++i) {
        const int lr = wave * 32 + i * RPI + lane / CH;
        const int lc = (lane % CH) ^ ((lr >> 2) & 3);
        voffA[i] = (unsigned)(lr * (int)p.sample_in + rg.inner + lc * 4) * 4u;
        voffB[i] = (unsigned)((tile_n0 + lr) * K + lc * 4) * 4u;
    }
    const u32x4 rsB = make_rsrc(p.wp, p.wp_bytes);
    const unsigned lds0 = (unsigned)(unsigned long long)(lds_ptr_t)smem + (unsigned)(wave * 32 * BK * 4);
    const int rl = lane & 31, hh = lane >> 5;
    const int rswz = (rl >> 2) & 3;
    const int aoff = (wm * 64 + rl) * BK, boff = TILE + (wn * 64 + rl) * BK;
    const int ncol = lane & 31;
    const int n_base = tile_n0 + wn * 64 + ncol;
    float gam[2], Gq[2], Hq[2];
#pragma unroll
    for (int ni = 0; ni < 2; ++ni) {
        const int o = pos * C + n_base + ni * 32;
        gam[ni] = q.gamma[o];
        Gq[ni] = q.lnsum_below ? q.G[o] : 0.f;
        Hq[ni] = q.lnsum_below ? q.Hb[o] : 0.f;
    }
    float ag[2] = {0.f, 0.f}, ab[2] = {0.f, 0.f}, a1[2] = {0.f, 0.f}, a2[2] = {0.f, 0.f};

    const int g_begin = chunk * q.groups_per_wg, g_end = min(q.n_groups, g_begin + q.groups_per_wg);
    for (int grp = g_begin; grp < g_end; ++grp) {
        const int b0 = grp * BM;
        const int nb = min(BM, p.B - b0);
        {
            const int r = tid >> 1, h = tid & 1;
            float4 v = make_float4(0.f, 0.f, 0.f, 0.f);
            if (r < nb) v = *(const float4*)(q.sc + 8 * (int64_t)(b0 + r) + 4 * h);
            *(float4*)(sSc + 8 * r + 4 * h) = v;
            sRow[tid] = 0.f;
            asm volatile("s_waitcnt lgkmcnt(0)" ::: "memory");
        }
        const u32x4 rsA = make_rsrc(p.x + (int64_t)b0 * p.sample_in, (unsigned)nb * (unsigned)p.sample_in * 4u);
        f32x16 acc[2][2];
#pragma unroll
        for (int mi = 0; mi < 2; ++mi)
#pragma unroll
            for (int ni = 0; ni < 2; ++ni)
#pragma unroll
                for (int r = 0; r < 16; ++r) acc[mi][ni][r] = 0.f;
#define NAFP_DL_DMA(s_, slot_)                                                                 \
        {                                                                                      \
            const int tsel_l = (s_) / cpt;                                                     \
            const int tap_l = (int)((tap_pack >> (2 * tsel_l)) & 3u);                          \
            const int c0_l = ((s_) - tsel_l * cpt) * BK;                                       \
            const unsigned la_l = lds0 + (unsigned)((slot_) * STAGE * 4);                      \
            const unsigned tapb_l = (unsigned)(tap_l * p.tap_stride) * 4u;                     \
            _Pragma("unroll") for (int i = 0; i < NI; ++i) {                                   \
                const int lr_l = wave * 32 + i * RPI + lane / CH;                              \
                lds_dma16(la_l + i * RPI * BK * 4, lr_l < nb ? voffA[i] + tapb_l : OOB, rsA, (unsigned)(c0_l * 4)); \
                lds_dma16(la_l + (TILE + i * RPI * BK) * 4, voffB[i], rsB, (unsigned)((tap_l * p.Cin + c0_l) * 4)); \
            }                                                                                  \
        }
#pragma unroll
        for (int s = 0; s < NSTAGE - 1; ++s)
            if (s < n_steps) NAFP_DL_DMA(s, s)
        int slot = 0;
        for (int s = 0; s < n_steps; ++s) {
            if (s + NSTAGE - 2 >= n_steps) asm volatile("s_waitcnt vmcnt(0)" ::: "memory");
            else asm volatile("s_waitcnt vmcnt(%0)" :: "i"((NSTAGE - 2) * 2 * NI) : "memory");
            __builtin_amdgcn_s_barrier();
            int nslot = slot + NSTAGE - 1; if (nslot >= NSTAGE) nslot -= NSTAGE;
            const float* St = smem + slot * STAGE;
            float4 a0[2], b0v[2];
            {
                const int pc4 = ((0 + hh) ^ rswz) * 4;
#pragma unroll
                for (int mi = 0; mi < 2; ++mi) a0[mi] = *(const float4*)(St + aoff + mi * 32 * BK + pc4);
#pragma unroll
                for (int ni = 0; ni < 2; ++ni) b0v[ni] = *(const float4*)(St + boff + ni * 32 * BK + pc4);
            }
            if (s + NSTAGE - 1 < n_steps) NAFP_DL_DMA(s + NSTAGE - 1, nslot)
#pragma unroll
            for (int kk = 0; kk < BK / 8; ++kk) {
                const int pc4 = ((2 * kk + hh) ^ rswz) * 4;
                float4 a[2], b[2];
#pragma unroll
                for (int mi = 0; mi < 2; ++mi) a[mi] = kk == 0 ? a0[mi] : *(const float4*)(St + aoff + mi * 32 * BK + pc4);
#pragma unroll
                for (int ni = 0; ni < 2; ++ni) b[ni] = kk == 0 ? b0v[ni] : *(const float4*)(St + boff + ni * 32 * BK + pc4);
// ... 286 lines not shown
```

neural-audio-fp_amd/csrc/nafp_common.h:

```cpp
#pragma once
#include <hip/hip_runtime.h>
#include <stdint.h>
#include <vector>

#include "../../include/nafp.h"

namespace nafp {

extern thread_local int g_last_hip_error;

#define NAFP_HIP_CHECK(expr)                                   \
    do {                                                       \
        hipError_t _e = (expr);                                \
        if (_e != hipSuccess) {                                \
            nafp::g_last_hip_error = (int)_e;                  \
            return NAFP_ERR_HIP;                               \
        }                                                      \
    } while (0)

#define NAFP_LAUNCH_CHECK() NAFP_HIP_CHECK(hipGetLastError())

constexpr float LN_EPS = 1e-3f;

struct SamePad { int n_out, before, after; };
inline SamePad same_pad(int n_in, int k, int s) {
    int n_out = (n_in + s - 1) / s;
    int total = (n_out - 1) * s + k - n_in;
    if (total < 0) total = 0;
    return {n_out, total / 2, total - total / 2};
}

struct ConvGeom {
    int axis;
    int Fin, Tin, Cin;
    int Fout, Tout, Cout;
    int stride;
    int pad;
};

std::vector<ConvGeom> encoder_geometry(int in_f, int in_t);

__device__ __forceinline__ float elu1(float v) {
    const float e = __expf(fminf(v, 0.f)) - 1.f;
    return v > 0.f ? v : (v != v ? v : e);
}

__device__ __forceinline__ float max_keep_nan(float v, float lo) { return v < lo ? lo : v; }

typedef long long stat_t;
constexpr int STAT_FRAC_BITS = 20;
constexpr double STAT_PARTIAL_LIMIT = 17179869184.0;
constexpr unsigned long long STAT_POISON = 1ull << 62;
#ifdef __HIPCC__
__device__ __forceinline__ void stat_poison(stat_t* sample_slots) {
    atomicOr((unsigned long long*)(sample_slots + 1), STAT_POISON);
}
__device__ __forceinline__ void stat_add(stat_t* slot, double v, bool range_is_benign = false) {
    if (fabs(v) < STAT_PARTIAL_LIMIT)
        atomicAdd((unsigned long long*)slot, (unsigned long long)__double2ll_rn(v * (double)(1 << STAT_FRAC_BITS)));
    else if (!(range_is_benign && fabs(v) < 1.0e300))
        atomicOr((unsigned long long*)((uintptr_t)slot | 8), STAT_POISON);
}
__device__ __forceinline__ double stat_get(const stat_t* slot) {
    const long long x = *slot;
    if (((uintptr_t)slot & 8) && (unsigned long long)x >= STAT_POISON) return __builtin_nan("");
    return (double)x * (1.0 / (double)(1 << STAT_FRAC_BITS));
}
__device__ __forceinline__ void stat_ln_scalars(const stat_t* sample_slots, double inv_n, float* r, float* c) {
    if (inv_n < 0.0) { const double z = stat_get(sample_slots + 1) * 0.0; *r = (float)(1.0 + z); *c = (float)z; return; }
    const double mean = stat_get(sample_slots) * inv_n;
    double var = stat_get(sample_slots + 1) * inv_n - mean * mean;
    var = var < 0.0 ? 0.0 : var;
    const double rstd = 1.0 / sqrt(var + (double)LN_EPS);
    *r = (float)rstd; *c = (float)(-mean * rstd);
}
__device__ __forceinline__ bool stat_is_poisoned(const stat_t* sample_slots) {
    return (unsigned long long)sample_slots[1] >= STAT_POISON;
}
__device__ __forceinline__ void stat_forward_poison(const stat_t* in_slots, stat_t* out_slots) {
    if (stat_is_poisoned(in_slots)) stat_poison(out_slots);
}
#endif

__device__ __forceinline__ float wave_sum(float v) {
#pragma unroll
    for (int o = 32; o > 0; o >>= 1) v += __shfl_xor(v, o, 64);
    return v;
}
__device__ __forceinline__ double wave_sum(double v) {
#pragma unroll
    for (int o = 32; o > 0; o >>= 1) v += __shfl_xor(v, o, 64);
    return v;
}
__device__ __forceinline__ float wave_max(float v) {
#pragma unroll
    for (int o = 32; o > 0; o >>= 1) v = fmaxf(v, __shfl_xor(v, o, 64));
    return v;
}
__device__ __forceinline__ float wave_min(float v) {
#pragma unroll
    for (int o = 32; o > 0; o >>= 1) v = fminf(v, __shfl_xor(v, o, 64));
    return v;
}

__device__ __forceinline__ void atomic_max_float(float* addr, float v) {
    if (v >= 0.f) atomicMax((int*)addr, __float_as_int(v));
    else          atomicMin((unsigned int*)addr, __float_as_uint(v));
}
__device__ __forceinline__ void atomic_min_float(float* addr, float v) {
    if (v >= 0.f) atomicMin((int*)addr, __float_as_int(v));
    else          atomicMax((unsigned int*)addr, __float_as_uint(v));
}


int launch_conv0(const float* feat, const float* w3, const float* bias, const float* gamma, float* y,
                 float* v_out, stat_t* stats, int64_t B, const ConvGeom& g, hipStream_t st,
                 const float* gstat = nullptr, int group_size = 0, int segment_norm = 0, bool ident_stats = false);

constexpr int NAFP_TICKET_SLOTS = 4096;
struct ScalarsJob { const float* mr; const double* lnsum; const float* mr_prev; float* sc; long long B; double inv_n; };
struct ConvGemmArgs {
    const float* x;
    const float* wp;
    const float* G;
    const float* Hb;
    const float* gamma_out;
    const float* bias;
    const stat_t* stats_in;
    bool ident_stats;
    stat_t* stats_out;
    float* y;
    float* v_out;
    bool plain;
    bool dgrad;
    float* slab;
    int64_t slab_floats;
    hipEvent_t ev_start, ev_stop;
    const float* wp_hm; const void* wp_l;
    int bf16x3;
    unsigned* tickets;
    const float* f0_feat; const float* f0_w; const float* f0_bias; const float* f0_gamma;
    const ConvGeom* f0_geom;
    const float* f0_gstat; int f0_group, f0_segnorm;
    const ScalarsJob* sj;
    int64_t plan_b;
};
int launch_conv0_stats(const float* feat, const float* w3, const float* bias, stat_t* stats, int64_t B,
                       const ConvGeom& g, hipStream_t st, const float* gstat = nullptr, int group_size = 0, int segment_norm = 0);
int64_t conv_gemm_slab_floats(int64_t B, const ConvGeom& g, bool with_dgrad = false, int64_t plan_b = 0);
int64_t fwd_plan_b();
int launch_conv_gemm(const ConvGemmArgs& a, int64_t B, const ConvGeom& g, hipStream_t st);
int conv_timeline_set(unsigned long long* buf, int64_t capacity_u64, int cin, int cout, int positions);
int conv_timeline_grid(int* out5);

struct DgradLnArgs {
    const float* dts_in; const float* wd;
    const float* t; const float* gamma; const float* G; const float* Hb; const float* sc;
    float* dts_out; float* dgamma; float* dbeta; float* dbias; float* S1; float* S2; double* lnsum_below;
};
bool dgrad_ln_eligible(int64_t B, const ConvGeom& g, int mode);
int launch_dgrad_ln(const DgradLnArgs& a, int64_t B, const ConvGeom& g, hipStream_t st);
int launch_ln_bwd_scalars(const float* mr, const double* lnsum, const float* mr_prev, float* sc, int64_t B, int64_t n, hipStream_t st);

struct TailArgs {
    const float* x;
    const stat_t* stats;
    const float* gamma;
    const float* beta;
    const float* w1p;
    const float* b1p;
    const float* w2p;
    const float* b2;
    float* out_flat;
    float* out_emb;
    int D, Q, S, l2norm;
    bool ident_stats;
    const int* nonfinite_weights;
    const unsigned* launch_error;
};
int launch_tail(const TailArgs& a, int64_t B, hipStream_t st);

struct TailBwdArgs {
    const float* z; const stat_t* stats; const float* gamma; const float* beta;
    bool ident_stats;
    const float* w1; const float* b1; const float* w2; const float* b2;
    const float* w1p; const float* b1p; const float* w2p;
    const float* d_emb;
    float* dy;
    float* ln;
    float* dxh;
    float* dw1; float* db1; float* dw2; float* db2;
    int D, Q, S, l2norm;
};
int launch_tail_bwd(const TailBwdArgs& a, int64_t B, hipStream_t st);
int launch_stats_to_mr(const stat_t* stats, float* mr, const double* inv_n_dev, int64_t B, int n_layers, hipStream_t st, bool identity = false);
int launch_ln_bwd(float* d, const float* tpre, const float* gamma, const float* mr, const float* mr_prev,
                  double* lnsum, float* sc, float* dgamma, float* dbeta, float* dbias, float* S1, float* S2,
                  int64_t B, int P, int C, hipStream_t st, bool reduce_here, const float* Gj, const float* Hbj,
                  double* lnsum_below, const float* feat0 = nullptr, const float* w0 = nullptr, const float* bias0 = nullptr,
                  const ConvGeom* g0 = nullptr, float* dW0 = nullptr, bool scalars_done = false,
                  float* part_slab = nullptr, int64_t part_slab_floats = 0, unsigned* tickets = nullptr, bool tpre_is_z = false);
int launch_wgrad(const float* X, const float* D, float* dW, int64_t B, const ConvGeom& g, hipStream_t st,
                 const float* X2 = nullptr, const float* D2 = nullptr, float* slab = nullptr, int64_t slab_floats = 0,
                 unsigned* tickets = nullptr, const ScalarsJob* sj = nullptr, int prec = 0);
int64_t wgrad_slab_floats(int64_t B, const ConvGeom& g);
int launch_conv0_bwd(const float* feat, const float* dt, float* dW0, float* dbias0, int64_t B, const ConvGeom& g,
                     hipStream_t st);
int launch_pack_dgrad_weight(const float* k3, float* wd, int Cin, int Cout, hipStream_t st);

struct BnExpandTable { const float* gamma_c[16]; const float* beta_c[16]; const float* mmean[16]; const float* mvar[16];
                       float* gamma_pos[16]; int64_t n[16]; int C[16]; int count; };
int launch_bn_expand(const BnExpandTable& t, hipStream_t st);
int launch_bn_param_grad(const float* dgp, const float* dbp, int P, int C, const float* mmean, const float* mvar, float* dgamma_c,
                         float* dbeta_c, hipStream_t st);
int launch_ln1d_fwd(float* x, int64_t rows, int C, const float* gamma_c, const float* beta_c, hipStream_t st);
int launch_ln1d_bwd(float* d, const float* tpre, int64_t rows, int C, const float* gamma_c, float* dgamma_c, float* dbeta_c, hipStream_t st);

struct PackTable { const float* k3[16]; float* wp[16]; float* wd[16]; int cin[16], cout[16]; int unit0[17]; int count;
                   int* nonfinite; };
int launch_multi_pack(const PackTable& t, hipStream_t st);
struct SplitTable { const float* wp[32]; float* hm[32]; void* wl[32]; int64_t n8[32]; int K[32]; int count; };
int launch_split_weights_multi(const SplitTable& t, hipStream_t st);
int launch_pack_conv_weight(const float* k3, float* wp, int Cin, int Cout, hipStream_t st);
constexpr int GH_MAX_LAYERS = 8;
struct GhTable {
    const float* wp[GH_MAX_LAYERS];
    const float* x[GH_MAX_LAYERS];
    float* y[GH_MAX_LAYERS];
    int cin[GH_MAX_LAYERS], cout[GH_MAX_LAYERS], P[GH_MAX_LAYERS], sample_in[GH_MAX_LAYERS];
    int src[GH_MAX_LAYERS][8][3];
    int wg0[GH_MAX_LAYERS + 1];
    int count;
};
bool gh_gemv_eligible(const ConvGeom& g);
void gh_table_add(GhTable& t, const ConvGeom& g, const float* wp, const float* x, float* y);
int launch_gh_gemv(const GhTable& t, hipStream_t st);
int launch_pack_div(const float* w1, const float* b1, const float* w2, float* w1p, float* b1p,
                    float* w2p, int Q, int S, hipStream_t st);

}
```

Measured before the change: 188,500.

## Add 4-wave 256x128 conv GEMM tile variant for inference layers

Adds a WIDE variant of the conv GEMM body where a 256x128 tile is computed by 4 waves (256 threads) instead of 8. Each wave covers the full 128 columns, so it does more MFMA work per wave and gets more B-fragment reuse. DMA issue is split into halves and the row-stat accumulation is split into per-column-group partials. It is enabled by default for BM=256 inference launches through a new option and env var. In exchange it raises register pressure and gives fewer waves per block to hide latency.

Result: no change. 187,400 (median of 2 runs) (-0.6%).

```diff
diff --git a/include/nafp.h b/include/nafp.h
--- a/include/nafp.h
+++ b/include/nafp.h
@@ -103,6 +103,7 @@
 #define NAFP_OPT_FUSED_LN_BWD 2
 #define NAFP_OPT_BWD_OVERLAP 4
 #define NAFP_OPT_SMALLNET 5
+#define NAFP_OPT_CONV_TILE 8
 #define NAFP_OPT_BF16X3 3
 int nafp_encoder_set_option(nafp_encoder* enc, int option, int value);
 
diff --git a/neural-audio-fp_amd/csrc/api.hip b/neural-audio-fp_amd/csrc/api.hip
--- a/neural-audio-fp_amd/csrc/api.hip
+++ b/neural-audio-fp_amd/csrc/api.hip
@@ -104,6 +104,7 @@
     int64_t bufA_per_seg = 0, bufB_per_seg = 0;
     std::vector<hipEvent_t> prof_events;
     int prof_max = 0, prof_count = 0;
+    int opt_conv_tile = []() { const char* v = getenv("NAFP_CONV_TILE"); return v ? (atoi(v) != 0 ? 1 : 0) : 1; }();
     int opt_bf16x3 = 0;
     float* d_x6_blob = nullptr; std::vector<float*> d_whm; std::vector<void*> d_wl; bool x6_dirty = true;
     std::vector<float*> d_wdhm; std::vector<void*> d_wdl;
@@ -342,6 +343,9 @@
             if (value < 0 || value > 2) return NAFP_ERR_INVALID_ARG;
             e->opt_fused_ln_bwd = value; return NAFP_OK;
         case NAFP_OPT_BWD_OVERLAP: e->opt_bwd_overlap = value < 0 ? 0 : (value > 2 ? 1 : value); return NAFP_OK;
+        case NAFP_OPT_CONV_TILE:
+            if (value < 0 || value > 1) return NAFP_ERR_INVALID_ARG;
+            e->opt_conv_tile = value; return NAFP_OK;
         case NAFP_OPT_SMALLNET: return NAFP_OK;
         case NAFP_OPT_DEBUG_SIDE_DELAY:
         case NAFP_OPT_DEBUG_SW_DELAY: {
@@ -620,6 +624,7 @@
         static const int x6_layers = []() { const char* v = getenv("NAFP_X6_LAYERS"); return v ? (int)strtol(v, nullptr, 0) : 0xffff; }();
         if (!((x6_layers >> j) & 1)) a.bf16x3 = 0;
         if (a.bf16x3 == 2) { a.wp_hm = e->d_whm[j]; a.wp_l = e->d_wl[j]; }
+        a.conv_tile = e->opt_conv_tile;
         a.plan_b = fwd_plan_b();
         if (j == 1 && fuse0) {
             a.x = nullptr; a.f0_feat = feat; a.f0_w = e->d_w[0]; a.f0_bias = e->d_bias[0];
diff --git a/neural-audio-fp_amd/csrc/conv.hip b/neural-audio-fp_amd/csrc/conv.hip
--- a/neural-audio-fp_amd/csrc/conv.hip
+++ b/neural-audio-fp_amd/csrc/conv.hip
@@ -361,17 +361,21 @@
 #ifndef NAFP_EXP_SKIP_TAP2
 #define NAFP_EXP_SKIP_TAP2 0
 #endif
-template <int BM, int BNT, int BK, int NSTAGE, bool FUSE0, int EPI, int PREC = 0>
+template <int BM, int BNT, int BK, int NSTAGE, bool FUSE0, int EPI, int PREC = 0, bool WIDE = false>
 __device__ __forceinline__ bool conv_gemm_body(const ConvKernelParams& p) {
     static_assert(!FUSE0 || (BK == 16 && BM == 128), "the in-kernel conv0 generator is written for BK = 16, BM = 128");
     static_assert(BM == 128 || BM == 256, "tile rows");
     static_assert(BNT == 128 || (BNT == 64 && BM == 128 && !FUSE0), "tile columns");
-    constexpr int NIW = BNT / 64;
-    constexpr int NT = 2 * BM;
-    constexpr int NW = BM / 32;
+    static_assert(!WIDE || (BM == 256 && BNT == 128 && BK == 16 && NSTAGE == 3 && !FUSE0 && EPI == 0 && PREC == 0), "the 4-wave tile");
+    constexpr int NWN = WIDE ? 1 : 2;
+    constexpr int NIW = BNT / (32 * NWN);
+    constexpr int NW = (BM / 64) * NWN;
+    constexpr int NT = 64 * NW;
+    constexpr int SP = WIDE ? 2 : 1;
     constexpr int CH = BK / 4;
     constexpr int RPI = 64 / CH;
-    constexpr int NI = 32 / RPI;
+    constexpr int AROWS = BM / NW;
+    constexpr int NI = AROWS / RPI;
     constexpr int BROWS = BNT / NW;
     constexpr int NIB = BROWS / RPI;
     static_assert(NIB >= 1, "B rows per wave");
@@ -390,7 +394,7 @@
     float* sW0 = sCB + BM + 96;
     const int tid = threadIdx.x, lane = tid & 63;
     const int wave = __builtin_amdgcn_readfirstlane(tid >> 6);
-    const int wm = wave >> 1, wn = wave & 1;
+    const int wm = wave / NWN, wn = wave % NWN;
     int sg = blockIdx.x, pb = blockIdx.y, colz = blockIdx.z, zsp = 0;
     if (p.opt & 8) {
         const unsigned lin = blockIdx.x, G = (unsigned)p.xcd_group;
@@ -474,7 +478,7 @@
     }
 #pragma unroll
     for (int q = 0; q < NI; ++q) {
-        const int lr = wave * 32 + q * RPI + lane / CH;
+        const int lr = wave * AROWS + q * RPI + lane / CH;
         const int pc = lane % CH;
         const int swz = BK == 32 ? ((lr >> 1) & 7) : ((lr >> 2) & 3);
         const int lc = pc ^ swz;
@@ -557,7 +561,7 @@
     const u32x4 rsA = make_rsrc(p.x + (int64_t)b0 * p.sample_in,
                                 NAFP_ABL(p, 512) ? 0u : (unsigned)nb * (unsigned)p.sample_in * 4u);
     const u32x4 rsB = make_rsrc(PREC == 2 ? p.wp_hm : p.wp, NAFP_ABL(p, 4096) ? 0u : p.wp_bytes);
-    const unsigned lds0 = (unsigned)(unsigned long long)(lds_ptr_t)smem + (unsigned)(wave * 32 * BK * 4);
+    const unsigned lds0 = (unsigned)(unsigned long long)(lds_ptr_t)smem + (unsigned)(wave * AROWS * BK * 4);
     const unsigned ldsB0 = (unsigned)(unsigned long long)(lds_ptr_t)smem + (unsigned)((TILE + wave * BROWS * BK) * 4);
     const u32x4 rsL = make_rsrc((const float*)p.wp_l, NAFP_ABL(p, 4096) ? 0u : p.wp_bytes / 2);
     const unsigned ldsL0 = (unsigned)(unsigned long long)(lds_ptr_t)smem + (unsigned)((TILE + TILEB) * 4 + wave * LROWS * 32);
@@ -648,11 +652,12 @@
 
     const int rl = lane & 31, hh = lane >> 5;
     const int rswz = BK == 32 ? ((rl >> 1) & 7) : ((rl >> 2) & 3);
-    const int aoff = (wm * 64 + rl) * BK, boff = TILE + (wn * (BNT / 2) + rl) * BK;
+    const int aoff = (wm * 64 + rl) * BK, boff = TILE + (wn * (BNT / NWN) + rl) * BK;
     const int ncol = lane & 31;
-    const int n_base = tile_n0 + wn * (BNT / 2) + ncol;
+    const int n_base = tile_n0 + wn * (BNT / NWN) + ncol;
     const int g4 = p.ST >> 2;
     constexpr int MIL = 1;
+    constexpr bool PREF = (EPI == 0 || EPI == 1) && !FUSE0 && BK == 16 && (BM == 128 || WIDE) && PREC == 0;
     float Gv[MIL][4][NIW], Hv[MIL][4][NIW], gv[MIL][4][NIW];
     const int pc_bytes = p.P * p.Cout * 4;
     const __amdgpu_buffer_rsrc_t rsG = __builtin_amdgcn_make_buffer_rsrc(const_cast<float*>(p.G), 0, pc_bytes, 0x00020000);
@@ -712,6 +717,8 @@
                                       (unsigned)((d_tap * p.Cin + d_c0) * 4));                 \
             if ((q_) == NI - 1) { d_c0 += BK; if (d_c0 == p.Cin) { d_c0 = 0; ++d_tsel; NAFP_DMA_TAP() } } \
         }
+#define NAFP_DMA_HALF(h_, slot_)                                                               \
+        _Pragma("unroll") for (int q = (h_) * (NI / 2); q < ((h_) + 1) * (NI / 2); ++q) NAFP_DMA_PIECE(q, slot_)
 #define NAFP_MM_HALF(a_, b_, mi_)                                                              \
         _Pragma("unroll") for (int ni = 0; ni < NIW; ++ni) {                                   \
             acc[mi_][ni] = __builtin_amdgcn_mfma_f32_32x32x2f32(a_[mi_].x, b_[ni].x, acc[mi_][ni], 0, 0, 0); \
@@ -719,7 +726,7 @@
             acc[mi_][ni] = __builtin_amdgcn_mfma_f32_32x32x2f32(a_[mi_].z, b_[ni].z, acc[mi_][ni], 0, 0, 0); \
             acc[mi_][ni] = __builtin_amdgcn_mfma_f32_32x32x2f32(a_[mi_].w, b_[ni].w, acc[mi_][ni], 0, 0, 0); \
         }
-        static_assert(NI == 2, "the DMA of a step is issued as two pieces");
+        static_assert(NI % 2 == 0 && (PREC == 0 || NI == 2), "the DMA of a step is issued in two halves");
         if (PREC >= 1) {
             typedef __bf16 bf16x8 __attribute__((ext_vector_type(8)));
             for (int s = s_begin; s < n_steps; ++s) {
@@ -747,7 +754,7 @@
                     for (int ni = 0; ni < NIW; ++ni) {
                         bh[ni] = *(const bf16x8*)(St + boff + ni * 32 * BK + ((hh ^ rswz) * 4));
                         bm[ni] = *(const bf16x8*)(St + boff + ni * 32 * BK + (((2 + hh) ^ rswz) * 4));
-                        bl[ni] = *(const bf16x8*)(St + TILE + TILEB + (wn * (BNT / 2) + ni * 32 + rl) * 8 + hh * 4);
+                        bl[ni] = *(const bf16x8*)(St + TILE + TILEB + (wn * (BNT / NWN) + ni * 32 + rl) * 8 + hh * 4);
                     }
                 }
                 if (has_next) { NAFP_DMA_PIECE(0, nslot) NAFP_DMA_L(nslot, d_tap * p.Cin + d_c0) NAFP_DMA_PIECE(1, nslot) }
@@ -826,7 +833,7 @@
             NAFP_LD_FRAG(St, 0, a0, b0)
             NAFP_LD_FRAG(St, 1, a1, b1)
             __builtin_amdgcn_sched_barrier(0);
-            if (s_begin + NSTAGE - 1 < n_steps && !NAFP_ABL(p, 1)) { NAFP_DMA_PIECE(0, NSTAGE - 1) NAFP_DMA_PIECE(1, NSTAGE - 1) }
+            if (s_begin + NSTAGE - 1 < n_steps && !NAFP_ABL(p, 1)) { NAFP_DMA_HALF(0, NSTAGE - 1) NAFP_DMA_HALF(1, NSTAGE - 1) }
             __builtin_amdgcn_sched_barrier(0);
             NAFP_MM_FRAG(a0, b0)
             __builtin_amdgcn_sched_barrier(0);
@@ -845,11 +852,11 @@
             __builtin_amdgcn_sched_barrier(0);                                                 \
             NAFP_MM_HALF(a1, b1, 0)                                                            \
             __builtin_amdgcn_sched_barrier(0);                                                 \
-            if (has_next) { NAFP_DMA_PIECE(0, nslot) }                                         \
+            if (has_next) { NAFP_DMA_HALF(0, nslot) }                                          \
             __builtin_amdgcn_sched_barrier(0);                                                 \
             NAFP_MM_HALF(a1, b1, 1)                                                            \
             __builtin_amdgcn_sched_barrier(0);                                                 \
-            if (has_next) { NAFP_DMA_PIECE(1, nslot) }                                         \
+            if (has_next) { NAFP_DMA_HALF(1, nslot) }                                          \
             NAFP_LD_FRAG(St, 1, a1, b1)                                                        \
             __builtin_amdgcn_sched_barrier(0);                                                 \
             if (s == n_steps - 1) break;           \
@@ -876,11 +883,12 @@
             }
         }
 #undef NAFP_K_STEP
-        if ((EPI == 0 || EPI == 1) && BM == 128) { NAFP_EPI_LOAD(0, 0) }
+        if (PREF) { NAFP_EPI_LOAD(0, 0) }
         __builtin_amdgcn_sched_barrier(0);
         if (s_begin + 1 < n_steps) { NAFP_MM_FRAG(a0, b0) }
         NAFP_MM_FRAG(a1, b1)
         }
+#undef NAFP_DMA_HALF
 #undef NAFP_DMA_PIECE
 #undef NAFP_DMA_TAP
 #undef NAFP_MM_HALF
@@ -950,7 +958,7 @@
         _Pragma("unroll") for (int ni = 0; ni < NIW; ++ni) {                                   \
             bh[ni] = *(const bf16x8*)((St_) + boff + ni * 32 * BK + ((hh ^ rswz) * 4));        \
             bm[ni] = *(const bf16x8*)((St_) + boff + ni * 32 * BK + (((2 + hh) ^ rswz) * 4));  \
-            bl[ni] = *(const bf16x8*)((St_) + TILE + TILEB + (wn * (BNT / 2) + ni * 32 + rl) * 8 + hh * 4); \
+            bl[ni] = *(const bf16x8*)((St_) + TILE + TILEB + (wn * (BNT / NWN) + ni * 32 + rl) * 8 + hh * 4); \
         }
         int s = 0;
         for (; s + 1 < n_steps; ++s) {
@@ -1142,7 +1150,11 @@
         }
     }
 
-    f32x2 s2[2] = {{0.f, 0.f}, {0.f, 0.f}}, q2[2] = {{0.f, 0.f}, {0.f, 0.f}};
+    f32x2 s2[SP][2], q2[SP][2];
+#pragma unroll
+    for (int g = 0; g < SP; ++g)
+#pragma unroll
+        for (int qp = 0; qp < 2; ++qp) { s2[g][qp] = (f32x2){0.f, 0.f}; q2[g][qp] = (f32x2){0.f, 0.f}; }
     float* rowS = smem;
     float* rowQ = smem + BM;
     const bool fast_stats = (EPI != 2 && EPI != 4) || p.ST == 4 || p.ST == 8;
@@ -1150,7 +1162,6 @@
         if (tid < BM) { rowS[tid] = 0.f; rowQ[tid] = 0.f; }
         __syncthreads();
     }
-    constexpr bool PREF = (EPI == 0 || EPI == 1) && !FUSE0 && BK == 16 && BM == 128 && PREC == 0;
     if (MIL == 2) { if (!PREF) { NAFP_EPI_LOAD(0, 0) } NAFP_EPI_LOAD(1, MIL - 1) }
     const __amdgpu_buffer_rsrc_t rsY = __builtin_amdgcn_make_buffer_rsrc(
         (EPI == 4 ? p.y_final : p.y) + (int64_t)b0 * p.P * p.Cout, 0, (int)((unsigned)nb * (unsigned)ystep_b), 0x00020000);
@@ -1168,7 +1179,8 @@
             _Pragma("unroll") for (int qp = 0; qp < 2; ++qp) {              \
                 const int r0 = rg * 4 + 2 * qp;                                                \
                 const f32x2 rb2 = *(const f32x2*)(sRB + sl0 + 2 * qp), cb2 = *(const f32x2*)(sCB + sl0 + 2 * qp); \
-                f32x2 rs2 = {0.f, 0.f}, rq2 = {0.f, 0.f};                                      \
+                f32x2 rs2[SP], rq2[SP];                                                        \
+                _Pragma("unroll") for (int g = 0; g < SP; ++g) { rs2[g] = (f32x2){0.f, 0.f}; rq2[g] = (f32x2){0.f, 0.f}; } \
                 _Pragma("unroll") for (int ni = 0; ni < NIW; ++ni) {                           \
                     const f32x2 a2 = {acc[mi][ni][r0], acc[mi][ni][r0 + 1]};                   \
                     const f32x2 t2 = __builtin_elementwise_fma(rb2, a2, __builtin_elementwise_fma(cb2, (f32x2)(Gv[ms][rg][ni]), (f32x2)(Hv[ms][rg][ni]))); \
@@ -1182,12 +1194,13 @@
                         __builtin_amdgcn_raw_buffer_store_b32(f2i(t2.x), rsV, voff, (2 * qp) * ystep_b + ni * 128, NAFP_T_AUX); \
                         __builtin_amdgcn_raw_buffer_store_b32(f2i(t2.y), rsV, voff, (2 * qp + 1) * ystep_b + ni * 128, NAFP_T_AUX); \
                     }                                                                          \
-                    rs2 += v2; rq2 = __builtin_elementwise_fma(v2, v2, rq2);                   \
+                    const int g = ni / (NIW / SP);                                             \
+                    rs2[g] += v2; rq2[g] = __builtin_elementwise_fma(v2, v2, rq2[g]);          \
                 }                                                                              \
-                if (FAST_) { s2[qp] += rs2; q2[qp] += rq2; }                                   \
-                else {                                                                         \
+                if (FAST_) { _Pragma("unroll") for (int g = 0; g < SP; ++g) { s2[g][qp] += rs2[g]; q2[g][qp] += rq2[g]; } } \
+                else _Pragma("unroll") for (int g = 0; g < SP; ++g) {                          \
                     _Pragma("unroll") for (int h2 = 0; h2 < 2; ++h2) {                         \
-                        float rs = rs2[h2], rq = rq2[h2];                                      \
+                        float rs = rs2[g][h2], rq = rq2[g][h2];                                \
                         _Pragma("unroll") for (int o = 16; o > 0; o >>= 1) { rs += __shfl_xor(rs, o, 64); rq += __shfl_xor(rq, o, 64); } \
                         if (ncol == 0) { atomicAdd(rowS + (grp << 2) + 2 * qp + h2, rs); atomicAdd(rowQ + (grp << 2) + 2 * qp + h2, rq); } \
                     }                                                                          \
@@ -1205,19 +1218,22 @@
 #undef NAFP_EPI_MAIN
     NAFP_TL(6)
     if NAFP_ABL(p, 16) {
-        if (s2[0].x + s2[0].y + s2[1].x + s2[1].y + q2[0].x + q2[0].y + q2[1].x + q2[1].y == 12345.678f) p.y[tid] = 1.f;
+        if (s2[0][0].x + s2[0][0].y + s2[0][1].x + s2[0][1].y + q2[0][0].x + q2[0][0].y + q2[0][1].x + q2[0][1].y == 12345.678f) p.y[tid] = 1.f;
         return false;
     }
     if (fast_stats) {
         double* red = (double*)smem;
-        float hs[4], hq[4];
-#pragma unroll
-        for (int q = 0; q < 4; ++q) { hs[q] = half_wave_sum_dpp(s2[q >> 1][q & 1]); hq[q] = half_wave_sum_dpp(q2[q >> 1][q & 1]); }
-        if ((lane & 31) == 31) {
-#pragma unroll
-            for (int q = 0; q < 4; ++q) {
-                red[wave * 16 + (lane >> 5) * 8 + q] = (double)hs[q];
-                red[wave * 16 + (lane >> 5) * 8 + 4 + q] = (double)hq[q];
+#pragma unroll
+        for (int g = 0; g < SP; ++g) {
+            float hs[4], hq[4];
+#pragma unroll
+            for (int q = 0; q < 4; ++q) { hs[q] = half_wave_sum_dpp(s2[g][q >> 1][q & 1]); hq[q] = half_wave_sum_dpp(q2[g][q >> 1][q & 1]); }
+            if ((lane & 31) == 31) {
+#pragma unroll
+                for (int q = 0; q < 4; ++q) {
+                    red[(wave * SP + g) * 16 + (lane >> 5) * 8 + q] = (double)hs[q];
+                    red[(wave * SP + g) * 16 + (lane >> 5) * 8 + 4 + q] = (double)hq[q];
+                }
             }
         }
         __syncthreads();
@@ -1228,10 +1244,10 @@
                 double t = 0.0;
                 if (p.ST == 8) {
 #pragma unroll
-                    for (int w = 0; w < NW; ++w) t += red[w * 16 + (sl >> 2) * 8 + which * 4 + (sl & 3)];
+                    for (int w = 0; w < NW * SP; ++w) t += red[w * 16 + (sl >> 2) * 8 + which * 4 + (sl & 3)];
                 } else {
 #pragma unroll
-                    for (int w = 0; w < NW; ++w) t += red[w * 16 + which * 4 + sl] + red[w * 16 + 8 + which * 4 + sl];
+                    for (int w = 0; w < NW * SP; ++w) t += red[w * 16 + which * 4 + sl] + red[w * 16 + 8 + which * 4 + sl];
                 }
                 stat_add(p.stats_out + 2 * (int64_t)b + which, t, p.inv_n_in < 0.0);
             }
@@ -1290,6 +1306,9 @@
 NAFP_GEMM_KERNEL(conv_gemm_m256k16s3_infer, 256, 128, 16, 3, 4, false, 0)
 NAFP_GEMM_KERNEL(conv_gemm_m256k16s3_train, 256, 128, 16, 3, 4, false, 1)
 NAFP_GEMM_KERNEL(conv_gemm_m256k16s3_plain, 256, 128, 16, 3, 4, false, 3)
+__global__ __launch_bounds__(256, 2) void conv_gemm_m256w4k16s3_infer(const ConvKernelParams p) {
+    conv_gemm_body<256, 128, 16, 3, false, 0, 0, true>(p);
+}
 static void (*const conv_gemm_m256k16s3_tab[4])(const ConvKernelParams) = {conv_gemm_m256k16s3_infer, conv_gemm_m256k16s3_train, nullptr,
                                                                             conv_gemm_m256k16s3_plain};
 
@@ -1367,17 +1386,17 @@
 
 template <typename KernelT>
 static int launch_variant(KernelT kernel, int BM, int BNt, int BK, int NSTAGE, const ConvKernelParams& p, dim3 grid, hipStream_t st,
-                          int extra_stage_floats = 0) {
+                          int extra_stage_floats = 0, int threads = 0) {
     static const int lds_pad = []() { const char* e = getenv("NAFP_LDS_PAD"); return e ? atoi(e) : 0; }();
     const int lds = (NSTAGE * ((BM + BNt) * BK + extra_stage_floats) + 2 * BM + 96 + (p.f0_feat ? 4 * p.Cin : 0)) * (int)sizeof(float) + lds_pad;
     NAFP_HIP_CHECK(hipFuncSetAttribute((const void*)kernel, hipFuncAttributeMaxDynamicSharedMemorySize, lds));
     if (g_ev_start || g_ev_stop) {
         ConvKernelParams pc = p;
         void* args[] = {(void*)&pc};
-        NAFP_HIP_CHECK(hipExtLaunchKernel((const void*)kernel, grid, dim3(2 * BM), args, (size_t)lds, st, g_ev_start, g_ev_stop, 0));
+        NAFP_HIP_CHECK(hipExtLaunchKernel((const void*)kernel, grid, dim3(threads ? threads : 2 * BM), args, (size_t)lds, st, g_ev_start, g_ev_stop, 0));
         g_ev_start = nullptr; g_ev_stop = nullptr;
     } else {
-        kernel<<<grid, 2 * BM, lds, st>>>(p);
+        kernel<<<grid, threads ? threads : 2 * BM, lds, st>>>(p);
     }
     NAFP_LAUNCH_CHECK();
     return NAFP_OK;
@@ -1839,7 +1858,9 @@
                            : launch_variant(conv_gemm_n64k16s3_tab[epi], 128, 64, 16, 3, q, gq, st);
         }
         return rc;
-    } else
+    } else if (BM == 256 && epi == 0 && a.conv_tile == 1)
+    rc = launch_variant(conv_gemm_m256w4k16s3_infer, 256, 128, 16, 3, p, grid, st, 0, 256);
+    else
     rc = BM == 256 ? launch_variant(conv_gemm_m256k16s3_tab[epi], 256, 128, 16, 3, p, grid, st)
          : (bn == 64 && two_stage) ? launch_variant(conv_gemm_n64k16s2_tab[epi], 128, 64, 16, 2, p, grid, st)
          : bn == 64 ? launch_variant(conv_gemm_n64k16s3_tab[epi], 128, 64, 16, 3, p, grid, st)
diff --git a/neural-audio-fp_amd/csrc/nafp_common.h b/neural-audio-fp_amd/csrc/nafp_common.h
--- a/neural-audio-fp_amd/csrc/nafp_common.h
+++ b/neural-audio-fp_amd/csrc/nafp_common.h
@@ -143,6 +143,7 @@
     const ConvGeom* f0_geom;
     const float* f0_gstat; int f0_group, f0_segnorm;
     const ScalarsJob* sj;
+    int conv_tile;
     int64_t plan_b;
 };
 int launch_conv0_stats(const float* feat, const float* w3, const float* bias, stat_t* stats, int64_t B,
```
